# KumarRobotics/top_down_renderer

Measured on AMD Instinct MI355X. Metric: particle-updates/sec (render+score+resample), higher is better.
Workload: dtype f32

## Files before the change

### top_down_renderer_amd/csrc/tdr_common.h

```cpp
#ifndef TDR_COMMON_H_
#define TDR_COMMON_H_
#include <hip/hip_runtime.h>

#include <cmath>
#include <cstdarg>
#include <cstdint>
#include <cstdio>
#include <cstdlib>
#include <cstring>
#include <limits>
#include <type_traits>
#include <utility>
#include <vector>

#include "tdr.h"

#ifndef TDR_SCORE_U
#define TDR_SCORE_U 4
#endif
#ifndef TDR_INIT_SCAN_LDS
#define TDR_INIT_SCAN_LDS 1
#endif
#ifndef TDR_XCD_SWIZZLE
#define TDR_XCD_SWIZZLE 0
#endif
#ifndef TDR_OOB_ALIAS
#define TDR_OOB_ALIAS 1
#endif

int tdr_fail(int code, const char* fmt, ...);
#define fail tdr_fail
#define HIP_TRY(expr)                                                                       \
  do {                                                                                      \
    hipError_t e_ = (expr);                                                                 \
    if (e_ != hipSuccess) return fail(TDR_ERR_HIP, "%s: %s", #expr, hipGetErrorString(e_)); \
  } while (0)
#define LAUNCH_CHECK(name)                                                                   \
  do {                                                                                       \
    hipError_t e_ = hipGetLastError();                                                       \
    if (e_ != hipSuccess) return fail(TDR_ERR_HIP, "launch %s: %s", name, hipGetErrorString(e_)); \
  } while (0)

int tdr_libm_fma();

static inline int64_t cdiv(int64_t a, int64_t b) { return (a + b - 1) / b; }

template <class F>
static inline int with_flags(F&& f) { return f(); }
template <class F, class... Rest>
static inline int with_flags(F&& f, bool b, Rest... rest) {
  auto next = [&](auto B) { return with_flags([&](auto... bs) { return f(B, bs...); }, rest...); };
  return b ? next(std::true_type{}) : next(std::false_type{});
}
template <class F>
static inline int with_nv4(int rf, const char* who, F&& f) {
  switch (rf / 4) {
    case 1: return f(std::integral_constant<int, 1>{});
    case 2: return f(std::integral_constant<int, 2>{});
    case 3: return f(std::integral_constant<int, 3>{});
    case 4: return f(std::integral_constant<int, 4>{});
    default: return fail(TDR_ERR_ARG, "%s: unsupported record size %d", who, rf);
  }
}

int tdr_chain_total(const float* raw, const float* mean_dev, int kind, int64_t n, float* total_out, void* workspace,
                    hipStream_t st);
int tdr_uw_small(const float* raw, const float* last_dist, int64_t n, float* w, float* info, hipStream_t st);
int tdr_mt_raw_stream(const uint32_t* state, int64_t nblocks, uint32_t* raw, hipStream_t s);
int tdr_mt_advance(const uint32_t* raw, int64_t nblocks, const uint32_t* consumed, uint32_t* state, hipStream_t s);
bool tdr_score_polar_float_form(const tdr_map_desc* map, int nb, int nr, int64_t n, int64_t n_total);
__host__ __device__ inline bool tdr_has_kslot(int ncls, int rf) { return ncls + 2 <= rf; }
uint32_t* tdr_profile_stats_ptr();
#endif
```

### top_down_renderer_amd/csrc/tdr_filter.hip

```cpp
#include <random>

#include <rocprim/device/device_radix_sort.hpp>
using TdrSortConfig = rocprim::radix_sort_config<rocprim::default_config, rocprim::merge_sort_config<512, 512, 4>, rocprim::default_config>;

#include "tdr_common.h"
#include "tdr_filter_dev.h"

__device__ __forceinline__ uint32_t mulhi32(uint32_t a, uint32_t b) { return __umulhi(a, b); }
__device__ void philox4x32_10(uint32_t c[4], uint32_t k0, uint32_t k1) {
#pragma unroll
  for (int r = 0; r < 10; r++) {
    uint32_t hi0 = mulhi32(0xD2511F53u, c[0]), lo0 = 0xD2511F53u * c[0];
    uint32_t hi1 = mulhi32(0xCD9E8D57u, c[2]), lo1 = 0xCD9E8D57u * c[2];
    uint32_t n0 = hi1 ^ c[1] ^ k0, n1 = lo1, n2 = hi0 ^ c[3] ^ k1, n3 = lo0;
    c[0] = n0; c[1] = n1; c[2] = n2; c[3] = n3;
    k0 += 0x9E3779B9u; k1 += 0xBB67AE85u;
  }
}

__global__ void propagate_kernel(float* __restrict__ st, int64_t cap, int64_t n, float* __restrict__ last_dist,
                                 float tx, float ty, float omega, int scale_freeze, float pos_cov, float theta_cov,
                                 const float* __restrict__ z4, uint64_t seed, uint64_t step, int64_t index_base,
                                 int libm_fma) {
  const int64_t p = (int64_t)blockIdx.x * blockDim.x + threadIdx.x;
// ... 28 lines not shown
}

extern "C" void* tdr_rng_create(uint32_t seed) { return new std::mt19937(seed); }
extern "C" void tdr_rng_destroy(void* rng) { delete (std::mt19937*)rng; }
extern "C" float tdr_rng_uniform_host(void* rng) {
  std::uniform_real_distribution<float> d(0., 1.);
  return d(*(std::mt19937*)rng);
}
extern "C" int tdr_propagate_normals_host(void* rng, int64_t n, int scale_freeze, float* z4) {
  if (!rng || !z4 || n < 0) return fail(TDR_ERR_ARG, "propagate_normals: bad arguments");
  std::mt19937& gen = *(std::mt19937*)rng;
  for (int64_t p = 0; p < n; p++) {
    std::normal_distribution<float> disp{0, 1}, th{0, 1};
    z4[4 * p + 0] = th(gen);
    z4[4 * p + 1] = disp(gen);
    z4[4 * p + 2] = disp(gen);
    if (!scale_freeze) {
      std::normal_distribution<float> sc{0, 1};
      z4[4 * p + 3] = sc(gen);
    } else {
      z4[4 * p + 3] = 0.f;
    }
  }
  return TDR_OK;
}

static bool on_road_host(const float* maps, int ncls, int rows, int cols, float resolution, int px, int py) {
  const int c0 = (int)((float)px / resolution), c1 = (int)((float)py / resolution);
  if (ncls < 2) return false;
  if (!(c0 < cols && c1 < rows && c0 >= 0 && c1 >= 0)) return false;
  return maps[(size_t)1 * rows * cols + c1 + (size_t)rows * c0] < 1;
}
static tdr_state draw_particle(std::mt19937& gen, const float* maps, int ncls, int rows, int cols, float resolution,
                               const tdr_filter_params* fp) {
  std::uniform_real_distribution<float> uniform_dist(0., 1.);
  std::normal_distribution<float> normal_dist(0., 1.);
  tdr_state st;
  std::memset(&st, 0, sizeof(st));
  const float map_w = (float)cols * resolution, map_h = (float)rows * resolution;
  if (fp->fixed_scale < 0) st.scale = (float)std::pow(10, ((double)uniform_dist(gen) - 0.5) * 2);
  else st.scale = fp->fixed_scale;
  while (true) {
    if (fp->init_pos_px_x > 0) {
      st.init_x_px = std::min(std::max(normal_dist(gen) * fp->init_pos_px_cov + fp->init_pos_px_x, 0.f), map_w);
      st.init_y_px = std::min(std::max(normal_dist(gen) * fp->init_pos_px_cov + fp->init_pos_px_y, 0.f), map_h);
    } else {
      st.init_x_px = uniform_dist(gen) * map_w;
      st.init_y_px = uniform_dist(gen) * map_h;
    }
    if (on_road_host(maps, ncls, rows, cols, resolution, (int)st.init_x_px, (int)st.init_y_px)) break;
  }
  if (fp->init_pos_deg_theta != std::numeric_limits<float>::infinity()) {
    st.theta = normal_dist(gen) * fp->init_pos_deg_cov + fp->init_pos_deg_theta;
    st.theta = (float)((double)st.theta * (M_PI / 180));
    st.have_init = 1;
  } else {
    st.theta = 0;
    st.have_init = 0;
  }
  return st;
}
extern "C" int tdr_init_particle_host(void* rng, const float* class_maps, int ncls, int rows, int cols, float resolution,
                                      const tdr_filter_params* fp, tdr_state* out) {
  if (!rng || !class_maps || !fp || !out) return fail(TDR_ERR_ARG, "init_particle: bad arguments");
  if (ncls < 2) return fail(TDR_ERR_ARG, "init_particle: class 1 (road) is required for the on-road test");
  bool any_road = false;
  for (size_t k = 0; k < (size_t)rows * cols && !any_road; k++) any_road = class_maps[(size_t)rows * cols + k] < 1;
  if (!any_road) return fail(TDR_ERR_ARG, "init_particle: the map has no road cell, rejection sampling cannot end");
  *out = draw_particle(*(std::mt19937*)rng, class_maps, ncls, rows, cols, resolution, fp);
  return TDR_OK;
}
extern "C" int tdr_init_particles_host(void* rng, const float* class_maps, int ncls, int rows, int cols,
                                       float resolution, const tdr_filter_params* fp, int max_num, tdr_state* out,
                                       int64_t* n_out) {
  if (!rng || !class_maps || !fp || !out || !n_out || max_num < 0) return fail(TDR_ERR_ARG, "init_particles: bad arguments");
  if (ncls < 2) return fail(TDR_ERR_ARG, "init_particles: class 1 (road) is required for the on-road test");
  std::mt19937& gen = *(std::mt19937*)rng;
  bool any_road = false;
  for (size_t k = 0; k < (size_t)rows * cols && !any_road; k++) any_road = class_maps[(size_t)rows * cols + k] < 1;
  if (!any_road) return fail(TDR_ERR_ARG, "init_particles: the map has no road cell, rejection sampling cannot end");
  const size_t num_at_scale = (fp->fixed_scale < 0) ? 10 : 1;
  int64_t count = 0;
  for (int i = 0; i < (int)((size_t)max_num / num_at_scale); i++) {
    const tdr_state proto = draw_particle(gen, class_maps, ncls, rows, cols, resolution, fp);
    for (float scale = 0; scale < 1; scale += 1. / num_at_scale) {
      tdr_state part = draw_particle(gen, class_maps, ncls, rows, cols, resolution, fp);
      if (fp->fixed_scale < 0) {
        part = proto;
        part.scale = (float)std::pow(10., (double)scale);
      }
      if (count < max_num + 16) out[count] = part;
      count++;
      (void)draw_particle(gen, class_maps, ncls, rows, cols, resolution, fp);
    }
  }
  *n_out = count;
  return TDR_OK;
}

__device__ long long block_sum_ll(long long v, long long* sh) {
  const int lane = threadIdx.x & 63, wave = threadIdx.x >> 6;
  for (int o = 32; o > 0; o >>= 1) v += __shfl_down(v, o, 64);
  __syncthreads();
  if (lane == 0) sh[wave] = v;
  __syncthreads();
  long long t = 0;
  const int nw = blockDim.x >> 6;
  for (int w = 0; w < nw; w++) t += sh[w];
  return t;
}

#define UW_G 256
struct UwScratch {
  double a[UW_G];
  double b[UW_G];
};
__device__ __forceinline__ void uw_chunk(int64_t n, int64_t& lo, int64_t& hi) {
  const int64_t per = (n + UW_G - 1) / UW_G;
  lo = (int64_t)blockIdx.x * per;
  hi = lo + per < n ? lo + per : n;
  if (lo > n) lo = n;
}
__device__ double uw_total(const double* part) {
  __shared__ double stage[UW_G];
  __shared__ double result;
  __syncthreads();
  for (int g = threadIdx.x; g < UW_G; g += blockDim.x) stage[g] = part[g];
  __syncthreads();
  if (threadIdx.x == 0) {
    double t = 0;
    for (int g = 0; g < UW_G; g++) t += stage[g];
    result = t;
  }
  __syncthreads();
  return result;
}
__global__ __launch_bounds__(256) void uw_pass1(const float* __restrict__ raw, int64_t n, UwScratch* s1) {
  __shared__ double shd[4];
  __shared__ long long shl[4];
  int64_t lo, hi;
  uw_chunk(n, lo, hi);
  double s = 0;
  long long c = 0;
  for (int64_t i = lo + threadIdx.x; i < hi; i += 256) {
    const float v = raw[i];
    if (!isnan(v)) { s += (double)v; c++; }
  }
  const double ts = block_sum_d(s, shd);
  const long long tc = block_sum_ll(c, shl);
  if (threadIdx.x == 0) { s1->a[blockIdx.x] = ts; s1->b[blockIdx.x] = (double)tc; }
}
struct UwExact {
  float sum, mean, bsum, pad;
};
__global__ __launch_bounds__(256) void uw_pass2(const float* __restrict__ raw, int64_t n, const UwScratch* s1,
                                                UwScratch* s2, UwExact* ex) {
  __shared__ long long shl[4];
  const float mean = ex->sum / (float)(long long)uw_total(s1->b);
  int64_t lo, hi;
  uw_chunk(n, lo, hi);
  long long cu = 0;
  for (int64_t i = lo + threadIdx.x; i < hi; i += 256) {
    const float v = raw[i];
    if (!isnan(v) && v < mean) cu++;
  }
  const long long tc = block_sum_ll(cu, shl);
  if (threadIdx.x == 0) {
    s2->b[blockIdx.x] = (double)tc;
    if (blockIdx.x == 0) ex->mean = mean;
  }
}
__global__ __launch_bounds__(256) void uw_pass3(const float* __restrict__ raw, int64_t n, const UwExact* ex,
                                                const UwScratch* s2, UwScratch* s3, float* __restrict__ w) {
  __shared__ double shd[4];
  const float sum = ex->sum, mean = ex->mean;
  const long long num_under = (long long)uw_total(s2->b);
  const float bottom = sqrtf(ex->bsum / (float)num_under);
  const bool fallback = (sum == 0.f || num_under < 1);
  const float fill = mean - bottom;
  int64_t lo, hi;
  uw_chunk(n, lo, hi);
  double acc = 0;
  for (int64_t i = lo + threadIdx.x; i < hi; i += 256) {
    float v = raw[i];
    v = fallback ? 1.f : (isnan(v) ? fill : v);
    w[i] = v;
    acc += (double)v;
  }
  const double t = block_sum_d(acc, shd);
  if (threadIdx.x == 0) s3->a[blockIdx.x] = t;
}
__global__ __launch_bounds__(256) void uw_pass4(const float* __restrict__ last_dist, int64_t n, const UwScratch* s3,
                                                UwScratch* s4, float* __restrict__ w) {
  __shared__ double shd[4];
  const float fs1 = (float)uw_total(s3->a);
  const float fn = (float)n;
  int64_t lo, hi;
  uw_chunk(n, lo, hi);
  double acc = 0;
  for (int64_t i = lo + threadIdx.x; i < hi; i += 256) {
    float v = w[i] / fs1;
    const float d = fminf(last_dist[i] * 5.f, 1.f);
    v = d * v + (1.f - d) / fn;
    w[i] = v;
    acc += (double)v;
  }
  const double t = block_sum_d(acc, shd);
  if (threadIdx.x == 0) s4->a[blockIdx.x] = t;
}
__global__ __launch_bounds__(256) void uw_pass5(int64_t n, const UwScratch* s4, UwScratch* s5, float* __restrict__ w) {
  __shared__ float sb[4];
  __shared__ long long si[4];
  const float fs2 = (float)uw_total(s4->a);
  int64_t lo, hi;
  uw_chunk(n, lo, hi);
  float best = -INFINITY;
  long long besti = 0x7fffffffffffffffll;
  for (int64_t i = lo + threadIdx.x; i < hi; i += 256) {
    const float v = w[i] / fs2;
    w[i] = v;
    if (v > best || (v == best && i < besti)) { best = v; besti = i; }
  }
  for (int o = 32; o > 0; o >>= 1) {
    const float ob = __shfl_down(best, o, 64);
    const long long oi = __shfl_down(besti, o, 64);
    if (ob > best || (ob == best && oi < besti)) { best = ob; besti = oi; }
  }
  if ((threadIdx.x & 63) == 0) { sb[threadIdx.x >> 6] = best; si[threadIdx.x >> 6] = besti; }
  __syncthreads();
  if (threadIdx.x == 0) {
    for (int k = 1; k < 4; k++)
      if (sb[k] > best || (sb[k] == best && si[k] < besti)) { best = sb[k]; besti = si[k]; }
    s5->a[blockIdx.x] = (double)best;
    s5->b[blockIdx.x] = (double)besti;
  }
}
__global__ __launch_bounds__(256) void uw_pass6(int64_t n, const UwScratch* s1, const UwScratch* s2,
                                                const UwScratch* s5, const UwExact* ex, float* info) {
  static_assert(UW_G == 256, "one candidate per thread");
  __shared__ float sb[4];
  __shared__ long long si[4];
  float best = (float)s5->a[threadIdx.x];
  long long besti = (long long)s5->b[threadIdx.x];
  if (best != best) { best = -INFINITY; besti = 0x7fffffffffffffffll; }
  for (int o = 32; o > 0; o >>= 1) {
    const float ob = __shfl_down(best, o, 64);
    const long long oi = __shfl_down(besti, o, 64);
    if (ob > best || (ob == best && oi < besti)) { best = ob; besti = oi; }
  }
  if ((threadIdx.x & 63) == 0) { sb[threadIdx.x >> 6] = best; si[threadIdx.x >> 6] = besti; }
  const float sum = ex->sum, mean = ex->mean;
  const long long nv = (long long)uw_total(s1->b), nu = (long long)uw_total(s2->b);
  const float bottom = sqrtf(ex->bsum / (float)nu);
  if (threadIdx.x != 0) return;
  for (int k = 1; k < 4; k++)
    if (sb[k] > best || (sb[k] == best && si[k] < besti)) { best = sb[k]; besti = si[k]; }
  if (besti == 0x7fffffffffffffffll) besti = 0;
  info[0] = __int_as_float((int)besti);
  info[1] = sum; info[2] = mean; info[3] = bottom; info[4] = (sum == 0.f || nu < 1) ? 1.f : 0.f;
  info[5] = (float)nv; info[6] = (float)nu; info[7] = 0.f;
}

#define TDR_UW_SINGLE_MAX_N 32768
extern "C" int tdr_k_update_weights(const float* raw_w, const float* last_dist, int64_t n, float* w_out,
                                    float* info_out, void* stream) {
  if (!raw_w || !last_dist || !w_out || !info_out) return fail(TDR_ERR_ARG, "update_weights: null pointer");
  if (n < 1) return fail(TDR_ERR_ARG, "update_weights: n must be >= 1");
  hipStream_t s = (hipStream_t)stream;
  if (n <= TDR_UW_SINGLE_MAX_N) {
    const int rc = tdr_uw_small(raw_w, last_dist, n, w_out, info_out, s);
    if (rc) return rc;
    LAUNCH_CHECK("update_weights");
    return TDR_OK;
  }
  constexpr size_t kFixed = 8 * sizeof(float) + 64 + 5 * sizeof(UwScratch) + sizeof(UwExact) + 64;
  static_assert(kFixed + 32 * 1024 <= TDR_UW_INFO_FLOATS * sizeof(float), "info scratch");
  UwScratch* sc = reinterpret_cast<UwScratch*>(
      (reinterpret_cast<uintptr_t>(info_out + 8) + 63) & ~(uintptr_t)63);
  UwExact* ex = reinterpret_cast<UwExact*>(sc + 5);
  void* chain_ws = reinterpret_cast<void*>((reinterpret_cast<uintptr_t>(ex + 1) + 63) & ~(uintptr_t)63);
  const size_t chain_room = TDR_UW_INFO_FLOATS * sizeof(float) - kFixed;
  if ((size_t)tdr_prefix_workspace_bytes(n) > chain_room)
    return fail(TDR_ERR_ARG, "update_weights: n = %lld needs more than TDR_UW_INFO_FLOATS of scratch", (long long)n);
  hipLaunchKernelGGL(uw_pass1, dim3(UW_G), dim3(256), 0, s, raw_w, n, sc + 0);
  int rc = tdr_chain_total(raw_w, nullptr, 0, n, &ex->sum, chain_ws, s);
  if (rc) return rc;
  hipLaunchKernelGGL(uw_pass2, dim3(UW_G), dim3(256), 0, s, raw_w, n, (const UwScratch*)(sc + 0), sc + 1, ex);
  rc = tdr_chain_total(raw_w, &ex->mean, 1, n, &ex->bsum, chain_ws, s);
  if (rc) return rc;
  hipLaunchKernelGGL(uw_pass3, dim3(UW_G), dim3(256), 0, s, raw_w, n, (const UwExact*)ex, (const UwScratch*)(sc + 1),
                     sc + 2, w_out);
  hipLaunchKernelGGL(uw_pass4, dim3(UW_G), dim3(256), 0, s, last_dist, n, (const UwScratch*)(sc + 2), sc + 3, w_out);
  hipLaunchKernelGGL(uw_pass5, dim3(UW_G), dim3(256), 0, s, n, (const UwScratch*)(sc + 3), sc + 4, w_out);
  hipLaunchKernelGGL(uw_pass6, dim3(1), dim3(256), 0, s, n, (const UwScratch*)(sc + 0), (const UwScratch*)(sc + 1),
                     (const UwScratch*)(sc + 4), (const UwExact*)ex, info_out);
  LAUNCH_CHECK("update_weights(multi)");
  return TDR_OK;
}

__global__ void resample_kernel(const float* __restrict__ runmax, int64_t n, int64_t n_new, float shift,
                                int64_t i_begin, int64_t i_end, int32_t* __restrict__ idx) {
  const int64_t i = i_begin + (int64_t)blockIdx.x * blockDim.x + threadIdx.x;
  if (i >= i_end) return;
  idx[i - i_begin] = (int32_t)resample_pick(runmax, n, n_new, i, shift);
}

extern "C" int tdr_k_resample(const float* runmax, int64_t n, int64_t n_new, float shift, int64_t i_begin,
                              int64_t i_end, int32_t* idx_out, void* stream) {
  if (!runmax || !idx_out) return fail(TDR_ERR_ARG, "resample: null pointer");
  if (n < 1 || n_new < 1 || i_begin < 0 || i_end > n_new || i_begin > i_end)
    return fail(TDR_ERR_ARG, "resample: bad range");
  if (i_begin == i_end) return TDR_OK;
  hipLaunchKernelGGL(resample_kernel, dim3((unsigned)cdiv(i_end - i_begin, 256)), dim3(256), 0, (hipStream_t)stream,
                     runmax, n, n_new, shift, i_begin, i_end, idx_out);
  LAUNCH_CHECK("resample");
  return TDR_OK;
}

__global__ void resample_dev_kernel(const float* __restrict__ runmax, int64_t n, int64_t n_new, const float* __restrict__ shift_dev,
                                    int64_t i_begin, int64_t i_end, int32_t* __restrict__ idx) {
  const int64_t i = i_begin + (int64_t)blockIdx.x * blockDim.x + threadIdx.x;
  if (i >= i_end) return;
  idx[i - i_begin] = (int32_t)resample_pick(runmax, n, n_new, i, *shift_dev);
}
extern "C" int tdr_k_resample_dev(const float* runmax, int64_t n, int64_t n_new, const float* shift_dev, int64_t i_begin,
                                  int64_t i_end, int32_t* idx_out, void* stream) {
  if (!runmax || !idx_out || !shift_dev) return fail(TDR_ERR_ARG, "resample: null pointer");
  if (n < 1 || n_new < 1 || i_begin < 0 || i_end > n_new || i_begin > i_end)
    return fail(TDR_ERR_ARG, "resample: bad range");
  if (i_begin == i_end) return TDR_OK;
  hipLaunchKernelGGL(resample_dev_kernel, dim3((unsigned)cdiv(i_end - i_begin, 256)), dim3(256), 0, (hipStream_t)stream,
                     runmax, n, n_new, shift_dev, i_begin, i_end, idx_out);
  LAUNCH_CHECK("resample");
  return TDR_OK;
}

__global__ void gather_states_kernel(const float* __restrict__ src, int64_t src_cap, int64_t src_shard,
                                     const int32_t* __restrict__ idx, int64_t n_new, float* __restrict__ dst,
                                     int64_t dst_cap) {
  const int64_t i = (int64_t)blockIdx.x * blockDim.x + threadIdx.x;
  if (i >= n_new) return;
  const int64_t j = idx[i];
  if (src_shard > 0) {
    const int64_t r = j / src_shard, l = j - r * src_shard;
#pragma unroll
    for (int f = 0; f < TDR_ST_FIELDS; f++) dst[f * dst_cap + i] = src[(r * TDR_ST_FIELDS + f) * src_shard + l];
  } else {
    gather_particle(src, src_cap, j, dst, dst_cap, i);
  }
}

extern "C" int tdr_k_gather_states(const float* src, int64_t src_cap, int64_t src_shard, const int32_t* idx,
                                   int64_t n_new, float* dst, int64_t dst_cap, void* stream) {
  if (!src || !idx || !dst) return fail(TDR_ERR_ARG, "gather_states: null pointer");
  if (n_new < 0 || dst_cap < n_new || src_shard < 0) return fail(TDR_ERR_ARG, "gather_states: n_new exceeds capacity");
  if (n_new == 0) return TDR_OK;
  hipLaunchKernelGGL(gather_states_kernel, dim3((unsigned)cdiv(n_new, 256)), dim3(256), 0, (hipStream_t)stream, src,
                     src_cap, src_shard, idx, n_new, dst, dst_cap);
  LAUNCH_CHECK("gather_states");
  return TDR_OK;
}

__device__ __forceinline__ McScratch* mc_scratch(float* out) { return reinterpret_cast<McScratch*>(out + 24); }
__global__ __launch_bounds__(1024) void mean_cov_kernel(const float* __restrict__ st, int64_t cap, int64_t n,
                                                       const float* __restrict__ about, float* __restrict__ out,
                                                       int libm_fma) {
  mean_cov_body(st, cap, n, about, out, libm_fma);
}
__global__ __launch_bounds__(MC_THREADS) void mc_sums_kernel(const float* __restrict__ st, int64_t cap, int64_t n,
                                                             float* __restrict__ out, int libm_fma) {
  mc_sums_body(st, cap, n, mc_scratch(out), libm_fma);
}
__global__ __launch_bounds__(MC_THREADS) void mc_cov_kernel(const float* __restrict__ st, int64_t cap, int64_t n,
                                                            const float* __restrict__ about, float* __restrict__ out) {
  mc_cov_body(st, cap, n, about, mc_scratch(out));
}
__global__ __launch_bounds__(MC_THREADS) void mc_final_kernel(int64_t n, const float* __restrict__ about,
                                                              float* __restrict__ out) {
  mc_final_body(n, about, mc_scratch(out), out);
}

extern "C" int tdr_k_mean_cov(const float* st, int64_t cap, int64_t n, const float* about, float* out, void* stream) {
  if (!st || !out || n < 1 || cap < n) return fail(TDR_ERR_ARG, "mean_cov: bad arguments");
  hipStream_t s = (hipStream_t)stream;
  if (n <= MC_SINGLE_MAX_N) {
    hipLaunchKernelGGL(mean_cov_kernel, dim3(1), dim3(1024), 0, s, st, cap, n, about, out, tdr_libm_fma());
  } else {
    hipLaunchKernelGGL(mc_sums_kernel, dim3(MC_WGS), dim3(MC_THREADS), 0, s, st, cap, n, out, tdr_libm_fma());
    hipLaunchKernelGGL(mc_cov_kernel, dim3(MC_WGS), dim3(MC_THREADS), 0, s, st, cap, n, about, out);
    hipLaunchKernelGGL(mc_final_kernel, dim3(1), dim3(MC_THREADS), 0, s, n, about, out);
  }
  LAUNCH_CHECK("mean_cov");
  return TDR_OK;
}

__global__ void set_scale_kernel(float* __restrict__ st, int64_t cap, int64_t n, const float* __restrict__ scale) {
  const int64_t p = (int64_t)blockIdx.x * blockDim.x + threadIdx.x;
  if (p < n) st[TDR_ST_SCALE * cap + p] = *scale;
}
extern "C" int tdr_k_set_scale(float* st, int64_t cap, int64_t n, const float* scale_dev, void* stream) {
  if (!st || !scale_dev || n < 0 || cap < n) return fail(TDR_ERR_ARG, "set_scale: bad arguments");
  if (n == 0) return TDR_OK;
  hipLaunchKernelGGL(set_scale_kernel, dim3((unsigned)cdiv(n, 256)), dim3(256), 0, (hipStream_t)stream, st, cap, n,
                     scale_dev);
  LAUNCH_CHECK("set_scale");
  return TDR_OK;
}

__global__ void shift_init_kernel(float* __restrict__ st, int64_t cap, int64_t n, float dx, float dy) {
  const int64_t p = (int64_t)blockIdx.x * blockDim.x + threadIdx.x;
  if (p < n) {
    st[TDR_ST_INIT_X * cap + p] += dx;
    st[TDR_ST_INIT_Y * cap + p] += dy;
  }
}
extern "C" int tdr_k_shift_init(float* st, int64_t cap, int64_t n, float dx, float dy, void* stream) {
  if (!st || n < 0 || cap < n) return fail(TDR_ERR_ARG, "shift_init: bad arguments");
  if (n == 0) return TDR_OK;
  hipLaunchKernelGGL(shift_init_kernel, dim3((unsigned)cdiv(n, 256)), dim3(256), 0, (hipStream_t)stream, st, cap, n,
                     dx, dy);
  LAUNCH_CHECK("shift_init");
  return TDR_OK;
}

__global__ void save_ml_state_kernel(const float* __restrict__ info, const float* __restrict__ st, int64_t cap,
                                     int64_t src_shard, int64_t n, float* __restrict__ out) {
  if (threadIdx.x != 0 || blockIdx.x != 0) return;
  const int64_t best = ml_index(info, n);
  float f[TDR_ST_FIELDS];
  if (src_shard > 0) {
    const int64_t r = best / src_shard, l = best - r * src_shard;
#pragma unroll
    for (int k = 0; k < TDR_ST_FIELDS; k++) f[k] = st[(r * TDR_ST_FIELDS + k) * src_shard + l];
  } else {
#pragma unroll
    for (int k = 0; k < TDR_ST_FIELDS; k++) f[k] = st[(int64_t)k * cap + best];
  }
  ml_record(f, out);
}
extern "C" int tdr_k_save_ml_state(const float* info, const float* st, int64_t cap, int64_t src_shard, int64_t n,
                                   float* out12, void* stream) {
  if (!info || !st || !out12 || n < 1 || src_shard < 0 || (src_shard == 0 && cap < n))
    return fail(TDR_ERR_ARG, "save_ml_state: bad arguments");
  hipLaunchKernelGGL(save_ml_state_kernel, dim3(1), dim3(64), 0, (hipStream_t)stream, info, st, cap, src_shard, n,
                     out12);
  LAUNCH_CHECK("save_ml_state");
  return TDR_OK;
}
// ... 225 lines not shown
```

### top_down_renderer_amd/csrc/tdr_prefix.hip

```cpp
#include "tdr_common.h"
#include "tdr_batch.h"

#define TDR_PFX_BLOCK 4096
__global__ __launch_bounds__(64) void prefix_serial_kernel(const float* __restrict__ w, int64_t n,
                                                           float* __restrict__ runmax) {
  __shared__ float4 buf4[TDR_PFX_BLOCK / 4];
  float* buf = reinterpret_cast<float*>(buf4);
  const int lane = threadIdx.x;
  float run = 0.f;
  float carry_max = -INFINITY;
  for (int64_t base = 0; base < n; base += TDR_PFX_BLOCK) {
    const int cnt = (int)min((int64_t)TDR_PFX_BLOCK, n - base);
    for (int t = lane; t < TDR_PFX_BLOCK; t += 64) buf[t] = (t < cnt) ? w[base + t] : 0.f;
    __builtin_amdgcn_s_waitcnt(0);
    __builtin_amdgcn_wave_barrier();
    if (lane == 0) {
      const int q4 = (cnt + 3) / 4;
#pragma unroll 4
      for (int q = 0; q < q4; q++) {
        float4 v = buf4[q];
        run = run + v.x; v.x = run;
        run = run + v.y; v.y = run;
        run = run + v.z; v.z = run;
        run = run + v.w; v.w = run;
// ... 892 lines not shown
  typename A::value_t xv[K];
  a.load_items(lo, cnt, threadIdx.x * K, xv);
  PfxPair mine = {0u, 0u};
  bool anybad = false;
#pragma unroll
  for (int k = 0; k < K; k++) {
    unsigned f; bool tie, bad;
    A::classify(xv[k], (unsigned)re, f, tie, bad);
    anybad |= bad;
    mine = pfx_compose(mine, pfx_element_pair(f, tie));
  }
  if (anybad) s_bad = 1;
  PfxPair total;
  (void)pfx_pair_scan<NT>(mine, shp, total);
  if (threadIdx.x == 0) {
    const bool ok = s_bad == 0 && total.a0 < (1u << 24) && total.a1 < (1u << 24);
    ch[c].re = ok ? re : -1;
    ch[c].d0 = total.a0;
    ch[c].d1 = total.a1;
  }
}
#define PFXW_BLOCK 512
template <bool FILL, class CH, class SLOW>
__device__ __forceinline__ void chain_walk_chunks(CH* __restrict__ ch, int nch, int c_first, float& r, float& carry, SLOW slow) {
  __shared__ int sm_re[PFXW_BLOCK];
  __shared__ unsigned sm_d0[PFXW_BLOCK], sm_d1[PFXW_BLOCK];
  __shared__ int sm_acc[FILL ? PFXW_BLOCK : 1];
  __shared__ float sm_r0[FILL ? PFXW_BLOCK : 1], sm_c0[FILL ? PFXW_BLOCK : 1];
  for (int cb = 0; cb < nch; cb += PFXW_BLOCK) {
    pfx_sync();
    for (int t = threadIdx.x; t < PFXW_BLOCK && cb + t < nch; t += PFXW_THREADS) {
      const PfxChunk x = ch[cb + t];
      sm_re[t] = x.re; sm_d0[t] = x.d0; sm_d1[t] = x.d1;
      if constexpr (FILL) sm_acc[t] = 0;
    }
    pfx_sync();
    const int ce = min(nch, cb + PFXW_BLOCK);
    for (int c = max(cb, c_first); c < ce; c++) {
      const unsigned rb = __float_as_uint(r);
      const int re = (int)(rb >> 23);
      const unsigned R = (rb & 0x7FFFFFu) | 0x800000u;
      const unsigned D = (R & 1u) ? sm_d1[c - cb] : sm_d0[c - cb];
      if (c > 0 && sm_re[c - cb] == re && R + D < (1u << 24)) {
        if constexpr (FILL) { sm_r0[c - cb] = r; sm_c0[c - cb] = carry; sm_acc[c - cb] = 1; }
        r = chain_mant((unsigned)re, R + D);
        carry = fmaxf(carry, r);
      } else {
        slow(c);
      }
#ifdef TDR_PFX_TIMING
      if constexpr (FILL)
        if (threadIdx.x == 0) *reinterpret_cast<long long*>(&ch[c].sum) = (long long)wall_clock64();
#endif
    }
    if constexpr (FILL) {
      pfx_sync();
      for (int t = threadIdx.x; t < PFXW_BLOCK && cb + t < nch; t += PFXW_THREADS) {
        PfxChunk* o = ch + cb + t;
        o->r0 = sm_r0[t];
        o->carry0 = sm_c0[t];
        o->accepted = sm_acc[t];
      }
    }
  }
}

__global__ __launch_bounds__(PFXM_THREADS) void pfx_chunk_sum_kernel(const float* __restrict__ w, int64_t n,
                                                                     PfxChunk* __restrict__ ch) {
  chain_sum_body<PFXM_THREADS, PFXM_K>(PfxRunSum{{w}, CHAIN_RUNSUM, 0.f}, n, ch);
}
__global__ __launch_bounds__(PFXM_THREADS) void pfx_chunk_summary_kernel(const float* __restrict__ w, int64_t n,
                                                                         PfxChunk* __restrict__ ch, int c_first) {
  chain_summary_body<PFXM_THREADS, PFXM_K>(PfxRunSum{{w}, CHAIN_RUNSUM, 0.f}, n, ch, c_first);
}
#define PFXW_HEAD 64
static int g_pfx_head = PFXW_HEAD;
extern "C" int tdr_config_prefix_head(int n) {
  if (n >= 0) g_pfx_head = n < 1 ? 1 : (n > PFX_HEAD ? PFX_HEAD : n);
  return g_pfx_head;
}
__device__ __forceinline__ void pfx_walk_chunk(const float* __restrict__ w, long long lo, int cnt,
                                               float* __restrict__ runmax, float* __restrict__ prefix_opt,
                                               float& r, float& carry, int head_len) {
  __shared__ PfxPair shp[PFXW_THREADS / 64];
  __shared__ ChainWgStop<float> stp;
  const PfxRunSum a{{w}, CHAIN_RUNSUM, 0.f};
  const int t0 = threadIdx.x * PFXW_K;
  float wv[PFXW_K];
  a.load_items(lo, cnt, t0, wv);
  const ChainWg<PFXW_THREADS, float> sc{shp, &stp};
  PfxGlobalSink sink{w, lo, runmax, prefix_opt, carry, head_len};
  r = chain_walk(a, wv, t0, 0, cnt, r, sc, sink);
}
__global__ __launch_bounds__(PFXW_THREADS) void pfx_walk_kernel(const float* __restrict__ w, int64_t n,
                                                               PfxChunk* __restrict__ ch, int nch,
                                                               float* __restrict__ runmax,
                                                               float* __restrict__ prefix_opt, int head_len,
                                                               int c_first, const float* __restrict__ tail) {
  float r = c_first > 0 ? tail[0] : 0.f, carry = c_first > 0 ? tail[1] : -INFINITY;
  chain_walk_chunks<true>(ch, nch, c_first, r, carry, [&](int c) {
    const long long lo = (long long)c * PFXM_CHUNK;
    const int cnt = (int)min((long long)PFXM_CHUNK, (long long)n - lo);
    pfx_walk_chunk(w, lo, cnt, runmax, prefix_opt, r, carry, head_len);
  });
}
__global__ __launch_bounds__(PFXM_THREADS) void pfx_chunk_fill_kernel(const float* __restrict__ w, int64_t n,
                                                                      const PfxChunk* __restrict__ ch,
                                                                      float* __restrict__ runmax,
                                                                      float* __restrict__ prefix_opt) {
  __shared__ PfxPair shp[PFXM_THREADS / 64];
  const int c = blockIdx.x;
  const PfxChunk hdr = ch[c];
  if (!hdr.accepted) return;
  const long long lo = (long long)c * PFXM_CHUNK;
  const int cnt = (int)min((long long)PFXM_CHUNK, (long long)n - lo);
  const PfxRunSum a{{w}, CHAIN_RUNSUM, 0.f};
  const int t0 = threadIdx.x * PFXM_K;
  float wv[PFXM_K];
  a.load_items(lo, cnt, t0, wv);
  const ChainWg<PFXM_THREADS, float> sc{shp, nullptr};
  unsigned st[PFXM_K];
  (void)chain_step<false, PfxRunSum>(wv, t0, 0, cnt, hdr.r0, sc, st);
  float val[PFXM_K];
#pragma unroll
  for (int k = 0; k < PFXM_K; k++) val[k] = chain_mant(__float_as_uint(hdr.r0) >> 23, st[k]);
  const float carry = hdr.carry0;
  if (t0 + PFXM_K <= cnt && ((lo & 3) == 0)) {
    float4* o = reinterpret_cast<float4*>(runmax + lo + t0);
#pragma unroll
    for (int k = 0; k < PFXM_K / 4; k++)
      o[k] = make_float4(fmaxf(carry, val[4 * k]), fmaxf(carry, val[4 * k + 1]), fmaxf(carry, val[4 * k + 2]),
                         fmaxf(carry, val[4 * k + 3]));
    if (prefix_opt) {
      float4* q = reinterpret_cast<float4*>(prefix_opt + lo + t0);
#pragma unroll
      for (int k = 0; k < PFXM_K / 4; k++) q[k] = make_float4(val[4 * k], val[4 * k + 1], val[4 * k + 2], val[4 * k + 3]);
    }
  } else {
#pragma unroll
    for (int k = 0; k < PFXM_K; k++)
      if (t0 + k < cnt) {
        runmax[lo + t0 + k] = fmaxf(carry, val[k]);
        if (prefix_opt) prefix_opt[lo + t0 + k] = val[k];
      }
  }
}

struct ChainSrc {
  const float* raw;
  const float* mean;
  int kind;
};
__device__ __forceinline__ ChainStat chain_stat(const ChainSrc& s) { return {{s.raw}, s.kind, s.kind ? *s.mean : 0.f}; }
__global__ __launch_bounds__(PFXW_THREADS) void chain_sum_kernel(ChainSrc s, int64_t n, PfxChunk* __restrict__ ch) {
  chain_sum_body<PFXW_THREADS, CHAIN_K>(chain_stat(s), n, ch);
}
__global__ __launch_bounds__(PFXW_THREADS) void chain_summary_kernel(ChainSrc s, int64_t n, PfxChunk* __restrict__ ch,
                                                                    int c_first) {
  chain_summary_body<PFXW_THREADS, CHAIN_K>(chain_stat(s), n, ch, c_first);
}
template <class A>
__device__ __forceinline__ void chain_walk_chunk(const A& a, long long lo, int cnt, float& r, int pos) {
  __shared__ PfxPair shp[PFXW_THREADS / 64];
  __shared__ ChainWgStop<double> stp;
  const int t0 = threadIdx.x * CHAIN_K;
  double xv[CHAIN_K];
  a.load_items(lo, cnt, t0, xv);
  const ChainWg<PFXW_THREADS, double> sc{shp, &stp};
  ChainNoSink sink;
  r = chain_walk(a, xv, t0, pos, cnt, r, sc, sink);
}
__global__ __launch_bounds__(PFXW_THREADS) void chain_walk_kernel(ChainSrc s, int64_t n, const PfxChunk* __restrict__ ch,
                                                                 int nch, float* __restrict__ total_out, int c_first,
                                                                 const float* __restrict__ r_first) {
  const ChainStat a = chain_stat(s);
  const int hn = c_first > 0 ? 0 : (int)min((long long)CHAIN_HEAD, (long long)n);
  float r = chain_head_serial<PFXW_THREADS>(a, hn, c_first > 0 ? *r_first : 0.f), carry = 0.f;
  chain_walk_chunks<false>(ch, nch, c_first, r, carry, [&](int c) {
    const long long lo = (long long)c * PFXM_CHUNK;
    chain_walk_chunk(a, lo, (int)min((long long)PFXM_CHUNK, (long long)n - lo), r, c == 0 ? hn : 0);
  });
  if (threadIdx.x == 0) *total_out = r;
}
static int g_pfx_small = 1;
extern "C" int tdr_config_prefix_small(int on) {
  if (on >= 0) g_pfx_small = on ? 1 : 0;
  return g_pfx_small;
}
#define CHAIN_HEAD_N 32768
static int chain_head_chunks(int64_t n) { return (g_pfx_small && n >= CHAIN_HEAD_N) ? CHAIN_HEAD_N / PFXM_CHUNK : 0; }
static int chain_head_launch(const float* raw, const float* mean_dev, int kind, int n_head, float* r_out, hipStream_t st);
int tdr_chain_total(const float* raw, const float* mean_dev, int kind, int64_t n, float* total_out, void* workspace,
                    hipStream_t st) {
  const int64_t nch64 = cdiv(n, (int64_t)PFXM_CHUNK);
  if (nch64 > (1 << 24)) return fail(TDR_ERR_ARG, "chain_total: n too large");
  const int nch = (int)nch64;
  PfxChunk* ch = reinterpret_cast<PfxChunk*>(workspace);
  ChainSrc s{raw, mean_dev, kind};
  const int c_first = chain_head_chunks(n);
  hipLaunchKernelGGL(chain_sum_kernel, dim3(nch), dim3(PFXW_THREADS), 0, st, s, n, ch);
  if (nch > c_first)
    hipLaunchKernelGGL(chain_summary_kernel, dim3(nch - c_first), dim3(PFXW_THREADS), 0, st, s, n, ch, c_first);
  float* r_first = reinterpret_cast<float*>(&ch[0].r0);
  if (c_first > 0) {
    const int rc = chain_head_launch(raw, mean_dev, kind, c_first * PFXM_CHUNK, r_first, st);
    if (rc) return rc;
  }
  hipLaunchKernelGGL(chain_walk_kernel, dim3(1), dim3(PFXW_THREADS), 0, st, s, n, (const PfxChunk*)ch, nch, total_out,
                     c_first, (const float*)r_first);
  return TDR_OK;
}

__device__ __forceinline__ float uws_chain_total(int kind, int n, float mean) {
  const UwsWgAdd a{{}, kind, mean};
  const int hn = min(CHAIN_HEAD, n);
  float r = chain_head_serial<PFXW_THREADS>(a, hn, 0.f);
  UW_STAMP(kind ? 5 : 2);
  const int nch = (n + PFXM_CHUNK - 1) / PFXM_CHUNK;
  for (int c = 0; c < nch; c++) {
    const int lo = c * PFXM_CHUNK;
    const int cnt = min((int)PFXM_CHUNK, n - lo);
    if (c == 0 && hn >= cnt) continue;
    chain_walk_chunk(a, lo, cnt, r, c == 0 ? hn : 0);
  }
  return r;
}
#define UWS_THREADS 1024
#define UWS_DUAL_SLOTS 8
#define UWS_DUAL_FLAG 0x100
struct UwsShared {
  double csum[64];
  int code[64];
  unsigned d0[64], d1[64];
  uint4 dual[UWS_DUAL_SLOTS][64];
  double shd[UWS_THREADS / 64];
  float total;
};
template <class A>
__device__ __forceinline__ float uws_wave_walk(const A& a, int lo, int cnt, float r, int pos) {
  const auto ad = a.as_double();
  const int t0 = (threadIdx.x & 63) * CHAIN_K;
  double xv[CHAIN_K];
  ad.load_items(lo, cnt, t0, xv);
  ChainNoSink sink;
  return chain_walk(ad, xv, t0, pos, cnt, r, ChainWave<false>{}, sink);
}
template <class A>
__device__ __forceinline__ float uws_wave_dual(const A& a, int lo, int cnt, float r, const uint4* pq, int& pos) {
  const int lane = threadIdx.x & 63, t0 = lane * CHAIN_K;
  const unsigned rb = __float_as_uint(r), re = rb >> 23, R = (rb & 0x7FFFFFu) | 0x800000u;
  const uint4 v = pq[lane];
  const unsigned after = R + ((R & 1u) ? v.y : v.x);
  const unsigned long long cross = __ballot(after >= (1u << 24));
  pos = cnt;
  if (cross == 0ull) return chain_mant(re, (unsigned)__builtin_amdgcn_readlane((int)after, 63));
  const int L = __ffsll((long long)cross) - 1;
  float rl = chain_mant(re, L > 0 ? (unsigned)__builtin_amdgcn_readlane((int)after, L - 1) : R);
  typename A::value_t x[CHAIN_K];
  a.load_items(lo, cnt, t0, x);
#pragma unroll
  for (int k = 0; k < CHAIN_K; k++) rl = chain_add(rl, x[k]);
  const float r2 = __uint_as_float((unsigned)__builtin_amdgcn_readlane((int)__float_as_uint(rl), L));
  const unsigned rb2 = __float_as_uint(r2), R2 = (rb2 & 0x7FFFFFu) | 0x800000u;
  const int next = (L + 1) * CHAIN_K;
  if (next >= cnt) return r2;
  pos = next;
  if ((rb2 >> 23) != re + 1u) return r2;
  const unsigned qL = (unsigned)__builtin_amdgcn_readlane((int)v.z, L);
  if (qL != (unsigned)__builtin_amdgcn_readlane((int)v.w, L)) return r2;
  const unsigned q63 = (unsigned)__builtin_amdgcn_readlane((int)(((R2 + qL) & 1u) ? v.w : v.z), 63);
  if (q63 >= PFXM_SAT || R2 + (q63 - qL) >= (1u << 24)) return r2;
  pos = cnt;
  return chain_mant(re + 1u, R2 + (q63 - qL));
}
template <class A>
__device__ __forceinline__ float uws_chain_total_waves(const A& a, int n, UwsShared& sh, float* rin = nullptr) {
  const int kind = a.kind;
  constexpr int NW = UWS_THREADS / 64;
  const int lane = threadIdx.x & 63, wave = __builtin_amdgcn_readfirstlane(threadIdx.x >> 6), t0 = lane * CHAIN_K;
  const int nwc = (n + UWS_WC - 1) / UWS_WC;
  float r = 0.f;
  if (wave == 0) {
    r = kind == CHAIN_RUNSUM ? chain_head_lanes<true>(a, min(UWS_WC, n)) : chain_head_lanes<false>(a, min(UWS_WC, n));
  } else {
    int my_code;
    {
      const double own = lane < nwc ? sh.csum[lane] : 0.0;
      const double after = uws_wave_scan_d(own), before = after - own;
      const int re_b = (int)(__float_as_uint((float)before) >> 23), re_a = (int)(__float_as_uint((float)after) >> 23);
      const bool inr = lane >= 1 && lane < nwc && re_b >= PFXM_RE_MIN && re_a <= PFXM_RE_MAX;
      const bool dualc = inr && re_a == re_b + 1;
      const unsigned long long dm = __ballot(dualc);
      const int slot = __popcll(dm & ((1ull << lane) - 1ull));
      my_code = (inr && re_a == re_b) ? re_b : (dualc && slot < UWS_DUAL_SLOTS) ? (re_b | UWS_DUAL_FLAG | (slot << 16)) : -1;
    }
    for (int c = wave; c < nwc; c += NW - 1) {
      const int code = __builtin_amdgcn_readlane(my_code, c);
      const int lo = c * UWS_WC, cnt = min(UWS_WC, n - lo);
      PfxPair P = {0u, 0u}, Q = {0u, 0u};
      bool anybad = false;
      if (code >= 0) {
        const unsigned re = (unsigned)(code & 0xFF);
        const bool dual = (code & UWS_DUAL_FLAG) != 0;
        typename A::value_t x[CHAIN_K];
        a.load_items(lo, cnt, t0, x);
        bool anytie = false;
        unsigned f; bool tie, bad;
#pragma unroll
        for (int k = 0; k < CHAIN_K; k++) {
          A::classify(x[k], re, f, tie, bad);
          anybad |= bad; anytie |= tie;
          P.a0 += f;
        }
        if (dual) {
#pragma unroll
          for (int k = 0; k < CHAIN_K; k++) {
            A::classify(x[k], re + 1u, f, tie, bad);
            anybad |= bad; anytie |= tie;
            Q.a0 += f;
          }
        }
        if (__ballot(anytie) == 0ull) {
          P.a0 = P.a1 = uws_wave_scan_u(P.a0);
          if (dual) Q.a0 = Q.a1 = uws_wave_scan_u(Q.a0);
        } else {
          unsigned re_t = re;
          asm volatile("" : "+s"(re_t));
          P = PfxPair{0u, 0u}; Q = PfxPair{0u, 0u};
#pragma unroll
          for (int k = 0; k < CHAIN_K; k++) {
            A::classify(x[k], re_t, f, tie, bad);
            P = pfx_compose(P, pfx_element_pair(f, tie));
          }
          P = pfx_pair_wave_scan(P);
          if (dual) {
#pragma unroll
            for (int k = 0; k < CHAIN_K; k++) {
              A::classify(x[k], re_t + 1u, f, tie, bad);
              Q = pfx_compose(Q, pfx_element_pair(f, tie));
            }
            Q = pfx_pair_wave_scan(Q);
          }
        }
        if (dual) sh.dual[code >> 16][lane] = make_uint4(P.a0, P.a1, Q.a0, Q.a1);
      }
      const bool ok = code >= 0 && __ballot(anybad) == 0ull;
      if (lane == 63) {
        sh.code[c] = (ok && ((code & UWS_DUAL_FLAG) || (P.a0 < (1u << 24) && P.a1 < (1u << 24)))) ? code : -1;
        sh.d0[c] = P.a0; sh.d1[c] = P.a1;
      }
    }
  }
  pfx_sync();
  UW_STAMP(kind ? 5 : 2);
  if (wave == 0) {
    const int v_code = (lane >= 1 && lane < nwc) ? sh.code[lane] : -1;
    const unsigned v_d0 = (lane >= 1 && lane < nwc) ? sh.d0[lane] : 0u, v_d1 = (lane >= 1 && lane < nwc) ? sh.d1[lane] : 0u;
    float v_rin = 0.f;
    int c = 1;
    while (c < nwc) {
      const unsigned rb = __float_as_uint(r);
      const int re = (int)(rb >> 23);
// ... 528 lines not shown
```

### top_down_renderer_amd/csrc/tdr_score.hip

```cpp

#include "tdr_common.h"
#include "tdr_batch.h"
#include "tdr_sincosf.h"

struct ScoreArgs {
  const float* rec;
  int rows, cols;
  float resolution;
  const float* tab;
  const float* utab = nullptr;
  const float* scan_pk;
  int nb, nr;
  float res;
  const float* st;
  int64_t cap, n;
  const int32_t* order;
  const int32_t* count = nullptr;
  const int32_t* slot_base = nullptr;
  int use_theta_override = 0;
  float theta_override = 0.f;
  int only_uninit = 0;
  int group, nchunks;
  int64_t npad;
  float* part;
// ... 54 lines not shown

  if constexpr (COMPACT)
    for (int t = threadIdx.x; t < a.dict_n; t += 256) ldict[t] = a.dict[t];
  const int rs = (a.group * NV4) | 1;
  for (int jj = 0; jj < gn; jj++)
    for (int t = threadIdx.x; t < nb * NV4; t += 256) {
      const float4 v = scan4[(int64_t)(j0 + jj) * nb * NV4 + t];
      const int row = t / NV4, pl = t - row * NV4;
      ring[row * rs + jj * NV4 + pl] = v;
    }
  __syncthreads();

  typedef float tdr_v2f __attribute__((ext_vector_type(2)));
  const tdr_v2f offv = {off0, off1};
  auto cell_offset = [&](float2 t) -> unsigned {
    tdr_v2f pv = {t.x, t.y};
    if constexpr (!USCALE) pv = (pv * scale) * a.res;
    pv = pv + offv;
    tdr_v2f qv = {__builtin_amdgcn_fmed3f(pv.x, -1.f, rmaxf), __builtin_amdgcn_fmed3f(pv.y, -1.f, cmaxf)};
    qv = qv + 0.49999997f;
    int ri, ci;
    asm("v_cvt_flr_i32_f32 %0, %1" : "=v"(ri) : "v"(qv.x));
    asm("v_cvt_flr_i32_f32 %0, %1" : "=v"(ci) : "v"(qv.y));
    if constexpr (COMPACT) {
      return cmap_offset<CW, LC>(ri, ci, ckcol, ckconst);
    } else {
#if TDR_OOB_ALIAS
      const bool inb = (unsigned)ri < (unsigned)a.rows && (unsigned)ci < (unsigned)a.cols;
      return inb ? (unsigned)(__mul24(ri, rowstride) + (ci * (RF * 4) + kbase)) : 0u;
#else
      return (unsigned)(__mul24(ri, rowstride) + (ci * (RF * 4) + kbase));
#endif
    }
  };
  struct Raw { uint32_t w[COMPACT ? CW : 1]; float4 q[COMPACT ? 1 : NV4]; };
  auto load_raw = [&](unsigned off, Raw& r) {
    if constexpr (COMPACT) cmap_load<CW>(crecb, off, r.w);
    else {
#pragma unroll
      for (int v = 0; v < NV4; v++) r.q[v] = *reinterpret_cast<const float4*>(recb + off + 16 * v);
    }
  };
  auto operands = [&](const Raw& r, float (&m)[RF]) {
    if constexpr (WIDE) cmap_decode_wide<RF, KSLOT>(r.w, ldict, m);
    else if constexpr (COMPACT) cmap_decode<RF, KSLOT>(r.w, ldict, m);
    else {
#pragma unroll
      for (int v = 0; v < NV4; v++) { m[4 * v] = r.q[v].x; m[4 * v + 1] = r.q[v].y; m[4 * v + 2] = r.q[v].z; m[4 * v + 3] = r.q[v].w; }
    }
  };

  float acc[RF];
#pragma unroll
  for (int k = 0; k < RF; k++) acc[k] = 0.f;
  float known = 0.f;
  auto step = [&](auto full_step, const unsigned (&boff)[U], const float4* const (&sp)[U], int cnt) {
    constexpr bool FULL = decltype(full_step)::value;
    Raw raw[U];
    float4 s[U][NV4];
#pragma unroll
    for (int u = 0; u < U; u++)
      if (FULL || u < cnt) load_raw(boff[u], raw[u]);
#pragma unroll
    for (int u = 0; u < U; u++)
      if (FULL || u < cnt) {
#pragma unroll
        for (int v = 0; v < NV4; v++) s[u][v] = sp[u][v];
      }
#pragma unroll
    for (int u = 0; u < U; u++)
      if (FULL || u < cnt) {
        float m[RF];
        operands(raw[u], m);
#pragma unroll
        for (int v = 0; v < NV4; v++) {
          acc[4 * v + 0] = __builtin_fmaf(s[u][v].x, m[4 * v + 0], acc[4 * v + 0]);
          acc[4 * v + 1] = __builtin_fmaf(s[u][v].y, m[4 * v + 1], acc[4 * v + 1]);
          acc[4 * v + 2] = __builtin_fmaf(s[u][v].z, m[4 * v + 2], acc[4 * v + 2]);
          acc[4 * v + 3] = __builtin_fmaf(s[u][v].w, m[4 * v + 3], acc[4 * v + 3]);
        }
        if (!KSLOT) known += m[RF - 1];
      }
  };
  if (gn >= U) {
    const int gfull = gn - gn % U;
    for (int i = 0; i < nb; i++) {
      int row = i + shift;
      row -= row >= nb ? nb : 0;
      const float4* const rl = ring + __mul24(row, rs);
      for (int jj = 0; jj < gfull; jj += U) {
        unsigned boff[U];
        const float4* sp[U];
        const float4* const rj = rl + jj * NV4;
#pragma unroll
        for (int u = 0; u < U; u++) {
          boff[u] = cell_offset(tab_at((int64_t)(j0 + jj + u) * nb + i));
          sp[u] = rj + u * NV4;
        }
        step(std::true_type{}, boff, sp, U);
      }
    }
    if (gfull < gn) {
      for (int i = 0; i < nb; i++) {
        int row = i + shift;
        row -= row >= nb ? nb : 0;
        const float4* const rl = ring + __mul24(row, rs);
        unsigned boff[U];
        const float4* sp[U];
#pragma unroll
        for (int u = 0; u < U; u++) {
          const int jc = min(gfull + u, gn - 1);
          boff[u] = cell_offset(tab_at((int64_t)(j0 + jc) * nb + i));
          sp[u] = rl + jc * NV4;
        }
        step(std::false_type{}, boff, sp, gn - gfull);
      }
    }
  } else {
    for (int jj = 0; jj < gn; jj++) {
      const float4* const rj = ring + jj * NV4;
      for (int i = 0; i < nb; i += U) {
        unsigned boff[U];
        const float4* sp[U];
#pragma unroll
        for (int u = 0; u < U; u++) {
          const int ic = min(i + u, nb - 1);
          int row = ic + shift;
          row -= row >= nb ? nb : 0;
          boff[u] = cell_offset(tab_at((int64_t)(j0 + jj) * nb + ic));
          sp[u] = rj + __mul24(row, rs);
        }
        step(std::false_type{}, boff, sp, min(U, nb - i));
      }
    }
  }
  if (sbase + slot < a.npad) {
    float* o = a.part + (int64_t)by * (RF + 1) * a.npad + sbase + slot;
#pragma unroll
    for (int k = 0; k < RF; k++) o[(int64_t)k * a.npad] = acc[k];
    o[(int64_t)RF * a.npad] = KSLOT ? acc[RF - 2] : known;
  }
  TDR_TL_END(g_timeline)
}
template <int NV4, int U, bool KSLOT, bool USCALE, bool COMPACT, bool WIDE = false>
__global__ __launch_bounds__(256, COMPACT ? (WIDE ? 3 : 5) : 1) void score_polar_kernel(ScoreArgs a) {
#if TDR_XCD_SWIZZLE
  const unsigned nbx = gridDim.x, per = (nbx + 7) / 8;
  unsigned bx = (blockIdx.x % 8) * per + blockIdx.x / 8;
  if (nbx % 8 != 0) bx = blockIdx.x;
#else
  const unsigned bx = blockIdx.x;
#endif
  score_polar_body<NV4, U, KSLOT, USCALE, COMPACT, WIDE>(a, bx, blockIdx.y);
}
template <int NV4, int U, bool KSLOT, bool USCALE, bool COMPACT, bool WIDE = false>
__global__ __launch_bounds__(256, COMPACT ? (WIDE ? 3 : 5) : 1) void score_polar_batch_kernel(const ScoreArgs* __restrict__ args,
                                                                                              const int32_t* __restrict__ blk, int k) {
  const int e = batch_find(k, (int)blockIdx.x, [&](int i) { return blk[i]; });
  const ScoreArgs a = args[e];
  if ((int)blockIdx.y >= a.nchunks || (a.utab != nullptr) != USCALE) return;
  score_polar_body<NV4, U, KSLOT, USCALE, COMPACT, WIDE>(a, blockIdx.x - (unsigned)blk[e], blockIdx.y);
}

__device__ __forceinline__ float linspaced_dev(int i, int size1, float low, float high, float step) {
  return (i == size1) ? high : (low + (float)i * step);
}

template <int NV4, int U, bool KSLOT, bool COMPACT, bool WIDE = false>
__global__ __launch_bounds__(256) void score_cart_kernel(CartArgs a) {
  constexpr int RF = 4 * NV4;
  static_assert(!WIDE || (COMPACT && NV4 == 2), "wide compact records: 8-float dense records only");
  constexpr int CW = WIDE ? 4 : CmapShape<RF, KSLOT>::CW, LC = WIDE ? 1 : CmapShape<RF, KSLOT>::LC;
  __shared__ float ldict[COMPACT ? (WIDE ? TDR_CMAP_WIDE_MAX_DICT : TDR_CMAP_MAX_DICT) : 1];
  if constexpr (COMPACT) {
    for (int t = threadIdx.x; t < a.dict_n; t += 256) ldict[t] = a.dict[t];
    __syncthreads();
  }
  const int lane = threadIdx.x & 63, wave = threadIdx.x >> 6;
  const int64_t slot = ((int64_t)blockIdx.x * 4 + wave) * 64 + lane;
  if ((int64_t)blockIdx.x * 256 >= a.n) return;
  const bool valid = slot < a.n;
  const int64_t p = a.order ? (int64_t)a.order[valid ? slot : 0] : (valid ? slot : 0);
  const float scale = a.st[TDR_ST_SCALE * a.cap + p];
  const float cx = a.st[TDR_ST_DX * a.cap + p] * scale + a.st[TDR_ST_INIT_X * a.cap + p];
  const float cy = a.st[TDR_ST_DY * a.cap + p] * scale + a.st[TDR_ST_INIT_Y * a.cap + p];
  const float theta = a.st[TDR_ST_THETA * a.cap + p];
  const float off0 = cy / a.resolution;
  const float off1 = cx / a.resolution;
  const float resq = (a.res * scale) / a.resolution;
  const float c = tdr_libm::cosf_v(theta, a.libm_fma), s = tdr_libm::sinf_v(theta, a.libm_fma);
  const float ns = -s;
  typedef float tdr_v2f __attribute__((ext_vector_type(2)));
  const tdr_v2f cs = {c, s}, offv = {off0, off1};
  const float lo_r = (float)((double)(-resq * (float)(a.rows - 1)) / 2.), hi_r = (float)((double)(resq * (float)(a.rows - 1)) / 2.);
  const float lo_c = (float)((double)(-resq * (float)(a.cols - 1)) / 2.), hi_c = (float)((double)(resq * (float)(a.cols - 1)) / 2.);
  const float step_r = a.rows == 1 ? 0.f : (hi_r - lo_r) / (float)(a.rows - 1);
  const float step_c = a.cols == 1 ? 0.f : (hi_c - lo_c) / (float)(a.cols - 1);
  const int r1 = a.rows == 1 ? 1 : a.rows - 1, c1 = a.cols == 1 ? 1 : a.cols - 1;

  const int j0 = blockIdx.y * a.cpc, j1 = min(a.cols, j0 + a.cpc);
  const int rowstride = (a.map_cols + 2) * (RF * 4);
  const int kbase = (a.map_cols + 3) * (RF * 4);
  const float rmaxf = (float)a.map_rows, cmaxf = (float)a.map_cols;
  const char* __restrict__ recb = reinterpret_cast<const char*>(a.rec);
  const char* __restrict__ crecb = reinterpret_cast<const char*>(a.crec);
  const int ckcol = a.ctiles_r * 128 - 16 * CW, ckconst = a.ctiles_r * 128 + 128;
  typedef const float __attribute__((address_space(4))) * tdr_const_f;
  const tdr_const_f scanc = (tdr_const_f)a.scan_pk;

  float acc[RF];
#pragma unroll
  for (int k = 0; k < RF; k++) acc[k] = 0.f;
  float known = 0.f;
  auto fetch = [&](unsigned off, float (&m)[RF]) {
    if constexpr (COMPACT) {
      uint32_t w[CW];
      cmap_load<CW>(crecb, off, w);
      if constexpr (WIDE) cmap_decode_wide<RF, KSLOT>(w, ldict, m);
      else cmap_decode<RF, KSLOT>(w, ldict, m);
    } else {
#pragma unroll
      for (int v = 0; v < NV4; v++) {
        const float4 q = *reinterpret_cast<const float4*>(recb + off + 16 * v);
        m[4 * v + 0] = q.x; m[4 * v + 1] = q.y; m[4 * v + 2] = q.z; m[4 * v + 3] = q.w;
      }
    }
  };
  auto cell_offset = [&](tdr_v2f cyi, tdr_v2f AB) -> unsigned {
    tdr_v2f pv = cyi + AB;
    pv = pv + offv;
    tdr_v2f qv = {__builtin_amdgcn_fmed3f(pv.x, -1.f, rmaxf), __builtin_amdgcn_fmed3f(pv.y, -1.f, cmaxf)};
    qv = qv + 0.49999997f;
    int ri, ci;
    asm("v_cvt_flr_i32_f32 %0, %1" : "=v"(ri) : "v"(qv.x));
    asm("v_cvt_flr_i32_f32 %0, %1" : "=v"(ci) : "v"(qv.y));
    const bool inb = (unsigned)ri < (unsigned)a.map_rows && (unsigned)ci < (unsigned)a.map_cols;
    if constexpr (COMPACT) return cmap_offset<CW, LC>(ri, ci, ckcol, ckconst);
    else return inb ? (unsigned)(__mul24(ri, rowstride) + (ci * (RF * 4) + kbase)) : 0u;
  };
  auto column_terms = [&](int j) -> tdr_v2f {
    const float xj = linspaced_dev(j, c1, lo_c, hi_c, step_c);
    return (tdr_v2f){ns * xj, c * xj};
  };
  int i = 0;
  for (; i + U <= a.rows - 1; i += U) {
    tdr_v2f cyi[U];
#pragma unroll
    for (int u = 0; u < U; u++) cyi[u] = cs * (lo_r + (float)(i + u) * step_r);
    for (int j = j0; j < j1; j++) {
      const tdr_v2f AB = column_terms(j);
      unsigned boff[U];
#pragma unroll
      for (int u = 0; u < U; u++) boff[u] = cell_offset(cyi[u], AB);
      float m[U][RF];
#pragma unroll
      for (int u = 0; u < U; u++) fetch(boff[u], m[u]);
      const int64_t sbase = ((int64_t)j * a.rows + i) * RF;
#pragma unroll
      for (int u = 0; u < U; u++) {
#pragma unroll
        for (int k = 0; k < RF; k++) acc[k] = __builtin_fmaf(scanc[sbase + u * RF + k], m[u][k], acc[k]);
        if (!KSLOT) known += m[u][RF - 1];
      }
    }
  }
  for (; i < a.rows; i++) {
    const tdr_v2f cyi = cs * linspaced_dev(i, r1, lo_r, hi_r, step_r);
    for (int j = j0; j < j1; j++) {
      float m[RF];
      fetch(cell_offset(cyi, column_terms(j)), m);
      const int64_t sbase = ((int64_t)j * a.rows + i) * RF;
#pragma unroll
      for (int k = 0; k < RF; k++) acc[k] = __builtin_fmaf(scanc[sbase + k], m[k], acc[k]);
      if (!KSLOT) known += m[RF - 1];
    }
  }
  if (slot < a.npad) {
    float* o = a.part + (int64_t)blockIdx.y * (RF + 1) * a.npad + slot;
#pragma unroll
    for (int k = 0; k < RF; k++) o[(int64_t)k * a.npad] = acc[k];
    o[(int64_t)RF * a.npad] = KSLOT ? acc[RF - 2] : known;
  }
}

struct LocalMapArgs {
  const float* rec;
  int map_rows, map_cols, ncls, rf;
  float resolution;
  const float* tab;
  int rows, cols;
  float cx, cy, scale_or_rot, res;
  float* dists;
  uint8_t* mask;
  int libm_fma;
};
template <bool POLAR>
__global__ void local_map_kernel(LocalMapArgs a) {
  const int64_t P = (int64_t)a.rows * a.cols;
  const int64_t k = (int64_t)blockIdx.x * blockDim.x + threadIdx.x;
  if (k >= P) return;
  const float off0 = a.cy / a.resolution, off1 = a.cx / a.resolution;
  float p0, p1;
  if constexpr (POLAR) {
    p0 = (a.tab[2 * k] * a.scale_or_rot) * a.res + off0;
    p1 = (a.tab[2 * k + 1] * a.scale_or_rot) * a.res + off1;
  } else {
    const int i = (int)(k % a.rows), j = (int)(k / a.rows);
    const float resq = a.res / a.resolution;
    const float c = tdr_libm::cosf_v(a.scale_or_rot, a.libm_fma), s = tdr_libm::sinf_v(a.scale_or_rot, a.libm_fma);
    const float lo_r = (float)((double)(-resq * (float)(a.rows - 1)) / 2.), hi_r = (float)((double)(resq * (float)(a.rows - 1)) / 2.);
    const float lo_c = (float)((double)(-resq * (float)(a.cols - 1)) / 2.), hi_c = (float)((double)(resq * (float)(a.cols - 1)) / 2.);
    const float step_r = a.rows == 1 ? 0.f : (hi_r - lo_r) / (float)(a.rows - 1);
    const float step_c = a.cols == 1 ? 0.f : (hi_c - lo_c) / (float)(a.cols - 1);
    const float yi = linspaced_dev(i, a.rows == 1 ? 1 : a.rows - 1, lo_r, hi_r, step_r);
    const float xj = linspaced_dev(j, a.cols == 1 ? 1 : a.cols - 1, lo_c, hi_c, step_c);
    p0 = (c * yi + (-s) * xj) + off0;
    p1 = (s * yi + c * xj) + off1;
  }
  p0 = __builtin_amdgcn_fmed3f(p0, -1.f, (float)a.map_rows);
  p1 = __builtin_amdgcn_fmed3f(p1, -1.f, (float)a.map_cols);
  const int ri = round_half_away_clamped(p0), ci = round_half_away_clamped(p1);
  const bool inb = (unsigned)ri < (unsigned)a.map_rows && (unsigned)ci < (unsigned)a.map_cols;
  const float* r = a.rec + ((int64_t)(ri + 1) * (a.map_cols + 2) + (ci + 1)) * a.rf;
  for (int c = 0; c < a.ncls; c++) a.dists[(int64_t)c * P + k] = inb ? r[c] : 0.f;
  a.mask[k] = inb ? (uint8_t)(r[a.rf - 1] == 0.f ? 1 : 0) : (uint8_t)1;
}
static int launch_local_map(bool polar, const tdr_map_desc* map, const float* tab, int rows, int cols, float cx, float cy,
                            float scale_or_rot, float res, float* dists_out, uint8_t* mask_out, void* stream) {
  if (!map || !map->rec || !dists_out || !mask_out || (polar && !tab))
    return fail(TDR_ERR_ARG, "local_map: null pointer");
  if (rows < 1 || cols < 1) return fail(TDR_ERR_ARG, "local_map: bad window shape");
  if (!(map->resolution > 0.f)) return fail(TDR_ERR_ARG, "local_map: map resolution must be > 0");
  LocalMapArgs a;
  a.rec = map->rec; a.map_rows = map->rows; a.map_cols = map->cols; a.ncls = map->ncls; a.rf = map->rec_floats;
  a.resolution = map->resolution; a.tab = tab; a.rows = rows; a.cols = cols; a.cx = cx; a.cy = cy;
  a.scale_or_rot = scale_or_rot; a.res = res; a.dists = dists_out; a.mask = mask_out;
  a.libm_fma = tdr_libm_fma();
  const dim3 grid((unsigned)cdiv((int64_t)rows * cols, 256)), block(256);
  if (polar) hipLaunchKernelGGL((local_map_kernel<true>), grid, block, 0, (hipStream_t)stream, a);
  else hipLaunchKernelGGL((local_map_kernel<false>), grid, block, 0, (hipStream_t)stream, a);
  LAUNCH_CHECK("local_map");
  return TDR_OK;
}
extern "C" int tdr_k_local_map_polar(const tdr_map_desc* map, const float* tab, int nb, int nr, float cx, float cy,
                                     float scale, float res, float* dists_out, uint8_t* mask_out, void* stream) {
  return launch_local_map(true, map, tab, nb, nr, cx, cy, scale, res, dists_out, mask_out, stream);
}
extern "C" int tdr_k_local_map_cart(const tdr_map_desc* map, int rows, int cols, float cx, float cy, float rot,
                                    float res, float* dists_out, uint8_t* mask_out, void* stream) {
  return launch_local_map(false, map, nullptr, rows, cols, cx, cy, rot, res, dists_out, mask_out, stream);
}

struct FinalizeArgs {
  const float* part;
  int rf, nchunks;
  int64_t npad, n, cap;
  const int32_t* order;
  const int32_t* count = nullptr;
  float* st;
  tdr_filter_params fp;
  GateArgs gate;
  int64_t P;
  int ncls;
  int mode = 0;
  int first = 0;
  float theta_override = 0.f;
  float* raw_w;
  float* best_cost = nullptr;
  float* best_theta = nullptr;
  const float* gpart = nullptr;
  int gnchunks = 0;
  float gsum0 = 0.f, gsum1 = 0.f;
  int only_uninit = 0;
  int tlog = 0;
  const int32_t* run_if = nullptr;
  const uint32_t* ipart = nullptr;
  const uint32_t* dict_tail = nullptr;
  const int32_t* counts = nullptr;
  const int32_t* inexact = nullptr;
  int ray_split = 1;
};

__device__ __forceinline__ void score_finalize_body(const FinalizeArgs& a, const int64_t gid) {
  const int T = 1 << a.tlog, t = (int)(gid & (T - 1));
  const int64_t slot = gid >> a.tlog;
  if (a.run_if && !int_form_off(a.run_if)) return;
  const int64_t nact = a.count ? (int64_t)*a.count : a.n;
  if (slot >= nact) return;
  const int64_t p = a.order ? (int64_t)a.order[slot] : slot;
  if (p < 0) return;
  const float scale = a.st[TDR_ST_SCALE * a.cap + p];
  const float cx = a.st[TDR_ST_DX * a.cap + p] * scale + a.st[TDR_ST_INIT_X * a.cap + p];
  const float cy = a.st[TDR_ST_DY * a.cap + p] * scale + a.st[TDR_ST_INIT_Y * a.cap + p];
  if (a.mode == 0 && particle_gated(a.gate, cx, cy, scale)) {
    a.raw_w[p] = 0.f;
    return;
  }
  if (a.mode == 1 && a.only_uninit && a.st[TDR_ST_HAVE_INIT * a.cap + p] != 0.f) return;
  constexpr int FIN_B = 4, FIN_S = TDR_MAX_CLASSES + 2;
  double tot[FIN_S];
#pragma unroll
  for (int k = 0; k < FIN_S; k++) tot[k] = 0;
  const int64_t cstride = (int64_t)(a.rf + 1) * a.npad;
  auto slot_row = [&](int k) { return k < a.ncls ? k : (k == a.ncls ? a.rf - 1 : a.rf); };
  const int share = (a.nchunks + T - 1) >> a.tlog, cend = min(a.nchunks, (t + 1) * share);
  int c0 = t * share;
  for (; c0 + FIN_B <= cend; c0 += FIN_B) {
    float v[FIN_B][FIN_S];
#pragma unroll
    for (int b = 0; b < FIN_B; b++)
#pragma unroll
      for (int k = 0; k < FIN_S; k++)
        if (k < a.ncls + 2) v[b][k] = a.part[(int64_t)(c0 + b) * cstride + (int64_t)slot_row(k) * a.npad + slot];
#pragma unroll
    for (int b = 0; b < FIN_B; b++)
#pragma unroll
      for (int k = 0; k < FIN_S; k++)
        if (k < a.ncls + 2) tot[k] += (double)v[b][k];
  }
  for (; c0 < cend; c0++) {
#pragma unroll
    for (int k = 0; k < FIN_S; k++)
      if (k < a.ncls + 2) tot[k] += (double)a.part[(int64_t)c0 * cstride + (int64_t)slot_row(k) * a.npad + slot];
  }
  if (T > 1) {
    for (int sft = T >> 1; sft >= 1; sft >>= 1)
#pragma unroll
      for (int k = 0; k < FIN_S; k++)
        if (k < a.ncls + 2) tot[k] += __shfl_xor(tot[k], sft, 64);
    if (t != 0) return;
  }
  double known = 0, norm = 0;
#pragma unroll
  for (int k = 0; k < FIN_S; k++) {
    if (k == a.ncls) norm = tot[k];
    if (k == a.ncls + 1) known = tot[k];
  }
  float cost;
  if ((float)known / (float)a.P < 0.5) {
    cost = __builtin_nanf("");
  } else {
    cost = 0.f;
#pragma unroll
    for (int k = 0; k < TDR_MAX_CLASSES; k++)
      if (k < a.ncls) cost = (float)((double)cost + (double)(float)tot[k] * 0.01 * (double)a.fp.class_weights[k]);
    float normf = (float)norm;
    if (a.gpart) {
      double g[2] = {0, 0};
      const int64_t gstride = (int64_t)5 * a.npad;
      for (int c0g = 0; c0g < a.gnchunks; c0g++) {
        g[0] += (double)a.gpart[(int64_t)c0g * gstride + slot];
        g[1] += (double)a.gpart[(int64_t)c0g * gstride + a.npad + slot];
      }
      cost = (float)((double)cost + (double)(float)g[0] * 0.01);
      normf = normf + a.gsum0;
      cost = (float)((double)cost + (double)(float)g[1] * 0.01);
      normf = normf + a.gsum1;
    }
    cost = cost / normf;
  }
  if (a.mode == 0) {
    a.raw_w[p] = (float)(1. / (double)(cost + a.fp.regularization));
  } else {
    float best = a.first ? 3.402823466e+38f : a.best_cost[slot];
    float bt = a.first ? 0.f : a.best_theta[slot];
    if (cost < best) { best = cost; bt = a.theta_override; }
    a.best_cost[slot] = best;
    a.best_theta[slot] = bt;
  }
}
__global__ __launch_bounds__(256) void score_finalize_kernel(FinalizeArgs a) {
  score_finalize_body(a, (int64_t)blockIdx.x * blockDim.x + threadIdx.x);
}
__global__ __launch_bounds__(256) void score_finalize_batch_kernel(const FinalizeArgs* __restrict__ args,
                                                                   const int32_t* __restrict__ blk, int k) {
  const int e = batch_find(k, (int)blockIdx.x, [&](int i) { return blk[i]; });
  const FinalizeArgs a = args[e];
  score_finalize_body(a, (int64_t)(blockIdx.x - (unsigned)blk[e]) * blockDim.x + threadIdx.x);
}

__global__ __launch_bounds__(256) void score_finalize_exact_kernel(FinalizeArgs a) {
  __shared__ unsigned long long red[3][TDR_MAX_CLASSES + 2][64];
  if (int_form_off(a.inexact)) return;
  const int lane = threadIdx.x & 63, t = threadIdx.x >> 6;
  const int64_t nslots = (int64_t)a.counts[2];
  if ((int64_t)blockIdx.x * 64 >= nslots) return;
  const int64_t slot = min((int64_t)blockIdx.x * 64 + lane, nslots - 1);
  const int rows = 2 * a.ncls + 2;
  const int nch = slot < (int64_t)a.counts[0] ? a.nchunks : a.ray_split;
  unsigned long long tot[TDR_MAX_CLASSES], norm = 0, known = 0;
#pragma unroll
  for (int k = 0; k < TDR_MAX_CLASSES; k++) tot[k] = 0;
  for (int c = t; c < nch; c += 4) {
    const uint32_t* o = a.ipart + (int64_t)c * rows * a.npad + slot;
#pragma unroll
    for (int k = 0; k < TDR_MAX_CLASSES; k++)
      if (k < a.ncls)
        tot[k] += (unsigned long long)o[(int64_t)(2 * k) * a.npad] | ((unsigned long long)o[(int64_t)(2 * k + 1) * a.npad] << 32);
    norm += o[(int64_t)(2 * a.ncls) * a.npad];
    known += o[(int64_t)(2 * a.ncls + 1) * a.npad];
  }
  if (t > 0) {
#pragma unroll
    for (int k = 0; k < TDR_MAX_CLASSES; k++)
      if (k < a.ncls) red[t - 1][k][lane] = tot[k];
    red[t - 1][TDR_MAX_CLASSES][lane] = norm;
    red[t - 1][TDR_MAX_CLASSES + 1][lane] = known;
  }
  __syncthreads();
  if (t > 0 || (int64_t)blockIdx.x * 64 + lane >= nslots) return;
  for (int u = 0; u < 3; u++) {
#pragma unroll
    for (int k = 0; k < TDR_MAX_CLASSES; k++)
      if (k < a.ncls) tot[k] += red[u][k][lane];
    norm += red[u][TDR_MAX_CLASSES][lane];
    known += red[u][TDR_MAX_CLASSES + 1][lane];
  }
  const int64_t p = a.order[slot];
  if (p < 0) return;
  const float scale = a.st[TDR_ST_SCALE * a.cap + p];
  const float cx = a.st[TDR_ST_DX * a.cap + p] * scale + a.st[TDR_ST_INIT_X * a.cap + p];
  const float cy = a.st[TDR_ST_DY * a.cap + p] * scale + a.st[TDR_ST_INIT_Y * a.cap + p];
  if (particle_gated(a.gate, cx, cy, scale)) {
    a.raw_w[p] = 0.f;
    return;
  }
  float cost;
  if ((float)known / (float)a.P < 0.5) {
    cost = __builtin_nanf("");
  } else {
    const int q = (int)a.dict_tail[0];
    cost = 0.f;
#pragma unroll
    for (int k = 0; k < TDR_MAX_CLASSES; k++)
      if (k < a.ncls) {
        const float dot = (float)ldexp((double)tot[k], -q);
        cost = (float)((double)cost + (double)dot * 0.01 * (double)a.fp.class_weights[k]);
      }
    cost = cost / (float)norm;
  }
  a.raw_w[p] = (float)(1. / (double)(cost + a.fp.regularization));
}

static int finalize_tlog(int nchunks, int64_t nslots) {
  int tl = 0;
  while (tl < 4 && (nchunks >> (tl + 1)) >= 4 && (nslots << (tl + 1)) <= 131072) tl++;
  return tl;
}
static void launch_finalize(FinalizeArgs& f, int64_t nslots, hipStream_t s) {
  f.tlog = finalize_tlog(f.nchunks, nslots);
  hipLaunchKernelGGL(score_finalize_kernel, dim3((unsigned)cdiv(nslots << f.tlog, 256)), dim3(256), 0, s, f);
}

#define TDR_CART_WAVE_MUL 2
static int64_t g_score_waves = 131072;
static int g_score_group = 0;
static int g_su_group = 0;
static int64_t score_wave_target() { return g_score_waves; }
extern "C" int tdr_config_init_ahead(int);
extern "C" int tdr_config_batch_init_search(int);
extern "C" int tdr_config_prefix_head(int);
extern "C" int tdr_config_ray_block_major(int);
extern "C" int tdr_config_ray_patch(int);
extern "C" int tdr_config_ray_borrow(int);
extern "C" int tdr_config_cart_seg_rows(int);
extern "C" int tdr_config_mt_stretches(int);
extern "C" int tdr_config_su_wave_span(int);
extern "C" int tdr_config_su_lds_pad(int);
extern "C" int tdr_config_su_tail_groups(int);
extern "C" int tdr_config_su_tail_parts(int);
extern "C" int tdr_config_su_order_bucket(int);
extern "C" int tdr_config_init_device(int);
extern "C" int64_t tdr_config_init_window_words(int64_t);
extern "C" int64_t tdr_config_cart_init_chunk(int64_t);
extern "C" int64_t tdr_config_tuning(const char* name, int64_t value) {
  if (!name) return -1;
  const std::string n(name);
  if (n == "score_waves") { if (value > 0) g_score_waves = value; return g_score_waves; }
  if (n == "score_group") { if (value >= 0) g_score_group = (int)value; return g_score_group; }
  if (n == "su_group") { if (value >= 0) g_su_group = (int)value; return g_su_group; }
  if (n == "batch_init_search") return tdr_config_batch_init_search((int)std::max<int64_t>(value, -1));
  if (n == "init_ahead") return tdr_config_init_ahead((int)std::min<int64_t>(std::max<int64_t>(value, -1), 3));
  if (n == "prefix_head") return tdr_config_prefix_head((int)std::max<int64_t>(value, -1));
  if (n == "ray_borrow") return tdr_config_ray_borrow((int)std::max<int64_t>(value, -1));
  if (n == "ray_patch") return tdr_config_ray_patch((int)std::max<int64_t>(value, -1));
  if (n == "ray_block_major") return tdr_config_ray_block_major((int)std::max<int64_t>(value, -1));
  if (n == "cart_seg_rows") return tdr_config_cart_seg_rows((int)std::max<int64_t>(value, -1));
  if (n == "mt_stretches") return tdr_config_mt_stretches((int)std::max<int64_t>(value, -1));
  if (n == "su_lds_pad") return tdr_config_su_lds_pad((int)std::max<int64_t>(value, -1));
  if (n == "su_tail_groups") return tdr_config_su_tail_groups((int)std::min<int64_t>(std::max<int64_t>(value, -1), 1 << 20));
  if (n == "su_tail_parts") return tdr_config_su_tail_parts((int)std::min<int64_t>(std::max<int64_t>(value, -1), 8));
  if (n == "su_order_bucket") return tdr_config_su_order_bucket((int)std::max<int64_t>(value, -1));
  if (n == "su_wave_span") return tdr_config_su_wave_span((int)std::max<int64_t>(value, -1));
  if (n == "init_device") return tdr_config_init_device((int)std::max<int64_t>(value, -1));
  if (n == "init_window_words") return tdr_config_init_window_words(value > 0 ? value : -1);
  if (n == "cart_init_chunk") return tdr_config_cart_init_chunk(value > 0 ? value : -1);
  return -1;
}
static void choose_chunks(int64_t n, int nr, int& rpc, int& nchunks, int target_mul = 1) {
  int64_t nbatches = cdiv(std::max<int64_t>(n, 1), 64);
  int64_t want = std::max<int64_t>(1, cdiv(score_wave_target() * target_mul, nbatches));
  nchunks = (int)std::min<int64_t>(nr, want);
  rpc = (int)cdiv(nr, nchunks);
  nchunks = (int)cdiv(nr, rpc);
}

__global__ void utab_kernel(const float* __restrict__ tab, int64_t n2, float scale, float res,
                            float* __restrict__ utab) {
  const int64_t k = (int64_t)blockIdx.x * blockDim.x + threadIdx.x;
  if (k < n2) utab[k] = (tab[k] * scale) * res;
}

static int score_group_rings(int nb, int nr, int rf, int64_t n_total) {
  const int forced = g_score_group;
  const int64_t ring_bytes = std::max<int64_t>((int64_t)nb * rf * 4, 1);
  int g = (int)std::min<int64_t>(8, (32 * 1024) / ring_bytes);
  const int64_t chunks_wanted = cdiv(2048, cdiv(std::max<int64_t>(n_total, 1), 256));
  g = (int)std::min<int64_t>(g, std::max<int64_t>(1, nr / std::max<int64_t>(chunks_wanted, 1)));
  if (forced > 0) g = forced;
  g = std::max(1, std::min<int>(g, (int)((60 * 1024) / ring_bytes)));
  if (g >= TDR_SCORE_U) g -= g % TDR_SCORE_U;
  return std::max(g, 1);
}
extern "C" int tdr_cmap_words(int ncls);
struct ScoreWs {
  int group, nchunks;
  int su_group, su_nchunks;
  int su_tail_k, su_tail_q, su_rows;
  int64_t npad, npad_part, off_aux, off_utab, off_su, total;
  bool su;
  SuWs suw;
};
static ScoreWs score_ws(int ncls, int nb, int nr, int64_t n, int64_t n_total) {
  ScoreWs w;
  const int rf = tdr_rec_floats(ncls);
  if (n_total <= 0) n_total = n;
  w.group = score_group_rings(nb, nr, rf, n_total);
  if (w.group % 4 != 0 && tdr_cmap_words(ncls) != 0 && tdr_su_shape_ok(nb, nr, 4, n_total))
    w.group = std::max(4, w.group - w.group % 4);
  w.nchunks = (int)cdiv(nr, w.group);
  w.npad = cdiv(std::max<int64_t>(n, 1), 64) * 64;
  w.su = tdr_su_shape_ok(nb, nr, w.group, n_total) && tdr_cmap_words(ncls) != 0;
  w.su_group = w.group;
  {
    const int forced = g_su_group;
    if (w.su && w.group == 4 && nr % 8 == 0 && cdiv(n_total, 256) * (nr / 8) >= 4096) w.su_group = 8;
    int k16 = 0, q16 = 1;
    if (w.su && w.su_group == 8 && nr % 16 == 0 && cdiv(std::max<int64_t>(n, 1), 256) * (nr / 16) >= 4096)
      tdr_su_tail(nr / 16, std::max<int64_t>(n, 1), &k16, &q16);
    if (k16 > 0) w.su_group = 16;
    if (w.su && forced >= 4 && forced % 4 == 0) w.su_group = forced;
  }
  w.su_nchunks = (int)cdiv(nr, w.su_group);
  tdr_su_tail(w.su_nchunks, std::max<int64_t>(n, 1), &w.su_tail_k, &w.su_tail_q);
  {
    int g, s0, s1;
    w.su_rows = su_tail_plan(w.su_nchunks, w.su_tail_k, w.su_tail_q, -1, &g, &s0, &s1);
  }
  w.npad_part = w.su ? su_npad(std::max<int64_t>(n, 1), nb) : w.npad;
  w.off_aux = w.su ? (int64_t)std::max(std::max(w.nchunks, w.su_rows), TDR_RAY_MAX_SPLIT) * std::max(rf + 1, 2 * ncls + 2) * w.npad_part
                   : (int64_t)w.nchunks * (rf + 1) * w.npad_part;
  w.off_utab = w.off_aux + 3 * w.npad + 64;
  w.off_su = (w.off_utab + 2 * (int64_t)nb * nr + 63) / 64 * 64;
  w.total = w.off_su;
  if (w.su) {
    w.suw = tdr_su_ws(nb, nr, w.su_group, std::max<int64_t>(n, 1));
    w.total += w.suw.total;
  }
  return w;
}
extern "C" size_t tdr_score_workspace_floats(int ncls, int nb, int nr, int64_t n, int64_t n_total) {
  if (ncls < 1 || ncls > TDR_MAX_CLASSES || nb < 1 || nr < 1 || n < 0) return 0;
  return (size_t)score_ws(ncls, nb, nr, n, n_total).total;
}
static int fill_utab(ScoreArgs& a, float* workspace, const ScoreWs& W, float uniform_scale, hipStream_t s) {
  a.utab = nullptr;
  if (!(uniform_scale > 0.f)) return TDR_OK;
  float* ut = workspace + W.off_utab;
  const int64_t n2 = 2 * (int64_t)a.nb * a.nr;
  hipLaunchKernelGGL(utab_kernel, dim3((unsigned)cdiv(n2, 256)), dim3(256), 0, s, a.tab, n2, uniform_scale, a.res, ut);
  LAUNCH_CHECK("utab");
  a.utab = ut;
  return TDR_OK;
}

static bool g_prof_on = false;
static std::vector<std::pair<hipEvent_t, hipEvent_t>> g_prof_events;
static size_t g_prof_used = 0;
struct ScoreProfScope {
  hipStream_t s;
  hipEvent_t stop = nullptr;
  explicit ScoreProfScope(hipStream_t s_, bool on = true) : s(s_) {
    if (!g_prof_on || !on) return;
    if (g_prof_used == g_prof_events.size()) {
      hipEvent_t a, b;
      if (hipEventCreate(&a) != hipSuccess || hipEventCreate(&b) != hipSuccess) return;
      g_prof_events.emplace_back(a, b);
    }
    auto& ev = g_prof_events[g_prof_used++];
    (void)hipEventRecord(ev.first, s);
    stop = ev.second;
  }
  ~ScoreProfScope() {
    if (stop) (void)hipEventRecord(stop, s);
  }
};
static hipEvent_t g_share_ev[2][2] = {{nullptr, nullptr}, {nullptr, nullptr}};
static bool g_share_valid = false;
static const int32_t* g_share_counts = nullptr;
struct ShareProfScope {
  hipStream_t s;
  hipEvent_t stop = nullptr;
  ShareProfScope(int which, hipStream_t s_, bool on) : s(s_) {
    if (!g_prof_on || !on) return;
    for (int k = 0; k < 2; k++)
      if (!g_share_ev[which][k] && hipEventCreate(&g_share_ev[which][k]) != hipSuccess) return;
    (void)hipEventRecord(g_share_ev[which][0], s);
    stop = g_share_ev[which][1];
  }
  ~ShareProfScope() {
    if (stop) (void)hipEventRecord(stop, s);
  }
};
static uint32_t* g_variant_stats = nullptr;
static bool g_prof_variants = false;
uint32_t* tdr_profile_stats_ptr() {
  if (!g_prof_on || !g_prof_variants) return nullptr;
  if (!g_variant_stats) {
    if (hipMalloc((void**)&g_variant_stats, 16 * sizeof(uint32_t)) != hipSuccess) { g_variant_stats = nullptr; return nullptr; }
    (void)hipMemset(g_variant_stats, 0, 16 * sizeof(uint32_t));
  }
  return g_variant_stats;
}
extern "C" int tdr_profile_variants(int64_t out[16]) {
  if (!out) return fail(TDR_ERR_ARG, "profile_variants: null pointer");
  for (int k = 0; k < 16; k++) out[k] = 0;
  if (!g_variant_stats) return TDR_OK;
  uint32_t h[16];
  HIP_TRY(hipDeviceSynchronize());
  HIP_TRY(hipMemcpy(h, g_variant_stats, sizeof(h), hipMemcpyDeviceToHost));
  HIP_TRY(hipMemset(g_variant_stats, 0, sizeof(h)));
  for (int k = 0; k < 16; k++) out[k] = h[k];
  return TDR_OK;
}
extern "C" int tdr_profile_enable(int on) {
  g_prof_on = on != 0;
  g_prof_variants = on == 2;
  g_prof_used = 0;
  g_share_valid = false;
  return TDR_OK;
}
extern "C" int tdr_profile_shares(double* dense_ms, double* scattered_ms, int64_t* scattered_particles) {
  if (!dense_ms || !scattered_ms || !scattered_particles) return fail(TDR_ERR_ARG, "profile_shares: null pointer");
  if (!g_share_valid || !g_share_counts) return fail(TDR_ERR_ARG, "profile_shares: no integer-form launch was profiled");
  float ms[2] = {0.f, 0.f};
  for (int k = 0; k < 2; k++) {
    HIP_TRY(hipEventSynchronize(g_share_ev[k][1]));
    HIP_TRY(hipEventElapsedTime(&ms[k], g_share_ev[k][0], g_share_ev[k][1]));
  }
  int32_t counts[3] = {0, 0, 0};
  HIP_TRY(hipMemcpy(counts, g_share_counts, sizeof(counts), hipMemcpyDeviceToHost));
  *scattered_ms = ms[0];
  *dense_ms = ms[1];
  *scattered_particles = counts[1];
  return TDR_OK;
}
extern "C" int tdr_profile_score_ms(double* total_ms, int64_t* launches) {
  if (!total_ms || !launches) return fail(TDR_ERR_ARG, "profile_score_ms: null pointer");
  double tot = 0;
  for (size_t i = 0; i < g_prof_used; i++) {
    HIP_TRY(hipEventSynchronize(g_prof_events[i].second));
    float ms = 0;
    HIP_TRY(hipEventElapsedTime(&ms, g_prof_events[i].first, g_prof_events[i].second));
    tot += ms;
  }
  *total_ms = tot;
  *launches = (int64_t)g_prof_used;
  g_prof_used = 0;
  return TDR_OK;
}

static int check_map_addressing(const tdr_map_desc* map, int rf, const char* who) {
  const uint64_t row_bytes = (uint64_t)(map->cols + 2) * rf * 4;
  const uint64_t total = row_bytes * (uint64_t)(map->rows + 2);
  if (row_bytes >= (1u << 24) || total > 0xFFFFFFFFull)
    return fail(TDR_ERR_ARG, "%s: map of %d x %d cells (%d-float records) exceeds the 4 GiB the kernels address", who,
                map->rows, map->cols, rf);
  return TDR_OK;
}

static int g_use_compact = 1;
extern "C" int tdr_config_compact(int on) {
  if (on >= 0) g_use_compact = on ? 1 : 0;
  return g_use_compact;
}
extern "C" int tdr_cmap_words(int ncls);
extern "C" size_t tdr_cmap_tile_words(int ncls, int rows, int cols);

static bool map_is_wide(const tdr_map_desc* map, int rf) {
  return rf == 8 && map->cwords == 4 && map->dict_n > TDR_CMAP_MAX_DICT;
}
static int compact_lc(const tdr_map_desc* map) {
  return map->cwords == 1 ? 3 : (map->cwords == 2 ? 2 : 1);
}
static bool map_has_compact(const tdr_map_desc* map, int rf) {
  if (!(g_use_compact && map->cwords > 0 && map->crec && map->dict && map->dict_n > 0 && rf <= 12 &&
        (map->cwords == tdr_cmap_words(map->ncls) || map_is_wide(map, rf))))
    return false;
  if (map->dict_n > (map_is_wide(map, rf) ? TDR_CMAP_WIDE_MAX_DICT : TDR_CMAP_MAX_DICT)) return false;
  return (int64_t)((map->rows >> compact_lc(map)) + 2) * 128 < (1 << 23) && map->cols < (1 << 24);
}
template <class Args>
static bool set_compact(Args& a, const tdr_map_desc* map, int rf) {
  const bool cm = map_has_compact(map, rf);
  a.crec = cm ? map->crec : nullptr;
  a.dict = cm ? map->dict : nullptr;
  a.dict_n = cm ? map->dict_n : 0;
  a.ctiles_r = cm ? (map->rows >> compact_lc(map)) + 2 : 0;
  return cm;
}
static size_t polar_lds_bytes(int nb, int group, int rf) { return (size_t)nb * ((group * (rf / 4)) | 1) * 16; }

template <bool BATCH, class F>
static int with_polar_kernel(const tdr_map_desc* map, int rf, bool us, const char* who, F&& f) {
  const bool cm = map_has_compact(map, rf);
  return with_nv4(rf, who, [&](auto N) {
    return with_flags([&](auto KS, auto US, auto CM, auto WD) {
      constexpr int NV4 = decltype(N)::value;
      constexpr bool ks = decltype(KS)::value, usc = decltype(US)::value, c = decltype(CM)::value, w = decltype(WD)::value;
      if constexpr ((c && NV4 == 4) || (w && !(c && NV4 == 2))) return fail(TDR_ERR_ARG, "%s: no kernel for this record form", who);
      else if constexpr (BATCH) return f(score_polar_batch_kernel<NV4, TDR_SCORE_U, ks, usc, c, w>);
      else return f(score_polar_kernel<NV4, TDR_SCORE_U, ks, usc, c, w>);
    }, tdr_has_kslot(map->ncls, rf), us, cm, cm && map_is_wide(map, rf));
  });
}
template <class K>
static void allow_lds(K kfn, size_t lds) {
  if (lds > 65536) (void)hipFuncSetAttribute(reinterpret_cast<const void*>(kfn), hipFuncAttributeMaxDynamicSharedMemorySize, (int)lds);
}
static int launch_score(ScoreArgs a, const tdr_map_desc* map, int rf, hipStream_t s, bool profile = true) {
  ScoreProfScope prof(profile ? s : nullptr, profile);
  set_compact(a, map, rf);
  const dim3 grid((unsigned)cdiv(a.n, 256), (unsigned)a.nchunks), block(256);
  const size_t lds = polar_lds_bytes(a.nb, a.group, rf);
  if (int rc = with_polar_kernel<false>(map, rf, a.utab != nullptr, "score", [&](auto kfn) {
        allow_lds(kfn, lds);
        hipLaunchKernelGGL(kfn, grid, block, lds, s, a);
        return TDR_OK;
      }))
    return rc;
  LAUNCH_CHECK("score_polar");
  return TDR_OK;
}

struct tdr_score_ctx {
  int device = 0;
  SpanTuner tuner;
  const float* fac = nullptr;
  int fac_nb = 0, fac_nr = 0;
};
extern "C" int tdr_score_ctx_set_polar_factors(tdr_score_ctx* c, const float* fac_dev, int nb, int nr) {
  if (!c || (fac_dev && (nb < 1 || nr < 1))) return fail(TDR_ERR_ARG, "score_ctx_set_polar_factors: bad arguments");
  c->fac = fac_dev;
  c->fac_nb = fac_dev ? nb : 0;
  c->fac_nr = fac_dev ? nr : 0;
  return TDR_OK;
}
extern "C" int tdr_score_ctx_create(tdr_score_ctx** out) {
  if (!out) return fail(TDR_ERR_ARG, "score_ctx_create: null pointer");
  *out = nullptr;
  tdr_score_ctx* c = new (std::nothrow) tdr_score_ctx;
  if (!c) return fail(TDR_ERR_NOMEM, "score_ctx_create: out of memory");
  const hipError_t e = hipGetDevice(&c->device);
  if (e != hipSuccess) {
    delete c;
    return fail(TDR_ERR_HIP, "score_ctx_create: %s", hipGetErrorString(e));
  }
  *out = c;
  return TDR_OK;
}
extern "C" void tdr_score_ctx_destroy(tdr_score_ctx* c) {
  if (!c) return;
  if (c->tuner.e0) (void)hipEventDestroy(c->tuner.e0);
  if (c->tuner.e1) (void)hipEventDestroy(c->tuner.e1);
  delete c;
}
extern "C" float tdr_score_ctx_span(const tdr_score_ctx* c) {
  return c ? c->tuner.best : tdr_config_shift_uniform_span(-1.f);
}
extern "C" int64_t tdr_score_ctx_trial_calls(const tdr_score_ctx* c) {
  return c ? c->tuner.trial_calls : 0;
}
struct TunerScope {
  tdr_score_ctx* c;
  hipStream_t s;
  TunerScope(tdr_score_ctx* c_, hipStream_t s_) : c(c_), s(s_) {}
  ~TunerScope() {
    if (c) tdr_su_span_end(&c->tuner, s);
  }
};

static bool int_form_applies(const ScoreWs& W, const tdr_map_desc* map, int rf) {
  return W.su && map_has_compact(map, rf) && !map_is_wide(map, rf) && tdr_ray_map_ok(map);
}
bool tdr_score_polar_float_form(const tdr_map_desc* map, int nb, int nr, int64_t n, int64_t n_total) {
  const int rf = tdr_rec_floats(map->ncls);
  return !int_form_applies(score_ws(map->ncls, nb, nr, n, n_total), map, rf);
}
static ScoreArgs make_score_args(const tdr_map_desc* map, const float* tab, const float* scan_pk, int nb, int nr, float res,
                                 const float* st, int64_t cap, int64_t n, const int32_t* order, const ScoreWs& W) {
  ScoreArgs a;
  a.rec = map->rec; a.rows = map->rows; a.cols = map->cols; a.resolution = map->resolution;
  a.tab = tab; a.scan_pk = scan_pk; a.nb = nb; a.nr = nr; a.res = res;
  a.st = st; a.cap = cap; a.n = n; a.order = order;
  a.group = W.group; a.nchunks = W.nchunks; a.npad = W.npad;
  a.part = nullptr;
  return a;
}
static FinalizeArgs make_finalize_args(const tdr_map_desc* map, const tdr_filter_params* fp, const float* part, int nchunks,
                                       int64_t npad, int64_t P, float* st, int64_t cap, int64_t n, const int32_t* order,
                                       float* raw_w) {
  FinalizeArgs f;
  f.part = part; f.rf = map->rec_floats; f.nchunks = nchunks; f.npad = npad; f.n = n; f.cap = cap;
  f.order = order; f.st = st; f.fp = *fp;
  f.gate = make_gate(fp, map);
  f.P = P; f.ncls = map->ncls; f.raw_w = raw_w;
  return f;
}
static void launch_finalize_exact(FinalizeArgs& f, const tdr_map_desc* map, int64_t npad, const int32_t* slots,
                                  const int32_t* counts, const int32_t* inexact, int nchunks_dense, int ray_split,
                                  hipStream_t s) {
  FinalizeArgs fx = f;
  fx.npad = npad; fx.order = slots; fx.counts = counts; fx.inexact = inexact;
  fx.ipart = reinterpret_cast<const uint32_t*>(f.part);
  fx.dict_tail = reinterpret_cast<const uint32_t*>(map->dict) + 2 * TDR_CMAP_MAX_DICT;
  fx.nchunks = nchunks_dense; fx.ray_split = ray_split;
  hipLaunchKernelGGL(score_finalize_exact_kernel, dim3((unsigned)cdiv(npad, 64)), dim3(256), 0, s, fx);
  f.run_if = inexact;
}

namespace {
struct BatchScoreHdr {
  int32_t blocks, max_chunks, fin_blocks, n_uscale;
  int32_t k_init;
  size_t lds;
};
struct UtabEntry {
  float scale, res;
  float* out;
};
struct BatchScoreLayout {
  size_t args, fargs, blk, fblk, utab, total;
};
BatchScoreLayout batch_layout(int k) {
  auto up = [](size_t x) { return (x + 63) / 64 * 64; };
  BatchScoreLayout L;
  L.args = up(sizeof(BatchScoreHdr));
  L.fargs = L.args + up(sizeof(ScoreArgs) * k);
  L.blk = L.fargs + up(sizeof(FinalizeArgs) * k);
  L.fblk = L.blk + up(sizeof(int32_t) * k);
  L.utab = L.fblk + up(sizeof(int32_t) * k);
  L.total = L.utab + up(sizeof(UtabEntry) * k);
  return L;
}
}
__global__ void utab_batch_kernel(const float* __restrict__ tab, int64_t n2, const UtabEntry* __restrict__ ut) {
  const UtabEntry e = ut[blockIdx.y];
  const int64_t k = (int64_t)blockIdx.x * blockDim.x + threadIdx.x;
  if (e.out && k < n2) e.out[k] = (tab[k] * e.scale) * e.res;
}
size_t tdr_batch_score_stage_bytes(int k, int k_init) {
  return k < 1 ? 0 : batch_layout(k).total + tdr_batch_init_stage_bytes(k_init);
}
int tdr_batch_score_build(const tdr_map_desc* map, const float* tab, int nb, int nr, int k, const TdrBatchScoreIn* in,
                          void* host_stage) {
  if (!map || !tab || !in || !host_stage || k < 1 || nb < 1 || nr < 1) return fail(TDR_ERR_ARG, "batch_score: bad arguments");
  const int rf = tdr_rec_floats(map->ncls);
  if (map->rec_floats != rf) return fail(TDR_ERR_ARG, "batch_score: map record size %d != %d", map->rec_floats, rf);
  if ((size_t)2 * nb * rf * 4 > 64 * 1024) return fail(TDR_ERR_ARG, "batch_score: nb too large for the LDS scan ring");
  if (int rc0 = check_map_addressing(map, rf, "batch_score")) return rc0;
  const BatchScoreLayout Lo = batch_layout(k);
  char* base = static_cast<char*>(host_stage);
  BatchScoreHdr& h = *reinterpret_cast<BatchScoreHdr*>(base);
  ScoreArgs* args = reinterpret_cast<ScoreArgs*>(base + Lo.args);
  FinalizeArgs* fargs = reinterpret_cast<FinalizeArgs*>(base + Lo.fargs);
  int32_t* blk = reinterpret_cast<int32_t*>(base + Lo.blk);
  int32_t* fblk = reinterpret_cast<int32_t*>(base + Lo.fblk);
  UtabEntry* ut = reinterpret_cast<UtabEntry*>(base + Lo.utab);
  h = BatchScoreHdr{};
  std::vector<TdrBatchInitIn> iin;
  for (int i = 0; i < k; i++) {
    const TdrBatchScoreIn& x = in[i];
    if (x.n < 1 || x.cap < x.n || !x.fp || x.fp->num_classes != map->ncls) return fail(TDR_ERR_ARG, "batch_score: filter %d", i);
    const ScoreWs W = score_ws(map->ncls, nb, nr, x.n, x.n);
    if (int_form_applies(W, map, rf)) return fail(TDR_ERR_ARG, "batch_score: filter %d takes the integer form", i);
    ScoreArgs a = make_score_args(map, tab, x.scan_pk, nb, nr, x.res, x.st, x.cap, x.n, nullptr, W);
    a.part = x.ws;
    a.utab = x.uniform_scale > 0.f ? x.ws + W.off_utab : nullptr;
    ut[i] = UtabEntry{x.uniform_scale, x.res, const_cast<float*>(a.utab)};
    set_compact(a, map, rf);
    args[i] = a;
    h.lds = std::max(h.lds, polar_lds_bytes(nb, a.group, rf));
    blk[i] = h.blocks;
    h.blocks += (int32_t)cdiv(x.n, 256);
    h.max_chunks = std::max(h.max_chunks, a.nchunks);
    h.n_uscale += a.utab ? 1 : 0;
    FinalizeArgs f = make_finalize_args(map, x.fp, a.part, a.nchunks, a.npad, (int64_t)nb * nr, x.st, x.cap, x.n, nullptr, x.raw_w);
    f.tlog = finalize_tlog(f.nchunks, x.n);
    fargs[i] = f;
    fblk[i] = h.fin_blocks;
    h.fin_blocks += (int32_t)cdiv(x.n << f.tlog, 256);
    if (x.init_search) iin.push_back(TdrBatchInitIn{x.scan_pk, x.res, x.fp, x.st, x.cap, x.n, a.utab, x.ws + W.off_aux, a.npad, x.raw_w});
  }
  h.k_init = (int32_t)iin.size();
  if (h.k_init > 0) return tdr_batch_init_build(map, tab, nb, nr, h.k_init, iin.data(), base + Lo.total);
  return TDR_OK;
}
int tdr_batch_score_launch(const tdr_map_desc* map, const float* tab, int nb, int nr, int k, const void* host_stage,
                           const void* dev_stage, hipStream_t s) {
  if (!map || !tab || !host_stage || !dev_stage || k < 1) return fail(TDR_ERR_ARG, "batch_score: bad arguments");
  const BatchScoreLayout Lo = batch_layout(k);
  const BatchScoreHdr& h = *static_cast<const BatchScoreHdr*>(host_stage);
  const char* d = static_cast<const char*>(dev_stage);
  const ScoreArgs* args = reinterpret_cast<const ScoreArgs*>(d + Lo.args);
  const FinalizeArgs* fargs = reinterpret_cast<const FinalizeArgs*>(d + Lo.fargs);
  const int32_t* blk = reinterpret_cast<const int32_t*>(d + Lo.blk);
  const int32_t* fblk = reinterpret_cast<const int32_t*>(d + Lo.fblk);
  const UtabEntry* ut = reinterpret_cast<const UtabEntry*>(d + Lo.utab);
  const int rf = tdr_rec_floats(map->ncls);
  if (h.n_uscale > 0) {
    const int64_t n2 = 2 * (int64_t)nb * nr;
    hipLaunchKernelGGL(utab_batch_kernel, dim3((unsigned)cdiv(n2, 256), (unsigned)k), dim3(256), 0, s, tab, n2, ut);
    LAUNCH_CHECK("batch_utab");
  }
  if (h.k_init > 0)
    if (int rc = tdr_batch_init_launch(map, nb, nr, static_cast<const char*>(host_stage) + Lo.total, d + Lo.total, s)) return rc;
  const dim3 grid((unsigned)h.blocks, (unsigned)h.max_chunks);
  for (int us = 1; us >= 0; us--) {
    if (us ? h.n_uscale == 0 : h.n_uscale == k) continue;
    if (int rc = with_polar_kernel<true>(map, rf, us != 0, "batch_score", [&](auto kfn) {
          allow_lds(kfn, h.lds);
          hipLaunchKernelGGL(kfn, grid, dim3(256), h.lds, s, args, blk, k);
          return TDR_OK;
        }))
      return rc;
  }
  LAUNCH_CHECK("batch_score_polar");
  hipLaunchKernelGGL(score_finalize_batch_kernel, dim3((unsigned)h.fin_blocks), dim3(256), 0, s, fargs, fblk, k);
  LAUNCH_CHECK("batch_score_finalize");
  if (h.k_init > 0) return tdr_batch_init_fixup(static_cast<const char*>(host_stage) + Lo.total, d + Lo.total, s);
  return TDR_OK;
}
extern "C" int tdr_k_score_polar(const tdr_map_desc* map, const float* tab, const float* scan_pk, int nb, int nr,
                                 float res, const tdr_filter_params* fp, float* st, int64_t cap, int64_t n,
                                 int64_t n_total, const int32_t* perm, float uniform_scale, int init_search,
                                 float* raw_w, float* workspace, void* stream) {
  return tdr_k_score_polar_ctx(map, tab, scan_pk, nb, nr, res, fp, st, cap, n, n_total, perm, uniform_scale, init_search,
                               raw_w, workspace, nullptr, stream);
}
extern "C" int tdr_k_score_polar_ctx(const tdr_map_desc* map, const float* tab, const float* scan_pk, int nb, int nr,
                                     float res, const tdr_filter_params* fp, float* st, int64_t cap, int64_t n,
                                     int64_t n_total, const int32_t* perm, float uniform_scale, int init_search,
                                     float* raw_w, float* workspace, tdr_score_ctx* ctx, void* stream) {
  if (!map || !map->rec || !tab || !scan_pk || !fp || !st || !raw_w || !workspace)
    return fail(TDR_ERR_ARG, "score: null pointer");
  if (n_total <= 0) n_total = n;
  if (n < 0 || cap < n) return fail(TDR_ERR_ARG, "score: n=%lld exceeds capacity %lld", (long long)n, (long long)cap);
  if (n == 0) return TDR_OK;
  if (nb < 1 || nr < 1) return fail(TDR_ERR_ARG, "score: bad image shape");
  if (map->ncls < 1 || map->ncls > TDR_MAX_CLASSES || fp->num_classes != map->ncls)
    return fail(TDR_ERR_ARG, "score: class count mismatch (map %d, params %d)", map->ncls, fp->num_classes);
  const int rf = tdr_rec_floats(map->ncls);
  if (map->rec_floats != rf) return fail(TDR_ERR_ARG, "score: map record size %d != %d", map->rec_floats, rf);
  if ((size_t)2 * nb * rf * 4 > 64 * 1024) return fail(TDR_ERR_ARG, "score: nb too large for the LDS scan ring");
  if (!(map->resolution > 0.f)) return fail(TDR_ERR_ARG, "score: map resolution must be > 0");
  if (int rc0 = check_map_addressing(map, rf, "score")) return rc0;
  hipStream_t s = (hipStream_t)stream;

  const ScoreWs W = score_ws(map->ncls, nb, nr, n, n_total);
  ScoreArgs a = make_score_args(map, tab, scan_pk, nb, nr, res, st, cap, n, perm, W);
  a.part = workspace;
  int rc = fill_utab(a, workspace, W, uniform_scale, s);
  if (rc) return rc;
  float* res_flag = workspace + W.off_aux;
  if (init_search)
    if ((rc = tdr_score_init_search(map, a.tab, a.utab, scan_pk, nb, nr, res, fp, st, cap, n, n_total, perm, res_flag, a.npad, s)))
      return rc;
  FinalizeArgs f = make_finalize_args(map, fp, a.part, a.nchunks, a.npad, (int64_t)nb * nr, st, cap, n, perm, raw_w);
  if (int_form_applies(W, map, rf)) {
    const int32_t* slots = nullptr;
    const int32_t* counts = nullptr;
    SuLaunch L;
    L.map = map; L.tab = a.utab ? a.utab : a.tab; L.uniform_scale = a.utab != nullptr; L.scan_pk = scan_pk;
    L.nb = nb; L.nr = nr; L.rf = rf; L.res = res; L.st = st; L.cap = cap; L.n = n; L.perm = perm;
    L.group = W.su_group; L.nchunks = W.su_nchunks; L.npad = W.npad_part; L.part = a.part;
    L.tail_k = W.su_tail_k; L.tail_q = W.su_tail_q; L.rows = W.su_rows;
    L.fac = ctx && ctx->fac && ctx->fac_nb == nb && ctx->fac_nr == nr ? ctx->fac : nullptr;
    L.uscale = uniform_scale;
    L.wave_span = tdr_su_wave_span();
    L.ray_split = tdr_ray_splits(nb, nr, n, tdr_ray_block_major(L));
    L.ws = reinterpret_cast<int32_t*>(workspace + W.off_su);
    TunerScope tuner_scope(ctx, s);
    L.span = tdr_su_span_begin(ctx ? &ctx->tuner : nullptr,
                               ((int64_t)n << 24) ^ ((int64_t)nb << 12) ^ nr ^ ((int64_t)map->rows << 40), s);
    if ((rc = tdr_su_prepare(L, W.suw, s, &slots, &counts))) return rc;
    if ((rc = tdr_ray_prepare(L, W.suw, s))) return rc;
    const int32_t* inexact = counts + 4;
    {
      ScoreProfScope prof(s);
      {
        ShareProfScope sp(0, s, true);
        if ((rc = tdr_ray_score(L, W.suw, s))) return rc;
      }
      {
        ShareProfScope sp(1, s, true);
        if ((rc = tdr_su_score(L, W.suw, s))) return rc;
      }
      if (g_prof_on) { g_share_valid = true; g_share_counts = counts; }
      ScoreArgs r = a;
      r.run_if = inexact;
      if ((rc = launch_score(r, map, rf, s, false))) return rc;
    }
    launch_finalize_exact(f, map, W.npad_part, slots, counts, inexact, W.su_rows, L.ray_split, s);
    LAUNCH_CHECK("score_finalize_exact");
    launch_finalize(f, n, s);
  } else {
    if ((rc = launch_score(a, map, rf, s))) return rc;
    launch_finalize(f, n, s);
  }
  LAUNCH_CHECK("score_finalize");
  if (init_search) return tdr_score_init_fixup(res_flag, n, fp->regularization, raw_w, s);
  return TDR_OK;
}

__global__ void init_from_best_kernel(const float* __restrict__ best_cost, const float* __restrict__ best_theta,
                                      const int32_t* __restrict__ order, int64_t n, float* __restrict__ st, int64_t cap,
                                      GateArgs gate, float* __restrict__ res_flag) {
  const int64_t slot = (int64_t)blockIdx.x * blockDim.x + threadIdx.x;
  if (slot >= n) return;
  const int64_t p = order ? (int64_t)order[slot] : slot;
  res_flag[p] = 0.f;
  if (st[TDR_ST_HAVE_INIT * cap + p] != 0.f) return;
  const float scale = st[TDR_ST_SCALE * cap + p];
  const float cx = st[TDR_ST_DX * cap + p] * scale + st[TDR_ST_INIT_X * cap + p];
  const float cy = st[TDR_ST_DY * cap + p] * scale + st[TDR_ST_INIT_Y * cap + p];
  if (particle_gated(gate, cx, cy, scale)) return;
  const bool none = !(best_cost[slot] < 3.402823466e+38f);
  st[TDR_ST_THETA * cap + p] = none ? 0.f : best_theta[slot];
  st[TDR_ST_HAVE_INIT * cap + p] = 1.f;
  res_flag[p] = none ? 2.f : 1.f;
}
extern "C" size_t tdr_score_geo_workspace_floats(int ncls, int nb, int nr, int64_t n, int64_t n_total) {
  const int64_t npad = cdiv(std::max<int64_t>(n, 1), 64) * 64;
  const int ggroup = score_group_rings(nb, nr, 4, n_total > 0 ? n_total : n);
  return tdr_score_workspace_floats(ncls, nb, nr, n, n_total) + (size_t)(cdiv(nr, ggroup) * 5 * npad);
}
extern "C" int tdr_k_score_polar_geo(const tdr_map_desc* map, const tdr_map_desc* geo_map, const float* tab,
                                     const float* scan_pk, const float* geo_pk, float geo_sum0, float geo_sum1, int nb,
                                     int nr, float res, const tdr_filter_params* fp, float* st, int64_t cap, int64_t n,
                                     int64_t n_total, const int32_t* perm, float uniform_scale, int init_search,
                                     float* raw_w, float* workspace, void* stream) {
  if (!map || !map->rec || !geo_map || !geo_map->rec || !tab || !scan_pk || !geo_pk || !fp || !st || !raw_w || !workspace)
    return fail(TDR_ERR_ARG, "score_geo: null pointer");
  if (n < 0 || cap < n) return fail(TDR_ERR_ARG, "score_geo: n exceeds capacity");
  if (n == 0) return TDR_OK;
  if (n_total <= 0) n_total = n;
  if (nb < 1 || nr < 1) return fail(TDR_ERR_ARG, "score_geo: bad image shape");
  if (map->ncls < 1 || map->ncls > TDR_MAX_CLASSES || fp->num_classes != map->ncls)
    return fail(TDR_ERR_ARG, "score_geo: class count mismatch");
  if (geo_map->ncls != 2 || geo_map->rec_floats != 4 || geo_map->rows != map->rows || geo_map->cols != map->cols)
    return fail(TDR_ERR_ARG, "score_geo: the geometric map must be the 2-layer map of the same grid");
  const int rf = tdr_rec_floats(map->ncls);
  if (map->rec_floats != rf) return fail(TDR_ERR_ARG, "score_geo: map record size mismatch");
  if ((size_t)nb * rf * 4 > 60 * 1024) return fail(TDR_ERR_ARG, "score_geo: nb too large for the LDS scan ring");
  if (int rc0 = check_map_addressing(map, rf, "score_geo")) return rc0;
  hipStream_t s = (hipStream_t)stream;
  const ScoreWs W = score_ws(map->ncls, nb, nr, n, n_total);
  ScoreArgs a = make_score_args(map, tab, scan_pk, nb, nr, res, st, cap, n, perm, W);
  a.part = workspace;
  int rc = fill_utab(a, workspace, W, uniform_scale, s);
  if (rc) return rc;
  float* best_cost = workspace + W.off_aux;
  float* best_theta = best_cost + a.npad;
  float* res_flag = best_theta + a.npad;
  ScoreArgs g = a;
  g.rec = geo_map->rec; g.scan_pk = geo_pk;
  g.group = score_group_rings(nb, nr, 4, n_total);
  g.nchunks = (int)cdiv(nr, g.group);
  g.part = workspace + tdr_score_workspace_floats(map->ncls, nb, nr, n, n_total);
  FinalizeArgs f = make_finalize_args(map, fp, a.part, a.nchunks, a.npad, (int64_t)nb * nr, st, cap, n, perm, raw_w);
  f.best_cost = best_cost; f.best_theta = best_theta;
  f.gpart = g.part; f.gnchunks = g.nchunks; f.gsum0 = geo_sum0; f.gsum1 = geo_sum1;
  const dim3 fgrid((unsigned)cdiv(n, 256)), fblock(256);
  if (init_search) {
    a.only_uninit = g.only_uninit = 1;
    a.use_theta_override = g.use_theta_override = 1;
    f.mode = 1; f.only_uninit = 1;
    int k = 0;
    for (float t = 0; t < 2 * M_PI; t += 2 * M_PI / 40) {
      a.theta_override = g.theta_override = t;
      if ((rc = launch_score(a, map, rf, s))) return rc;
      if ((rc = launch_score(g, geo_map, 4, s))) return rc;
      f.first = k == 0; f.theta_override = t;
      launch_finalize(f, n, s);
      LAUNCH_CHECK("score_finalize(geo init)");
      k++;
    }
    hipLaunchKernelGGL(init_from_best_kernel, fgrid, fblock, 0, s, (const float*)best_cost, (const float*)best_theta, perm,
                       n, st, cap, f.gate, res_flag);
    LAUNCH_CHECK("init_from_best");
    a.only_uninit = g.only_uninit = 0;
    a.use_theta_override = g.use_theta_override = 0;
  }
  if ((rc = launch_score(a, map, rf, s))) return rc;
  if ((rc = launch_score(g, geo_map, 4, s))) return rc;
  f.mode = 0; f.first = 0; f.theta_override = 0.f; f.only_uninit = 0;
  launch_finalize(f, n, s);
  LAUNCH_CHECK("score_finalize(geo)");
  if (init_search) return tdr_score_init_fixup(res_flag, n, fp->regularization, raw_w, s);
  return TDR_OK;
}

static int64_t cart_part_floats(int ncls, int cols, int64_t n, int64_t n_total) {
  int cpc, nchunks;
  choose_chunks(n_total > 0 ? n_total : n, cols, cpc, nchunks, TDR_CART_WAVE_MUL);
  const int64_t npad = su_npad(std::max<int64_t>(n, 1), 1);
  const int rowsmax = std::max(tdr_rec_floats(ncls) + 1, 2 * ncls + 2);
  return cdiv((int64_t)std::max(nchunks, TDR_RAY_MAX_SPLIT) * rowsmax * npad + 64, 64) * 64;
}
extern "C" size_t tdr_score_cart_workspace_floats(int ncls, int rows, int cols, int64_t n, int64_t n_total) {
  return (size_t)(cart_part_floats(ncls, cols, n, n_total) + tdr_cart_desc_words(rows, cols) +
                  tdr_cart_int_words(rows, cols, std::max<int64_t>(n, 1)));
}

extern "C" int tdr_k_score_cart(const tdr_map_desc* map, const float* scan_pk, int rows, int cols, float res,
                                const tdr_filter_params* fp, float* st, int64_t cap, int64_t n, int64_t n_total,
                                const int32_t* perm, float* raw_w, float* workspace, void* stream) {
  if (!map || !map->rec || !scan_pk || !fp || !st || !raw_w || !workspace)
    return fail(TDR_ERR_ARG, "score_cart: null pointer");
  if (n_total <= 0) n_total = n;
  if (n < 0 || cap < n) return fail(TDR_ERR_ARG, "score_cart: n exceeds capacity");
  if (n == 0) return TDR_OK;
  if (rows < 1 || cols < 1) return fail(TDR_ERR_ARG, "score_cart: bad window shape");
  if (fp->num_classes != map->ncls) return fail(TDR_ERR_ARG, "score_cart: class count mismatch");
  const int rf = tdr_rec_floats(map->ncls);
  if (map->rec_floats != rf) return fail(TDR_ERR_ARG, "score_cart: map record size mismatch");
  if (int rc0 = check_map_addressing(map, rf, "score_cart")) return rc0;
  hipStream_t s = (hipStream_t)stream;
  CartArgs a;
  a.rec = map->rec; a.map_rows = map->rows; a.map_cols = map->cols; a.resolution = map->resolution;
  a.scan_pk = scan_pk; a.rows = rows; a.cols = cols; a.res = res;
  a.st = st; a.cap = cap; a.n = n; a.order = perm;
  choose_chunks(n_total, cols, a.cpc, a.nchunks, TDR_CART_WAVE_MUL);
  a.npad = cdiv(n, 64) * 64;
  a.part = workspace;
  a.libm_fma = tdr_libm_fma();
  dim3 grid((unsigned)cdiv(n, 256), (unsigned)a.nchunks), block(256);
  const bool ks = tdr_has_kslot(map->ncls, rf);
  const bool cm = set_compact(a, map, rf), wide = cm && map_is_wide(map, rf);
  CartIntOut io{};
  bool int_form = false;
  if (cm && !wide && tdr_cart_skip_ok(map, rf)) {
    ScoreProfScope prof(s);
    uint32_t* desc_ws = reinterpret_cast<uint32_t*>(workspace + cart_part_floats(map->ncls, cols, n, n_total));
    if (tdr_cart_int_ok(map, rf, rows, cols, n_total)) {
      int32_t* iws = reinterpret_cast<int32_t*>(desc_ws + tdr_cart_desc_words(rows, cols));
      if (int rc = tdr_cart_int_launch(a, map, rf, desc_ws, iws, 4.f * tdr_config_shift_uniform_span(-1.f), s, &io)) return rc;
      int_form = true;
    } else if (int rc = tdr_cart_skip_launch(a, map, rf, desc_ws, s)) return rc;
  } else {
    ScoreProfScope prof(s);
    if (int rc = with_nv4(rf, "score_cart", [&](auto N) {
          return with_flags([&](auto KS, auto CM, auto WD) {
            constexpr int NV4 = decltype(N)::value;
            constexpr bool c = decltype(CM)::value, w = decltype(WD)::value;
            if constexpr ((c && NV4 == 4) || (w && !(c && NV4 == 2))) return fail(TDR_ERR_ARG, "score_cart: no kernel for this record form");
            else hipLaunchKernelGGL((score_cart_kernel<NV4, TDR_SCORE_U, decltype(KS)::value, c, w>), grid, block, 0, s, a);
            return TDR_OK;
          }, ks, cm, wide);
        }))
      return rc;
  }
  LAUNCH_CHECK("score_cart");
  FinalizeArgs f = make_finalize_args(map, fp, a.part, a.nchunks, a.npad, (int64_t)rows * cols, st, cap, n, perm, raw_w);
  f.gate.force_on_map = 0;
  f.gate.scale_unknown = 0;
  if (int_form) launch_finalize_exact(f, map, io.npad, io.slots, io.counts, io.flags, io.nchunks_dense, io.ray_split, s);
  launch_finalize(f, n, s);
  LAUNCH_CHECK("score_finalize(cart)");
  return TDR_OK;
}

__global__ void selftest_round_kernel(const float* __restrict__ x, int64_t n, float limit, int32_t* __restrict__ out) {
  const int64_t i = (int64_t)blockIdx.x * blockDim.x + threadIdx.x;
  if (i < n) out[i] = round_half_away_clamped(__builtin_amdgcn_fmed3f(x[i], -1.f, limit));
}
extern "C" int tdr_k_selftest_round(const float* x, int64_t n, float limit, int32_t* out, void* stream) {
  if (!x || !out || n < 1) return fail(TDR_ERR_ARG, "selftest_round: bad arguments");
  hipLaunchKernelGGL(selftest_round_kernel, dim3((unsigned)cdiv(n, 256)), dim3(256), 0, (hipStream_t)stream, x, n, limit,
                     out);
  LAUNCH_CHECK("selftest_round");
  return TDR_OK;
}
```

### top_down_renderer_amd/csrc/tdr_score_su.hip

```cpp
#include <rocprim/device/device_radix_sort.hpp>

#include <atomic>

#include "tdr_score_dev.h"
#include "tdr_score_su.h"
#include "tdr_score_su_asm.h"

#define SU_CODE_FULL 0xFFu
#define SU_CODE_FULL_ALL 0xFEu
#define SU_CODE_PAD 0xFDu
#define SU_NSECT TDR_SU_NSECT
#define SU_BOX_WORDS 4096

struct SuArgs {
  const uint32_t* crec;
  const uint32_t* kmask;
  int kcolw;
  unsigned kmask_off;
  const uint32_t* dict_int;
  int dict_n, ctiles_r;
  int pkcol;
  const int32_t* inexact;
  int rows, cols;
  float resolution;
  const float* tab_su;
  const uint32_t* desc;
  const float* bbox;
  const float* scan_pk;
  int nb, nr;
  float res;
  const float* st;
  int64_t cap;
  const int32_t* slots;
  const int32_t* nslots;
  int group, nchunks, ncls;
  int tail_k, tail_q;
  int64_t npad;
  uint32_t* part;
  uint32_t* stats;
};

__global__ __launch_bounds__(256) void su_prep_kernel(const float* __restrict__ tab, const float* __restrict__ scan_pk,
                                                      int nb, int nr, int rf, int ncls, int ckconst, unsigned pbase,
                                                      unsigned plane_bytes, int group, int nchunks,
                                                      const float* __restrict__ dict, int dict_n, float* __restrict__ tab_su,
                                                      uint32_t* __restrict__ desc) {
  const int64_t t = (int64_t)blockIdx.x * blockDim.x + threadIdx.x;
  bool bad = false;
  for (int k = threadIdx.x; k < dict_n; k += blockDim.x) bad |= !(fabsf(dict[k]) <= 3.402823466e+38f);
  const bool dict_bad = __syncthreads_or(bad);
  const int64_t total = (int64_t)nchunks * nb * group;
  const bool live = t < total;
  const int64_t tt = live ? t : 0;
  const int jj = (int)(tt % group);
  const int64_t q = tt / group;
  const int i = (int)(q % nb), chunk = (int)(q / nb);
  const int j = chunk * group + jj;
  float tx = 0.f, ty = 0.f, val = 0.f;
  uint32_t code = SU_CODE_PAD, ckc = (uint32_t)ckconst, sh = 0;
  if (live && j >= nr) {
    const int64_t k = (int64_t)(nr - 1) * nb + i;
    tx = tab[2 * k];
    ty = tab[2 * k + 1];
  }
  if (live && j < nr) {
    code = 0;
    const int64_t k = (int64_t)j * nb + i;
    tx = tab[2 * k];
    ty = tab[2 * k + 1];
    const float* r = scan_pk + k * rf;
    int nz = 0, first = 0;
    bool finite = true;
    for (int c = 0; c < ncls; c++) {
      finite &= fabsf(r[c]) <= 3.402823466e+38f;
      if (r[c] != 0.f) {
        if (!nz) first = c;
        nz++;
      }
    }
    if (dict_bad || !finite) { code = SU_CODE_FULL_ALL; val = r[rf - 1]; }
    else if (nz == 1) { code = (uint32_t)first + 1u; val = r[first]; ckc = pbase + (uint32_t)first * plane_bytes; }
    else if (nz > 1) { code = SU_CODE_FULL; val = r[rf - 1]; }
  }
  uint32_t anyfull = code >= SU_CODE_FULL_ALL ? 1u : 0u;
  anyfull |= __shfl_xor(anyfull, 1);
  anyfull |= __shfl_xor(anyfull, 2);
  if (!live) return;
  tab_su[2 * t] = tx;
  tab_su[2 * t + 1] = ty;
  desc[4 * t] = code;
  desc[4 * t + 1] = (uint32_t)val;
  desc[4 * t + 2] = ckc;
  desc[4 * t + 3] = sh | (((jj & 3) == 0 && anyfull) ? 0x80000000u : 0u);
}

__global__ __launch_bounds__(256) void su_bbox_kernel(const float* __restrict__ tab_su, int nb, int nr, int group,
                                                      float* __restrict__ bbox) {
  const int chunk = blockIdx.x, sect = blockIdx.y;
  const int i0 = (int)((int64_t)sect * nb / SU_NSECT), i1 = (int)((int64_t)(sect + 1) * nb / SU_NSECT);
  const int gn = min(nr - chunk * group, group);
  float lo0 = 3.402823466e+38f, hi0 = -3.402823466e+38f, lo1 = lo0, hi1 = hi0;
  const int cnt = (i1 - i0) * gn;
  for (int t = threadIdx.x; t < cnt; t += 256) {
    const int i = i0 + t / gn, jj = t % gn;
    const float* e = tab_su + (((int64_t)chunk * nb + i) * group + jj) * 2;
    lo0 = fminf(lo0, e[0]); hi0 = fmaxf(hi0, e[0]);
    lo1 = fminf(lo1, e[1]); hi1 = fmaxf(hi1, e[1]);
  }
  __shared__ float red[4][256];
  red[0][threadIdx.x] = lo0; red[1][threadIdx.x] = hi0; red[2][threadIdx.x] = lo1; red[3][threadIdx.x] = hi1;
  __syncthreads();
  for (int d = 128; d > 0; d >>= 1) {
    if ((int)threadIdx.x < d) {
      red[0][threadIdx.x] = fminf(red[0][threadIdx.x], red[0][threadIdx.x + d]);
      red[1][threadIdx.x] = fmaxf(red[1][threadIdx.x], red[1][threadIdx.x + d]);
      red[2][threadIdx.x] = fminf(red[2][threadIdx.x], red[2][threadIdx.x + d]);
      red[3][threadIdx.x] = fmaxf(red[3][threadIdx.x], red[3][threadIdx.x + d]);
    }
    __syncthreads();
  }
  if (threadIdx.x < 4) bbox[((int64_t)chunk * SU_NSECT + sect) * 4 + threadIdx.x] = red[threadIdx.x][0];
}

__global__ __launch_bounds__(256) void su_key_kernel(const float* __restrict__ st, int64_t cap, int64_t n,
                                                     const int32_t* __restrict__ perm, int nb, float span, int per_block,
                                                     uint32_t* __restrict__ keys, int32_t* __restrict__ vals,
                                                     int* __restrict__ cnt, int* __restrict__ seg_hist) {
  extern __shared__ int hist[];
  for (int k = threadIdx.x; k <= nb; k += 256) hist[k] = 0;
  __syncthreads();
  for (int it = 0; it < per_block; it += 256) {
    const int64_t t = (int64_t)blockIdx.x * per_block + it + threadIdx.x;
    if (t >= n) break;
    const int32_t p = perm ? perm[t] : (int32_t)t;
    uint32_t key = (uint32_t)rot_shift_dev(st[TDR_ST_THETA * cap + p], nb);
    if (span > 0.f) {
      auto centre = [&](int64_t q, float& x, float& y) {
        const float sc = st[TDR_ST_SCALE * cap + q];
        x = st[TDR_ST_DX * cap + q] * sc + st[TDR_ST_INIT_X * cap + q];
        y = st[TDR_ST_DY * cap + q] * sc + st[TDR_ST_INIT_Y * cap + q];
      };
      const int64_t ta = t >= 32 ? t - 32 : 0, tb = t + 32 < n ? t + 32 : n - 1;
      float x0, y0, x1, y1;
      centre(perm ? perm[ta] : ta, x0, y0);
      centre(perm ? perm[tb] : tb, x1, y1);
      if (!(fabsf(x1 - x0) <= span && fabsf(y1 - y0) <= span)) key = (uint32_t)nb;
    }
    keys[t] = key;
    vals[t] = p;
    atomicAdd(&hist[key], 1);
  }
  __syncthreads();
  if (seg_hist) {
    int* row = seg_hist + (int64_t)blockIdx.x * (nb + 1);
    for (int k = threadIdx.x; k <= nb; k += 256) row[k] = hist[k];
  } else {
    for (int k = threadIdx.x; k <= nb; k += 256)
      if (hist[k]) atomicAdd(&cnt[k], hist[k]);
  }
}

#define SU_SEG 512
#define SU_COLSCAN_WAVES 16
__global__ __launch_bounds__(64 * SU_COLSCAN_WAVES) void su_colscan_kernel(int* __restrict__ seg_hist, int segs, int nkeys,
                                                                           int* __restrict__ cnt) {
  __shared__ int wsum[SU_COLSCAN_WAVES][64];
  const int lane = threadIdx.x & 63, w = threadIdx.x >> 6;
  const int k = blockIdx.x * 64 + lane;
  const bool live = k < nkeys;
  const int per = (segs + SU_COLSCAN_WAVES - 1) / SU_COLSCAN_WAVES;
  const int s0 = min(w * per, segs), s1 = min(s0 + per, segs);
  int* col = seg_hist + (live ? k : 0);
  int sum = 0;
  if (live)
    for (int sgm = s0; sgm < s1; sgm += 8) {
      int v[8];
#pragma unroll
      for (int u = 0; u < 8; u++) v[u] = sgm + u < s1 ? col[(int64_t)(sgm + u) * nkeys] : 0;
#pragma unroll
      for (int u = 0; u < 8; u++) sum += v[u];
    }
  wsum[w][lane] = sum;
  __syncthreads();
  int run = 0, tot = 0;
#pragma unroll
  for (int j = 0; j < SU_COLSCAN_WAVES; j++) {
    const int v = wsum[j][lane];
    run += j < w ? v : 0;
    tot += v;
  }
  if (!live) return;
  if (w == 0) cnt[k] = tot;
  for (int sgm = s0; sgm < s1; sgm += 8) {
    int v[8];
#pragma unroll
    for (int u = 0; u < 8; u++) v[u] = sgm + u < s1 ? col[(int64_t)(sgm + u) * nkeys] : 0;
#pragma unroll
    for (int u = 0; u < 8; u++) {
      if (sgm + u < s1) col[(int64_t)(sgm + u) * nkeys] = run;
      run += v[u];
    }
  }
}

__global__ __launch_bounds__(256) void su_offsets_kernel(const int* __restrict__ cnt, int nkeys, int* __restrict__ start,
                                                         int* __restrict__ slot_start, int* __restrict__ counts,
                                                         int32_t* __restrict__ pad_slots) {
  __shared__ int sa[256], sb[256];
  int carry_a = 0, carry_b = 0;
  for (int base = 0; base < nkeys; base += 256) {
    const int k = base + threadIdx.x;
    const int c = k < nkeys ? cnt[k] : 0;
    const int cp = k < nkeys - 1 ? (c + 63) & ~63 : c;
    sa[threadIdx.x] = c;
    sb[threadIdx.x] = cp;
    __syncthreads();
    for (int d = 1; d < 256; d <<= 1) {
      const int va = threadIdx.x >= d ? sa[threadIdx.x - d] : 0;
      const int vb = threadIdx.x >= d ? sb[threadIdx.x - d] : 0;
      __syncthreads();
      sa[threadIdx.x] += va;
      sb[threadIdx.x] += vb;
      __syncthreads();
    }
    if (k < nkeys) {
      start[k] = carry_a + sa[threadIdx.x] - c;
      slot_start[k] = carry_b + sb[threadIdx.x] - cp;
      if (pad_slots)
        for (int j = c; j < cp; j++) pad_slots[carry_b + sb[threadIdx.x] - cp + j] = -1;
    }
    carry_a += sa[255];
    carry_b += sb[255];
    __syncthreads();
  }
  if (threadIdx.x == 0) {
    const int sparse = cnt[nkeys - 1];
    counts[0] = carry_b - sparse;
    counts[1] = sparse;
    counts[2] = carry_b;
  }
  if (pad_slots && threadIdx.x >= 3 && threadIdx.x < TDR_SU_TAIL_INTS) counts[threadIdx.x] = 0;
}

__global__ __launch_bounds__(256) void su_scatter_kernel(const uint32_t* __restrict__ keys, const int32_t* __restrict__ vals,
                                                         int64_t n, const int* __restrict__ start,
                                                         const int* __restrict__ slot_start, int32_t* __restrict__ slots) {
  const int64_t t = (int64_t)blockIdx.x * blockDim.x + threadIdx.x;
  if (t >= n) return;
  const uint32_t k = keys[t];
  slots[slot_start[k] + ((int)t - start[k])] = vals[t];
}

__global__ __launch_bounds__(64) void su_rank_scatter_kernel(const uint32_t* __restrict__ keys, const int32_t* __restrict__ vals,
                                                             int64_t n, const int* __restrict__ seg_pre,
                                                             const int* __restrict__ slot_start, int nkeys, int bits,
                                                             int32_t* __restrict__ slots) {
  extern __shared__ int ctr[];
  const int lane = threadIdx.x;
  const int64_t t0 = (int64_t)blockIdx.x * SU_SEG;
  uint32_t key[SU_SEG / 64];
  int32_t val[SU_SEG / 64];
#pragma unroll
  for (int it = 0; it < SU_SEG / 64; it++) {
    const int64_t t = t0 + it * 64 + lane;
    key[it] = t < n ? keys[t] : 0u;
    val[it] = t < n ? vals[t] : 0;
  }
  const int* row = seg_pre + (int64_t)blockIdx.x * nkeys;
  for (int k0 = lane; k0 < nkeys; k0 += 256) {
    int a[4], b[4];
#pragma unroll
    for (int u = 0; u < 4; u++) {
      const int k = k0 + 64 * u;
      a[u] = k < nkeys ? slot_start[k] : 0;
      b[u] = k < nkeys ? row[k] : 0;
    }
#pragma unroll
    for (int u = 0; u < 4; u++)
      if (k0 + 64 * u < nkeys) ctr[k0 + 64 * u] = a[u] + b[u];
  }
  __syncthreads();
#pragma unroll
  for (int it = 0; it < SU_SEG / 64; it++) {
    const bool live = t0 + it * 64 + lane < n;
    uint64_t same = __ballot(live);
    for (int b = 0; b < bits; b++) {
      const bool one = (key[it] >> b) & 1u;
      const uint64_t ones = __ballot(one);
      same &= one ? ones : ~ones;
    }
    const int below = __popcll(same & (((uint64_t)1 << lane) - 1)), all = __popcll(same);
    int at = 0;
    if (live) {
      at = ctr[key[it]];
      slots[at + below] = val[it];
    }
    __syncthreads();
    if (live && below == all - 1) ctr[key[it]] = at + all;
    __syncthreads();
  }
}

__global__ __launch_bounds__(256) void su_wave_far_kernel(const float* __restrict__ st, int64_t cap, const int32_t* __restrict__ slots,
                                                          const int32_t* __restrict__ counts, float wave_span,
                                                          int32_t* __restrict__ keep, int32_t* __restrict__ moved) {
  const int lane = threadIdx.x & 63;
  const int64_t w = (int64_t)blockIdx.x * 4 + (threadIdx.x >> 6), base = w * 64;
  if (base >= (int64_t)counts[0]) return;
  const int32_t p = slots[base + lane];
  float x0 = 3.0e38f, x1 = -3.0e38f, y0 = 3.0e38f, y1 = -3.0e38f;
  if (p >= 0) {
    const float sc = st[TDR_ST_SCALE * cap + p];
    const float x = st[TDR_ST_DX * cap + p] * sc + st[TDR_ST_INIT_X * cap + p];
    const float y = st[TDR_ST_DY * cap + p] * sc + st[TDR_ST_INIT_Y * cap + p];
    x0 = x1 = x;
    y0 = y1 = y;
  }
#pragma unroll
  for (int d = 32; d > 0; d >>= 1) {
    x0 = fminf(x0, __shfl_xor(x0, d)); x1 = fmaxf(x1, __shfl_xor(x1, d));
    y0 = fminf(y0, __shfl_xor(y0, d)); y1 = fmaxf(y1, __shfl_xor(y1, d));
  }
  const int nvalid = __popcll(__ballot(p >= 0));
  const bool far = (x1 - x0 > wave_span) || (y1 - y0 > wave_span);
  if (lane == 0) {
    keep[w] = far ? 0 : 1;
    moved[w] = far ? nvalid : 0;
  }
}
__global__ __launch_bounds__(256) void su_compact_offsets_kernel(int32_t* __restrict__ keep, int32_t* __restrict__ moved,
                                                                 int32_t* __restrict__ counts, int32_t* __restrict__ old_counts) {
  __shared__ int sa[256], sb[256];
  const int c0 = counts[0], c1 = counts[1], c2 = counts[2];
  const int nw = c0 >> 6;
  int carry_a = 0, carry_b = 0;
  for (int base = 0; base < nw; base += 256) {
    const int w = base + threadIdx.x;
    const int a = w < nw ? keep[w] : 0, b = w < nw ? moved[w] : 0;
    sa[threadIdx.x] = a;
    sb[threadIdx.x] = b;
    __syncthreads();
    for (int d = 1; d < 256; d <<= 1) {
      const int va = threadIdx.x >= d ? sa[threadIdx.x - d] : 0;
      const int vb = threadIdx.x >= d ? sb[threadIdx.x - d] : 0;
      __syncthreads();
      sa[threadIdx.x] += va;
      sb[threadIdx.x] += vb;
      __syncthreads();
    }
    if (w < nw) {
      keep[w] = a ? (carry_a + sa[threadIdx.x] - a) * 64 : -1;
      moved[w] = carry_b + sb[threadIdx.x] - b;
    }
    carry_a += sa[255];
    carry_b += sb[255];
    __syncthreads();
  }
  if (threadIdx.x == 0) {
    old_counts[0] = c0; old_counts[1] = c1; old_counts[2] = c2;
    counts[0] = carry_a * 64;
    counts[1] = c1 + carry_b;
    counts[2] = carry_a * 64 + c1 + carry_b;
  }
}
__global__ __launch_bounds__(256) void su_compact_scatter_kernel(const int32_t* __restrict__ slots, const int32_t* __restrict__ keep,
                                                                 const int32_t* __restrict__ moved,
                                                                 const int32_t* __restrict__ counts,
                                                                 const int32_t* __restrict__ old_counts, int32_t* __restrict__ out) {
  const int64_t t = (int64_t)blockIdx.x * blockDim.x + threadIdx.x;
  const int oc0 = old_counts[0], oc1 = old_counts[1];
  if (t >= (int64_t)oc0 + oc1) return;
  const int32_t p = slots[t];
  if (t >= oc0) {
    out[(int64_t)counts[0] + (t - oc0)] = p;
    return;
  }
  const int64_t w = t >> 6;
  const int32_t k = keep[w];
  const uint64_t valid = __ballot(p >= 0);
  if (k >= 0) {
    out[(int64_t)k + (t & 63)] = p;
  } else if (p >= 0) {
    const int rank = __popcll(valid & (((uint64_t)1 << (t & 63)) - 1));
    out[(int64_t)counts[0] + oc1 + moved[w] + rank] = p;
  }
}
__global__ void su_copy_slots_kernel(const int32_t* __restrict__ src, const int32_t* __restrict__ counts, int32_t* __restrict__ dst) {
  const int64_t t = (int64_t)blockIdx.x * blockDim.x + threadIdx.x;
  if (t < (int64_t)counts[2]) dst[t] = src[t];
}

struct SuLds {
  uint32_t dict[TDR_CMAP_MAX_DICT];
  uint32_t bits[SU_BOX_WORDS];
// ... 494 lines not shown
}
namespace {
constexpr float kSpanCand[] = {2.f, 8.f, 16.f, 24.f, 40.f};
constexpr int kSpanCands = (int)(sizeof(kSpanCand) / sizeof(kSpanCand[0]));
constexpr int kSpanTrials = 2;
constexpr int kSpanSkip = 30;
constexpr int kSpanRetune = 4000;
}
float tdr_su_span_begin(SpanTuner* t, int64_t shape, hipStream_t s) {
  if (g_su_span_fixed || !t) return g_su_span;
  if (!t->e0 && (hipEventCreate(&t->e0) != hipSuccess || hipEventCreate(&t->e1) != hipSuccess)) return g_su_span;
  if (shape != t->shape) { t->shape = shape; t->phase = -kSpanSkip; t->trial = 0; t->best_ms = 3.0e38f; t->pending = false; t->best = t->round_best = g_su_span; }
  if (t->pending) {
    if (hipEventQuery(t->e1) != hipSuccess) return t->best;
    float ms = 0.f;
    if (hipEventElapsedTime(&ms, t->e0, t->e1) == hipSuccess && ms > 0.f && ms < t->best_ms) {
      t->best_ms = ms;
      t->round_best = kSpanCand[t->phase];
    }
    t->pending = false;
    if (++t->trial >= kSpanTrials) { t->trial = 0; t->phase++; }
    if (t->phase >= kSpanCands) { t->settled_launches = 0; t->best = t->round_best; }
  }
  if (t->phase < 0) { t->phase++; return t->best; }
  if (t->phase >= kSpanCands) {
    if (++t->settled_launches < kSpanRetune) return t->best;
    t->phase = 0;
    t->best_ms = 3.0e38f;
    t->round_best = t->best;
  }
  t->open = hipEventRecord(t->e0, s) == hipSuccess;
  t->trial_calls++;
  return kSpanCand[t->phase];
}
void tdr_su_span_end(SpanTuner* t, hipStream_t s) {
  if (g_su_span_fixed || !t || !t->open) return;
  t->open = false;
  t->pending = hipEventRecord(t->e1, s) == hipSuccess;
}
static float g_su_wave_span = 0.f;
extern "C" int tdr_config_su_wave_span(int cells) {
  if (cells >= 0) g_su_wave_span = (float)cells;
  return (int)g_su_wave_span;
}
float tdr_su_wave_span() { return g_su_wave_span; }
static int g_su_lds_pad = 0;
extern "C" int tdr_config_su_lds_pad(int bytes) {
  if (bytes >= 0) g_su_lds_pad = bytes;
  return g_su_lds_pad;
}
static std::atomic<int64_t> g_su_launches{0};
extern "C" int64_t tdr_shift_uniform_launches(void) { return g_su_launches.load(); }
bool tdr_su_shape_ok(int nb, int nr, int group, int64_t n_total) {
  if (g_su_mode == 0) return false;
  if (group % 4 != 0 || nb > 4095) return false;
  if (g_su_mode == 2) return true;
  if ((int64_t)nb * nr < 8192) return false;
  return n_total >= (int64_t)64 * nb;
}
static int g_su_tail_groups = 4, g_su_tail_parts = 4;
extern "C" int tdr_config_su_tail_groups(int k) {
  if (k >= 0) g_su_tail_groups = k;
  return g_su_tail_groups;
}
extern "C" int tdr_config_su_tail_parts(int q) {
  if (q >= 0) g_su_tail_parts = q >= 8 ? 8 : (q >= 4 ? 4 : (q >= 2 ? 2 : 1));
  return g_su_tail_parts;
}
void tdr_su_tail(int nchunks, int64_t n, int* k, int* q) {
  *k = std::min(g_su_tail_groups, nchunks);
  *q = g_su_tail_parts;
  if (g_su_mode != 2 && cdiv(std::max<int64_t>(n, 1), 256) * nchunks < 2 * 256 * 6) *k = 0;
  if (*k == 0 || *q == 1) { *k = 0; *q = 1; }
}
extern "C" int tdr_su_tail_plan(int nchunks, int k, int q, int row, int* group, int* s0, int* s1) {
  int g = 0, a = 0, b = 0;
  const int rows = su_tail_plan(nchunks, k, q, row, &g, &a, &b);
  if (row >= 0 && row < rows) {
    if (group) *group = g;
    if (s0) *s0 = a;
    if (s1) *s1 = b;
  }
  return rows;
}
static int g_su_order_bucket = 1;
extern "C" int tdr_config_su_order_bucket(int v) {
  if (v >= 0) g_su_order_bucket = v ? 1 : 0;
  return g_su_order_bucket;
}
static int64_t su_seg_table_words(int nb, int64_t n) {
  const int64_t words = cdiv(std::max<int64_t>(n, 1), SU_SEG) * ((int64_t)nb + 1);
  return words <= 4 * std::max<int64_t>(n, 1) + 65536 ? words : 0;
}
static int64_t su_seg_table_reserve(int nb, int64_t n) {
  const int64_t m = std::max<int64_t>(n, 1);
  return std::min<int64_t>(cdiv(m, SU_SEG) * ((int64_t)nb + 1), 4 * m + 65536);
}
static bool su_order_is_bucket(int nb, int64_t n) { return g_su_order_bucket && su_seg_table_words(nb, n) > 0; }
static size_t su_sort_tmp_bytes(int64_t n) {
  size_t bytes = 0;
  uint32_t* k = nullptr;
  int32_t* v = nullptr;
  hipError_t e = rocprim::radix_sort_pairs(nullptr, bytes, k, k, v, v, (size_t)std::max<int64_t>(n, 1), 0u, 12u,
                                           (hipStream_t)0, false);
  if (e != hipSuccess || bytes == 0) bytes = (size_t)(n + 4096) * 16;
  return bytes;
}
SuWs tdr_su_ws(int nb, int nr, int group, int64_t n) {
  SuWs w;
  const int64_t nchunks = cdiv(nr, group), nbins = nchunks * nb * group;
  int64_t o = 0;
  auto take = [&](int64_t words) { const int64_t at = o; o += (words + 63) / 64 * 64; return at; };
  w.tab_su = take(2 * nbins);
  w.desc = take(4 * nbins);
  w.bbox = take(nchunks * SU_NSECT * 4);
  w.keys_in = take(n);
  w.keys_out = take(n);
  w.vals_in = take(n);
  w.vals_out = take(n);
  w.ints = take(3 * ((int64_t)nb + 1) + TDR_SU_TAIL_INTS);
  w.slots = take(su_npad(n, nb));
  w.slots2 = take(su_npad(n, nb));
  w.wave_tmp = take(2 * (su_npad(n, nb) / 64 + 1));
  w.sort_tmp = take((int64_t)((su_sort_tmp_bytes(n) + 3) / 4));
  const int64_t T = tdr_ray_padded_samples(nb, nr);
  w.ray_tab = take(2 * T);
  w.ray_desc = take((T + 1) / 2);
  w.ray_multi = take((int64_t)nb * nr);
  w.ray_rad = take(T / nb);
  w.seg_hist = take(su_seg_table_reserve(nb, n));
  w.total = o;
  return w;
}

int tdr_su_order(const SuLaunch& L, const SuWs& W, hipStream_t s, const int32_t** slots_out, const int32_t** counts_out) {
  int32_t* base = L.ws;
  uint32_t* keys_in = reinterpret_cast<uint32_t*>(base + W.keys_in);
  uint32_t* keys_out = reinterpret_cast<uint32_t*>(base + W.keys_out);
  int32_t* vals_in = base + W.vals_in;
  int32_t* vals_out = base + W.vals_out;
  int* cnt = base + W.ints;
  const int nkeys = L.nb + 1;
  int* start = cnt + nkeys;
  int* slot_start = start + nkeys;
  int* counts = slot_start + nkeys;
  int32_t* slots = base + W.slots;
  const int64_t n = L.n;
  if (su_order_is_bucket(L.nb, n)) {
    int* seg_hist = base + W.seg_hist;
    const int64_t segs = cdiv(n, SU_SEG);
    hipLaunchKernelGGL(su_key_kernel, dim3((unsigned)segs), dim3(256), sizeof(int) * (size_t)nkeys, s, L.st, L.cap, n, L.perm,
                       L.nb, L.span, SU_SEG, keys_in, vals_in, (int*)nullptr, seg_hist);
    LAUNCH_CHECK("su_key");
    hipLaunchKernelGGL(su_colscan_kernel, dim3((unsigned)cdiv(nkeys, 64)), dim3(64 * SU_COLSCAN_WAVES), 0, s, seg_hist,
                       (int)segs, nkeys, cnt);
    LAUNCH_CHECK("su_colscan");
    hipLaunchKernelGGL(su_offsets_kernel, dim3(1), dim3(256), 0, s, (const int*)cnt, nkeys, start, slot_start, counts, slots);
    LAUNCH_CHECK("su_offsets");
    unsigned bits = 1;
    while ((1u << bits) < (unsigned)nkeys) bits++;
    hipLaunchKernelGGL(su_rank_scatter_kernel, dim3((unsigned)segs), dim3(64), sizeof(int) * (size_t)nkeys, s,
                       (const uint32_t*)keys_in, (const int32_t*)vals_in, n, (const int*)seg_hist, (const int*)slot_start, nkeys,
                       (int)bits, slots);
    LAUNCH_CHECK("su_rank_scatter");
  } else {
    HIP_TRY(hipMemsetAsync(cnt, 0, sizeof(int) * (size_t)(3 * nkeys + TDR_SU_TAIL_INTS), s));
    HIP_TRY(hipMemsetAsync(slots, 0xFF, sizeof(int32_t) * (size_t)L.npad, s));
    hipLaunchKernelGGL(su_key_kernel, dim3((unsigned)cdiv(n, 256)), dim3(256), sizeof(int) * (size_t)nkeys, s, L.st, L.cap, n,
                       L.perm, L.nb, L.span, 256, keys_in, vals_in, cnt, (int*)nullptr);
    LAUNCH_CHECK("su_key");
    hipLaunchKernelGGL(su_offsets_kernel, dim3(1), dim3(256), 0, s, (const int*)cnt, nkeys, start, slot_start, counts,
                       (int32_t*)nullptr);
    LAUNCH_CHECK("su_offsets");
    unsigned bits = 1;
    while ((1u << bits) < (unsigned)nkeys) bits++;
    size_t tmp_bytes = su_sort_tmp_bytes(n);
    HIP_TRY(rocprim::radix_sort_pairs(base + W.sort_tmp, tmp_bytes, keys_in, keys_out, vals_in, vals_out, (size_t)n, 0u, bits,
                                      s, false));
    hipLaunchKernelGGL(su_scatter_kernel, dim3((unsigned)cdiv(n, 256)), dim3(256), 0, s, (const uint32_t*)keys_out,
                       (const int32_t*)vals_out, n, (const int*)start, (const int*)slot_start, slots);
    LAUNCH_CHECK("su_scatter");
  }
  if (L.wave_span > 0.f && L.nb > 1) {
    int32_t* slots2 = base + W.slots2;
    int32_t* keep = base + W.wave_tmp;
    int32_t* moved = keep + (L.npad / 64 + 1);
    int32_t* old_counts = counts + 7;
    const int64_t nwaves = L.npad / 64;
    hipLaunchKernelGGL(su_wave_far_kernel, dim3((unsigned)cdiv(nwaves, 4)), dim3(256), 0, s, L.st, L.cap, (const int32_t*)slots,
                       (const int32_t*)counts, L.wave_span, keep, moved);
    hipLaunchKernelGGL(su_compact_offsets_kernel, dim3(1), dim3(256), 0, s, keep, moved, counts, old_counts);
    hipLaunchKernelGGL(su_compact_scatter_kernel, dim3((unsigned)cdiv(L.npad, 256)), dim3(256), 0, s, (const int32_t*)slots,
                       (const int32_t*)keep, (const int32_t*)moved, (const int32_t*)counts, (const int32_t*)old_counts, slots2);
    hipLaunchKernelGGL(su_copy_slots_kernel, dim3((unsigned)cdiv(L.npad, 256)), dim3(256), 0, s, (const int32_t*)slots2,
                       (const int32_t*)counts, slots);
    LAUNCH_CHECK("su_reroute");
  }
  *slots_out = slots;
  *counts_out = counts;
  return TDR_OK;
}
extern "C" size_t tdr_k_su_order_workspace_ints(int64_t n, int nb) {
  if (n < 1 || nb < 1 || nb > 4095) return 0;
  return (size_t)tdr_su_ws(nb, 4, 4, n).total;
}
extern "C" int64_t tdr_k_su_order_slots(int64_t n, int nb) { return n < 1 || nb < 1 ? 0 : su_npad(n, nb); }
extern "C" int tdr_k_su_order(const float* st, int64_t cap, int64_t n, const int32_t* perm, int nb, float span,
                              int32_t* workspace, int32_t* slots_out, int32_t* keys_out, int32_t* counts_out, int* bucket_out,
                              void* stream) {
  if (!st || !workspace || !slots_out || !keys_out || !counts_out) return fail(TDR_ERR_ARG, "su_order: null pointer");
  if (n < 1 || cap < n || nb < 1 || nb > 4095) return fail(TDR_ERR_ARG, "su_order: bad shape");
  hipStream_t s = (hipStream_t)stream;
  const SuWs W = tdr_su_ws(nb, 4, 4, n);
  SuLaunch L{};
  L.st = st; L.cap = cap; L.n = n; L.perm = perm; L.nb = nb; L.span = span; L.ws = workspace;
  L.npad = su_npad(n, nb);
  const int32_t* slots = nullptr;
  const int32_t* counts = nullptr;
  if (bucket_out) *bucket_out = su_order_is_bucket(nb, n) ? 1 : 0;
  if (int rc = tdr_su_order(L, W, s, &slots, &counts)) return rc;
  HIP_TRY(hipMemcpyAsync(slots_out, slots, sizeof(int32_t) * (size_t)L.npad, hipMemcpyDeviceToDevice, s));
  HIP_TRY(hipMemcpyAsync(keys_out, workspace + W.keys_in, sizeof(int32_t) * (size_t)n, hipMemcpyDeviceToDevice, s));
  HIP_TRY(hipMemcpyAsync(counts_out, counts, sizeof(int32_t) * 3, hipMemcpyDeviceToDevice, s));
  return TDR_OK;
}
int tdr_su_prepare(const SuLaunch& L, const SuWs& W, hipStream_t s, const int32_t** slots_out, const int32_t** counts_out) {
  if (int rc = tdr_su_order(L, W, s, slots_out, counts_out)) return rc;
  int32_t* base = L.ws;
  float* tab_su = reinterpret_cast<float*>(base + W.tab_su);
  uint32_t* desc = reinterpret_cast<uint32_t*>(base + W.desc);
  const int64_t ndesc = (int64_t)L.nchunks * L.nb * L.group;
  const int lc = L.map->cwords == 1 ? 3 : (L.map->cwords == 2 ? 2 : 1);
  const int ckconst = ((L.map->rows >> lc) + 2) * 128 + 128;
  const unsigned plane_bytes = (unsigned)(tdr_cmap_plane_words(L.map->ncls, L.map->rows, L.map->cols) * 4);
  const unsigned pbase = (unsigned)(tdr_cmap_plane_offset_words(L.map->ncls, L.map->rows, L.map->cols) * 4) +
                         (unsigned)(plane_trows(L.map->rows) * 128) + 128u;
  hipLaunchKernelGGL(su_prep_kernel, dim3((unsigned)cdiv(ndesc, 256)), dim3(256), 0, s, L.tab, L.scan_pk, L.nb, L.nr, L.rf,
                     L.map->ncls, ckconst, pbase, plane_bytes, L.group, L.nchunks, L.map->dict, L.map->dict_n, tab_su, desc);
  LAUNCH_CHECK("su_prep");
  hipLaunchKernelGGL(su_bbox_kernel, dim3((unsigned)L.nchunks, SU_NSECT), dim3(256), 0, s, (const float*)tab_su, L.nb, L.nr,
                     L.group, reinterpret_cast<float*>(base + W.bbox));
  LAUNCH_CHECK("su_bbox");
  return TDR_OK;
}

int tdr_su_score(const SuLaunch& L, const SuWs& W, hipStream_t s) {
  const tdr_map_desc* map = L.map;
  int32_t* base = L.ws;
  int* nslots = base + W.ints + 3 * (L.nb + 1);
  SuArgs u;
  const int lc = map->cwords == 1 ? 3 : (map->cwords == 2 ? 2 : 1);
  u.crec = map->crec; u.dict_int = reinterpret_cast<const uint32_t*>(map->dict) + TDR_CMAP_MAX_DICT;
  u.dict_n = map->dict_n; u.ctiles_r = (map->rows >> lc) + 2;
  u.pkcol = plane_trows(map->rows) * 128 - 16;
  u.inexact = nslots + 4;
  u.rows = map->rows; u.cols = map->cols; u.resolution = map->resolution;
  u.tab_su = reinterpret_cast<const float*>(base + W.tab_su);
  u.desc = reinterpret_cast<const uint32_t*>(base + W.desc);
  u.bbox = reinterpret_cast<const float*>(base + W.bbox);
  u.kmask = map->crec + tdr_cmap_tile_words(map->ncls, map->rows, map->cols);
  u.kcolw = kmask_trows(map->rows) * 32;
  u.kmask_off = (unsigned)(tdr_cmap_tile_words(map->ncls, map->rows, map->cols) * 4);
  u.scan_pk = L.scan_pk;
  u.nb = L.nb; u.nr = L.nr; u.res = L.res; u.st = L.st; u.cap = L.cap;
  u.slots = base + W.slots; u.nslots = nslots;
  u.group = L.group; u.nchunks = L.nchunks; u.tail_k = L.tail_k; u.tail_q = L.tail_q; u.ncls = map->ncls; u.npad = L.npad; u.part = reinterpret_cast<uint32_t*>(L.part);
  u.stats = tdr_profile_stats_ptr();
  int rg, r0, r1;
  const int rows = su_tail_plan(L.nchunks, L.tail_k, L.tail_q, -1, &rg, &r0, &r1);
  if (L.rows != rows) return fail(TDR_ERR_ARG, "score: %d rows of partial sums for a plan of %d", L.rows, rows);
  const dim3 grid((unsigned)cdiv(L.npad, 256), (unsigned)rows), block(256);
  const bool ks = tdr_has_kslot(map->ncls, L.rf), us = L.uniform_scale;
#define TDR_LAUNCH_SU(NV4)                                                                         \
  if (ks && us) hipLaunchKernelGGL((score_polar_su_kernel<NV4, true, true>), grid, block, g_su_lds_pad, s, u);  \
  else if (ks) hipLaunchKernelGGL((score_polar_su_kernel<NV4, true, false>), grid, block, g_su_lds_pad, s, u);  \
  else if (us) hipLaunchKernelGGL((score_polar_su_kernel<NV4, false, true>), grid, block, g_su_lds_pad, s, u);  \
  else hipLaunchKernelGGL((score_polar_su_kernel<NV4, false, false>), grid, block, g_su_lds_pad, s, u);
  switch (L.rf / 4) {
    case 1: TDR_LAUNCH_SU(1) break;
    case 2: TDR_LAUNCH_SU(2) break;
    case 3: TDR_LAUNCH_SU(3) break;
    default: return fail(TDR_ERR_ARG, "score: no shift-uniform kernel for record size %d", L.rf);
  }
#undef TDR_LAUNCH_SU
  LAUNCH_CHECK("score_polar_su");
  g_su_launches.fetch_add(1);
  return TDR_OK;
}
```

Before: 23.48 million.

## Fold weight-update count passes into chain sums and fuse several small scoring kernels

```diff
diff --git a/top_down_renderer_amd/csrc/tdr_common.h b/top_down_renderer_amd/csrc/tdr_common.h
--- a/top_down_renderer_amd/csrc/tdr_common.h
+++ b/top_down_renderer_amd/csrc/tdr_common.h
@@ -64,7 +64,7 @@
 }
 
 int tdr_chain_total(const float* raw, const float* mean_dev, int kind, int64_t n, float* total_out, void* workspace,
-                    hipStream_t st);
+                    hipStream_t st, long long* count_out = nullptr, float* mean_out = nullptr);
 int tdr_uw_small(const float* raw, const float* last_dist, int64_t n, float* w, float* info, hipStream_t st);
 int tdr_mt_raw_stream(const uint32_t* state, int64_t nblocks, uint32_t* raw, hipStream_t s);
 int tdr_mt_advance(const uint32_t* raw, int64_t nblocks, const uint32_t* consumed, uint32_t* state, hipStream_t s);
diff --git a/top_down_renderer_amd/csrc/tdr_filter.hip b/top_down_renderer_amd/csrc/tdr_filter.hip
--- a/top_down_renderer_amd/csrc/tdr_filter.hip
+++ b/top_down_renderer_amd/csrc/tdr_filter.hip
@@ -204,6 +204,7 @@
 }
 struct UwExact {
   float sum, mean, bsum, pad;
+  long long nvalid, nunder;
 };
 __global__ __launch_bounds__(256) void uw_pass2(const float* __restrict__ raw, int64_t n, const UwScratch* s1,
                                                 UwScratch* s2, UwExact* ex) {
@@ -226,7 +227,7 @@
                                                 const UwScratch* s2, UwScratch* s3, float* __restrict__ w) {
   __shared__ double shd[4];
   const float sum = ex->sum, mean = ex->mean;
-  const long long num_under = (long long)uw_total(s2->b);
+  const long long num_under = s2 ? (long long)uw_total(s2->b) : ex->nunder;
   const float bottom = sqrtf(ex->bsum / (float)num_under);
   const bool fallback = (sum == 0.f || num_under < 1);
   const float fill = mean - bottom;
@@ -302,7 +303,13 @@
   }
   if ((threadIdx.x & 63) == 0) { sb[threadIdx.x >> 6] = best; si[threadIdx.x >> 6] = besti; }
   const float sum = ex->sum, mean = ex->mean;
-  const long long nv = (long long)uw_total(s1->b), nu = (long long)uw_total(s2->b);
+  long long nv, nu;
+  if (s1) {
+    nv = (long long)uw_total(s1->b); nu = (long long)uw_total(s2->b);
+  } else {
+    nv = ex->nvalid; nu = ex->nunder;
+    __syncthreads();
+  }
   const float bottom = sqrtf(ex->bsum / (float)nu);
   if (threadIdx.x != 0) return;
   for (int k = 1; k < 4; k++)
@@ -313,6 +320,11 @@
   info[5] = (float)nv; info[6] = (float)nu; info[7] = 0.f;
 }
 
+static int g_uw_fold_counts = 1;
+extern "C" int tdr_config_uw_fold_counts(int on) {
+  if (on >= 0) g_uw_fold_counts = on ? 1 : 0;
+  return g_uw_fold_counts;
+}
 #define TDR_UW_SINGLE_MAX_N 32768
 extern "C" int tdr_k_update_weights(const float* raw_w, const float* last_dist, int64_t n, float* w_out,
                                     float* info_out, void* stream) {
@@ -334,18 +346,20 @@
   const size_t chain_room = TDR_UW_INFO_FLOATS * sizeof(float) - kFixed;
   if ((size_t)tdr_prefix_workspace_bytes(n) > chain_room)
     return fail(TDR_ERR_ARG, "update_weights: n = %lld needs more than TDR_UW_INFO_FLOATS of scratch", (long long)n);
-  hipLaunchKernelGGL(uw_pass1, dim3(UW_G), dim3(256), 0, s, raw_w, n, sc + 0);
-  int rc = tdr_chain_total(raw_w, nullptr, 0, n, &ex->sum, chain_ws, s);
+  const bool fold = g_uw_fold_counts != 0;
+  const UwScratch* const c1 = fold ? nullptr : sc + 0;
+  const UwScratch* const c2 = fold ? nullptr : sc + 1;
+  if (!fold) hipLaunchKernelGGL(uw_pass1, dim3(UW_G), dim3(256), 0, s, raw_w, n, sc + 0);
+  int rc = tdr_chain_total(raw_w, nullptr, 0, n, &ex->sum, chain_ws, s, fold ? &ex->nvalid : nullptr,
+                           fold ? &ex->mean : nullptr);
   if (rc) return rc;
-  hipLaunchKernelGGL(uw_pass2, dim3(UW_G), dim3(256), 0, s, raw_w, n, (const UwScratch*)(sc + 0), sc + 1, ex);
-  rc = tdr_chain_total(raw_w, &ex->mean, 1, n, &ex->bsum, chain_ws, s);
+  if (!fold) hipLaunchKernelGGL(uw_pass2, dim3(UW_G), dim3(256), 0, s, raw_w, n, c1, sc + 1, ex);
+  rc = tdr_chain_total(raw_w, &ex->mean, 1, n, &ex->bsum, chain_ws, s, fold ? &ex->nunder : nullptr);
   if (rc) return rc;
-  hipLaunchKernelGGL(uw_pass3, dim3(UW_G), dim3(256), 0, s, raw_w, n, (const UwExact*)ex, (const UwScratch*)(sc + 1),
-                     sc + 2, w_out);
+  hipLaunchKernelGGL(uw_pass3, dim3(UW_G), dim3(256), 0, s, raw_w, n, (const UwExact*)ex, c2, sc + 2, w_out);
   hipLaunchKernelGGL(uw_pass4, dim3(UW_G), dim3(256), 0, s, last_dist, n, (const UwScratch*)(sc + 2), sc + 3, w_out);
   hipLaunchKernelGGL(uw_pass5, dim3(UW_G), dim3(256), 0, s, n, (const UwScratch*)(sc + 3), sc + 4, w_out);
-  hipLaunchKernelGGL(uw_pass6, dim3(1), dim3(256), 0, s, n, (const UwScratch*)(sc + 0), (const UwScratch*)(sc + 1),
-                     (const UwScratch*)(sc + 4), (const UwExact*)ex, info_out);
+  hipLaunchKernelGGL(uw_pass6, dim3(1), dim3(256), 0, s, n, c1, c2, (const UwScratch*)(sc + 4), (const UwExact*)ex, info_out);
   LAUNCH_CHECK("update_weights(multi)");
   return TDR_OK;
 }
diff --git a/top_down_renderer_amd/csrc/tdr_prefix.hip b/top_down_renderer_amd/csrc/tdr_prefix.hip
--- a/top_down_renderer_amd/csrc/tdr_prefix.hip
+++ b/top_down_renderer_amd/csrc/tdr_prefix.hip
@@ -1068,8 +1068,28 @@
   int kind;
 };
 __device__ __forceinline__ ChainStat chain_stat(const ChainSrc& s) { return {{s.raw}, s.kind, s.kind ? *s.mean : 0.f}; }
+template <bool COUNT>
 __global__ __launch_bounds__(PFXW_THREADS) void chain_sum_kernel(ChainSrc s, int64_t n, PfxChunk* __restrict__ ch) {
-  chain_sum_body<PFXW_THREADS, CHAIN_K>(chain_stat(s), n, ch);
+  const ChainStat a = chain_stat(s);
+  chain_sum_body<PFXW_THREADS, CHAIN_K>(a, n, ch);
+  if constexpr (COUNT) {
+    __shared__ int s_cnt;
+    const long long lo = (long long)blockIdx.x * PFXM_CHUNK;
+    const int cnt = (int)min((long long)PFXM_CHUNK, (long long)n - lo), t0 = threadIdx.x * CHAIN_K;
+    if (threadIdx.x == 0) s_cnt = 0;
+    int c = 0;
+#pragma unroll
+    for (int k = 0; k < CHAIN_K; k++) {
+      const float v = a.src.read(lo + t0 + k, t0 + k < cnt);
+      c += (t0 + k < cnt && v == v && (a.kind == CHAIN_SUM || v < a.mean)) ? 1 : 0;
+    }
+#pragma unroll
+    for (int o = 32; o >= 1; o >>= 1) c += __shfl_xor(c, o, 64);
+    pfx_sync();
+    if ((threadIdx.x & 63) == 0) atomicAdd(&s_cnt, c);
+    pfx_sync();
+    if (threadIdx.x == 0) ch[blockIdx.x].accepted = s_cnt;
+  }
 }
 __global__ __launch_bounds__(PFXW_THREADS) void chain_summary_kernel(ChainSrc s, int64_t n, PfxChunk* __restrict__ ch,
                                                                     int c_first) {
@@ -1088,15 +1108,34 @@
 }
 __global__ __launch_bounds__(PFXW_THREADS) void chain_walk_kernel(ChainSrc s, int64_t n, const PfxChunk* __restrict__ ch,
                                                                  int nch, float* __restrict__ total_out, int c_first,
-                                                                 const float* __restrict__ r_first) {
+                                                                 const float* __restrict__ r_first,
+                                                                 long long* __restrict__ count_out,
+                                                                 float* __restrict__ mean_out) {
   const ChainStat a = chain_stat(s);
+  __shared__ long long s_count[PFXW_THREADS / 64];
+  if (count_out) {
+    long long c = 0;
+    for (int j = threadIdx.x; j < nch; j += PFXW_THREADS) c += ch[j].accepted;
+#pragma unroll
+    for (int o = 32; o >= 1; o >>= 1) c += __shfl_xor(c, o, 64);
+    if ((threadIdx.x & 63) == 0) s_count[threadIdx.x >> 6] = c;
+  }
   const int hn = c_first > 0 ? 0 : (int)min((long long)CHAIN_HEAD, (long long)n);
   float r = chain_head_serial<PFXW_THREADS>(a, hn, c_first > 0 ? *r_first : 0.f), carry = 0.f;
   chain_walk_chunks<false>(ch, nch, c_first, r, carry, [&](int c) {
     const long long lo = (long long)c * PFXM_CHUNK;
     chain_walk_chunk(a, lo, (int)min((long long)PFXM_CHUNK, (long long)n - lo), r, c == 0 ? hn : 0);
   });
-  if (threadIdx.x == 0) *total_out = r;
+  pfx_sync();
+  if (threadIdx.x == 0) {
+    *total_out = r;
+    if (count_out) {
+      long long c = 0;
+      for (int w = 0; w < PFXW_THREADS / 64; w++) c += s_count[w];
+      *count_out = c;
+      if (mean_out) *mean_out = r / (float)c;
+    }
+  }
 }
 static int g_pfx_small = 1;
 extern "C" int tdr_config_prefix_small(int on) {
@@ -1107,14 +1146,15 @@
 static int chain_head_chunks(int64_t n) { return (g_pfx_small && n >= CHAIN_HEAD_N) ? CHAIN_HEAD_N / PFXM_CHUNK : 0; }
 static int chain_head_launch(const float* raw, const float* mean_dev, int kind, int n_head, float* r_out, hipStream_t st);
 int tdr_chain_total(const float* raw, const float* mean_dev, int kind, int64_t n, float* total_out, void* workspace,
-                    hipStream_t st) {
+                    hipStream_t st, long long* count_out, float* mean_out) {
   const int64_t nch64 = cdiv(n, (int64_t)PFXM_CHUNK);
   if (nch64 > (1 << 24)) return fail(TDR_ERR_ARG, "chain_total: n too large");
   const int nch = (int)nch64;
   PfxChunk* ch = reinterpret_cast<PfxChunk*>(workspace);
   ChainSrc s{raw, mean_dev, kind};
   const int c_first = chain_head_chunks(n);
-  hipLaunchKernelGGL(chain_sum_kernel, dim3(nch), dim3(PFXW_THREADS), 0, st, s, n, ch);
+  if (count_out) hipLaunchKernelGGL(chain_sum_kernel<true>, dim3(nch), dim3(PFXW_THREADS), 0, st, s, n, ch);
+  else hipLaunchKernelGGL(chain_sum_kernel<false>, dim3(nch), dim3(PFXW_THREADS), 0, st, s, n, ch);
   if (nch > c_first)
     hipLaunchKernelGGL(chain_summary_kernel, dim3(nch - c_first), dim3(PFXW_THREADS), 0, st, s, n, ch, c_first);
   float* r_first = reinterpret_cast<float*>(&ch[0].r0);
@@ -1123,7 +1163,7 @@
     if (rc) return rc;
   }
   hipLaunchKernelGGL(chain_walk_kernel, dim3(1), dim3(PFXW_THREADS), 0, st, s, n, (const PfxChunk*)ch, nch, total_out,
-                     c_first, (const float*)r_first);
+                     c_first, (const float*)r_first, count_out, count_out ? mean_out : nullptr);
   return TDR_OK;
 }
 
diff --git a/top_down_renderer_amd/csrc/tdr_score.hip b/top_down_renderer_amd/csrc/tdr_score.hip
--- a/top_down_renderer_amd/csrc/tdr_score.hip
+++ b/top_down_renderer_amd/csrc/tdr_score.hip
@@ -230,6 +230,22 @@
   const unsigned bx = blockIdx.x;
 #endif
   score_polar_body<NV4, U, KSLOT, USCALE, COMPACT, WIDE>(a, bx, blockIdx.y);
+}
+#define TDR_SCORE_UNITS_GRID 2048
+template <int NV4, int U, bool KSLOT, bool USCALE>
+__global__ __launch_bounds__(256, 5) void score_polar_units_kernel(ScoreArgs a, unsigned nbx, unsigned nby) {
+  if (!int_form_off(a.run_if)) return;
+  const uint64_t units = (uint64_t)nbx * nby;
+  for (uint64_t u = blockIdx.x; u < units; u += gridDim.x) {
+    const unsigned x = (unsigned)(u % nbx), by = (unsigned)(u / nbx);
+#if TDR_XCD_SWIZZLE
+    const unsigned bx = nbx % 8 != 0 ? x : (x % 8) * ((nbx + 7) / 8) + x / 8;
+#else
+    const unsigned bx = x;
+#endif
+    score_polar_body<NV4, U, KSLOT, USCALE, true, false>(a, bx, by);
+    __syncthreads();
+  }
 }
 template <int NV4, int U, bool KSLOT, bool USCALE, bool COMPACT, bool WIDE = false>
 __global__ __launch_bounds__(256, COMPACT ? (WIDE ? 3 : 5) : 1) void score_polar_batch_kernel(const ScoreArgs* __restrict__ args,
@@ -459,6 +475,7 @@
   int ray_split = 1;
 };
 
+template <int NCMAX = TDR_MAX_CLASSES, int FIN_B = 4>
 __device__ __forceinline__ void score_finalize_body(const FinalizeArgs& a, const int64_t gid) {
   const int T = 1 << a.tlog, t = (int)(gid & (T - 1));
   const int64_t slot = gid >> a.tlog;
@@ -475,7 +492,7 @@
     return;
   }
   if (a.mode == 1 && a.only_uninit && a.st[TDR_ST_HAVE_INIT * a.cap + p] != 0.f) return;
-  constexpr int FIN_B = 4, FIN_S = TDR_MAX_CLASSES + 2;
+  constexpr int FIN_S = NCMAX + 2;
   double tot[FIN_S];
 #pragma unroll
   for (int k = 0; k < FIN_S; k++) tot[k] = 0;
@@ -520,7 +537,7 @@
   } else {
     cost = 0.f;
 #pragma unroll
-    for (int k = 0; k < TDR_MAX_CLASSES; k++)
+    for (int k = 0; k < NCMAX; k++)
       if (k < a.ncls) cost = (float)((double)cost + (double)(float)tot[k] * 0.01 * (double)a.fp.class_weights[k]);
     float normf = (float)norm;
     if (a.gpart) {
@@ -557,22 +574,22 @@
   score_finalize_body(a, (int64_t)(blockIdx.x - (unsigned)blk[e]) * blockDim.x + threadIdx.x);
 }
 
-__global__ __launch_bounds__(256) void score_finalize_exact_kernel(FinalizeArgs a) {
-  __shared__ unsigned long long red[3][TDR_MAX_CLASSES + 2][64];
-  if (int_form_off(a.inexact)) return;
+template <int NCMAX>
+__device__ __forceinline__ void score_finalize_exact_body(const FinalizeArgs& a, const unsigned bx) {
+  __shared__ unsigned long long red[3][NCMAX + 2][64];
   const int lane = threadIdx.x & 63, t = threadIdx.x >> 6;
   const int64_t nslots = (int64_t)a.counts[2];
-  if ((int64_t)blockIdx.x * 64 >= nslots) return;
-  const int64_t slot = min((int64_t)blockIdx.x * 64 + lane, nslots - 1);
+  if ((int64_t)bx * 64 >= nslots) return;
+  const int64_t slot = min((int64_t)bx * 64 + lane, nslots - 1);
   const int rows = 2 * a.ncls + 2;
   const int nch = slot < (int64_t)a.counts[0] ? a.nchunks : a.ray_split;
-  unsigned long long tot[TDR_MAX_CLASSES], norm = 0, known = 0;
-#pragma unroll
-  for (int k = 0; k < TDR_MAX_CLASSES; k++) tot[k] = 0;
+  unsigned long long tot[NCMAX], norm = 0, known = 0;
+#pragma unroll
+  for (int k = 0; k < NCMAX; k++) tot[k] = 0;
   for (int c = t; c < nch; c += 4) {
     const uint32_t* o = a.ipart + (int64_t)c * rows * a.npad + slot;
 #pragma unroll
-    for (int k = 0; k < TDR_MAX_CLASSES; k++)
+    for (int k = 0; k < NCMAX; k++)
       if (k < a.ncls)
         tot[k] += (unsigned long long)o[(int64_t)(2 * k) * a.npad] | ((unsigned long long)o[(int64_t)(2 * k + 1) * a.npad] << 32);
     norm += o[(int64_t)(2 * a.ncls) * a.npad];
@@ -580,19 +597,19 @@
   }
   if (t > 0) {
 #pragma unroll
-    for (int k = 0; k < TDR_MAX_CLASSES; k++)
+    for (int k = 0; k < NCMAX; k++)
       if (k < a.ncls) red[t - 1][k][lane] = tot[k];
-    red[t - 1][TDR_MAX_CLASSES][lane] = norm;
-    red[t - 1][TDR_MAX_CLASSES + 1][lane] = known;
+    red[t - 1][NCMAX][lane] = norm;
+    red[t - 1][NCMAX + 1][lane] = known;
   }
   __syncthreads();
-  if (t > 0 || (int64_t)blockIdx.x * 64 + lane >= nslots) return;
+  if (t > 0 || (int64_t)bx * 64 + lane >= nslots) return;
   for (int u = 0; u < 3; u++) {
 #pragma unroll
-    for (int k = 0; k < TDR_MAX_CLASSES; k++)
+    for (int k = 0; k < NCMAX; k++)
       if (k < a.ncls) tot[k] += red[u][k][lane];
-    norm += red[u][TDR_MAX_CLASSES][lane];
-    known += red[u][TDR_MAX_CLASSES + 1][lane];
+    norm += red[u][NCMAX][lane];
+    known += red[u][NCMAX + 1][lane];
   }
   const int64_t p = a.order[slot];
   if (p < 0) return;
@@ -610,7 +627,7 @@
     const int q = (int)a.dict_tail[0];
     cost = 0.f;
 #pragma unroll
-    for (int k = 0; k < TDR_MAX_CLASSES; k++)
+    for (int k = 0; k < NCMAX; k++)
       if (k < a.ncls) {
         const float dot = (float)ldexp((double)tot[k], -q);
         cost = (float)((double)cost + (double)dot * 0.01 * (double)a.fp.class_weights[k]);
@@ -618,6 +635,11 @@
     cost = cost / (float)norm;
   }
   a.raw_w[p] = (float)(1. / (double)(cost + a.fp.regularization));
+}
+template <int NV4>
+__global__ __launch_bounds__(256) void score_finalize_both_kernel(FinalizeArgs fx, FinalizeArgs f) {
+  if (int_form_off(fx.inexact)) score_finalize_body<4 * NV4 - 1, 2>(f, (int64_t)blockIdx.x * blockDim.x + threadIdx.x);
+  else score_finalize_exact_body<4 * NV4 - 1>(fx, blockIdx.x);
 }
 
 static int finalize_tlog(int nchunks, int64_t nslots) {
@@ -648,6 +670,7 @@
 extern "C" int tdr_config_su_tail_groups(int);
 extern "C" int tdr_config_su_tail_parts(int);
 extern "C" int tdr_config_su_order_bucket(int);
+extern "C" int tdr_config_uw_fold_counts(int);
 extern "C" int tdr_config_init_device(int);
 extern "C" int64_t tdr_config_init_window_words(int64_t);
 extern "C" int64_t tdr_config_cart_init_chunk(int64_t);
@@ -670,6 +693,7 @@
   if (n == "su_tail_parts") return tdr_config_su_tail_parts((int)std::min<int64_t>(std::max<int64_t>(value, -1), 8));
   if (n == "su_order_bucket") return tdr_config_su_order_bucket((int)std::max<int64_t>(value, -1));
   if (n == "su_wave_span") return tdr_config_su_wave_span((int)std::max<int64_t>(value, -1));
+  if (n == "uw_fold_counts") return tdr_config_uw_fold_counts((int)std::max<int64_t>(value, -1));
   if (n == "init_device") return tdr_config_init_device((int)std::max<int64_t>(value, -1));
   if (n == "init_window_words") return tdr_config_init_window_words(value > 0 ? value : -1);
   if (n == "cart_init_chunk") return tdr_config_cart_init_chunk(value > 0 ? value : -1);
@@ -930,6 +954,27 @@
   LAUNCH_CHECK("score_polar");
   return TDR_OK;
 }
+static int launch_score_fallback(ScoreArgs a, const tdr_map_desc* map, int rf, hipStream_t s) {
+  set_compact(a, map, rf);
+  const unsigned nbx = (unsigned)cdiv(a.n, 256), nby = (unsigned)a.nchunks;
+  const dim3 grid((unsigned)std::min<uint64_t>((uint64_t)nbx * nby, TDR_SCORE_UNITS_GRID)), block(256);
+  const size_t lds = polar_lds_bytes(a.nb, a.group, rf);
+  if (int rc = with_nv4(rf, "score", [&](auto N) {
+        return with_flags([&](auto KS, auto US) {
+          constexpr int NV4 = decltype(N)::value;
+          if constexpr (NV4 == 4) return fail(TDR_ERR_ARG, "score: no kernel for this record form");
+          else {
+            auto kfn = score_polar_units_kernel<NV4, TDR_SCORE_U, decltype(KS)::value, decltype(US)::value>;
+            allow_lds(kfn, lds);
+            hipLaunchKernelGGL(kfn, grid, block, lds, s, a, nbx, nby);
+            return TDR_OK;
+          }
+        }, tdr_has_kslot(map->ncls, rf), a.utab != nullptr);
+      }))
+    return rc;
+  LAUNCH_CHECK("score_polar_units");
+  return TDR_OK;
+}
 
 struct tdr_score_ctx {
   int device = 0;
@@ -1007,14 +1052,20 @@
 }
 static void launch_finalize_exact(FinalizeArgs& f, const tdr_map_desc* map, int64_t npad, const int32_t* slots,
                                   const int32_t* counts, const int32_t* inexact, int nchunks_dense, int ray_split,
-                                  hipStream_t s) {
+                                  int64_t n_float, hipStream_t s) {
   FinalizeArgs fx = f;
   fx.npad = npad; fx.order = slots; fx.counts = counts; fx.inexact = inexact;
   fx.ipart = reinterpret_cast<const uint32_t*>(f.part);
   fx.dict_tail = reinterpret_cast<const uint32_t*>(map->dict) + 2 * TDR_CMAP_MAX_DICT;
   fx.nchunks = nchunks_dense; fx.ray_split = ray_split;
-  hipLaunchKernelGGL(score_finalize_exact_kernel, dim3((unsigned)cdiv(npad, 64)), dim3(256), 0, s, fx);
   f.run_if = inexact;
+  f.tlog = finalize_tlog(f.nchunks, n_float);
+  const dim3 grid((unsigned)std::max<int64_t>(cdiv(npad, 64), cdiv(n_float << f.tlog, 256))), block(256);
+  switch (tdr_rec_floats(map->ncls) / 4) {
+    case 1: hipLaunchKernelGGL(score_finalize_both_kernel<1>, grid, block, 0, s, fx, f); break;
+    case 2: hipLaunchKernelGGL(score_finalize_both_kernel<2>, grid, block, 0, s, fx, f); break;
+    default: hipLaunchKernelGGL(score_finalize_both_kernel<3>, grid, block, 0, s, fx, f); break;
+  }
 }
 
 namespace {
@@ -1197,11 +1248,9 @@
       if (g_prof_on) { g_share_valid = true; g_share_counts = counts; }
       ScoreArgs r = a;
       r.run_if = inexact;
-      if ((rc = launch_score(r, map, rf, s, false))) return rc;
+      if ((rc = launch_score_fallback(r, map, rf, s))) return rc;
     }
-    launch_finalize_exact(f, map, W.npad_part, slots, counts, inexact, W.su_rows, L.ray_split, s);
-    LAUNCH_CHECK("score_finalize_exact");
-    launch_finalize(f, n, s);
+    launch_finalize_exact(f, map, W.npad_part, slots, counts, inexact, W.su_rows, L.ray_split, n, s);
   } else {
     if ((rc = launch_score(a, map, rf, s))) return rc;
     launch_finalize(f, n, s);
@@ -1363,8 +1412,8 @@
   FinalizeArgs f = make_finalize_args(map, fp, a.part, a.nchunks, a.npad, (int64_t)rows * cols, st, cap, n, perm, raw_w);
   f.gate.force_on_map = 0;
   f.gate.scale_unknown = 0;
-  if (int_form) launch_finalize_exact(f, map, io.npad, io.slots, io.counts, io.flags, io.nchunks_dense, io.ray_split, s);
-  launch_finalize(f, n, s);
+  if (int_form) launch_finalize_exact(f, map, io.npad, io.slots, io.counts, io.flags, io.nchunks_dense, io.ray_split, n, s);
+  else launch_finalize(f, n, s);
   LAUNCH_CHECK("score_finalize(cart)");
   return TDR_OK;
 }
diff --git a/top_down_renderer_amd/csrc/tdr_score_su.hip b/top_down_renderer_amd/csrc/tdr_score_su.hip
--- a/top_down_renderer_amd/csrc/tdr_score_su.hip
+++ b/top_down_renderer_amd/csrc/tdr_score_su.hip
@@ -161,51 +161,9 @@
 }
 
 #define SU_SEG 512
-#define SU_COLSCAN_WAVES 16
-__global__ __launch_bounds__(64 * SU_COLSCAN_WAVES) void su_colscan_kernel(int* __restrict__ seg_hist, int segs, int nkeys,
-                                                                           int* __restrict__ cnt) {
-  __shared__ int wsum[SU_COLSCAN_WAVES][64];
-  const int lane = threadIdx.x & 63, w = threadIdx.x >> 6;
-  const int k = blockIdx.x * 64 + lane;
-  const bool live = k < nkeys;
-  const int per = (segs + SU_COLSCAN_WAVES - 1) / SU_COLSCAN_WAVES;
-  const int s0 = min(w * per, segs), s1 = min(s0 + per, segs);
-  int* col = seg_hist + (live ? k : 0);
-  int sum = 0;
-  if (live)
-    for (int sgm = s0; sgm < s1; sgm += 8) {
-      int v[8];
-#pragma unroll
-      for (int u = 0; u < 8; u++) v[u] = sgm + u < s1 ? col[(int64_t)(sgm + u) * nkeys] : 0;
-#pragma unroll
-      for (int u = 0; u < 8; u++) sum += v[u];
-    }
-  wsum[w][lane] = sum;
-  __syncthreads();
-  int run = 0, tot = 0;
-#pragma unroll
-  for (int j = 0; j < SU_COLSCAN_WAVES; j++) {
-    const int v = wsum[j][lane];
-    run += j < w ? v : 0;
-    tot += v;
-  }
-  if (!live) return;
-  if (w == 0) cnt[k] = tot;
-  for (int sgm = s0; sgm < s1; sgm += 8) {
-    int v[8];
-#pragma unroll
-    for (int u = 0; u < 8; u++) v[u] = sgm + u < s1 ? col[(int64_t)(sgm + u) * nkeys] : 0;
-#pragma unroll
-    for (int u = 0; u < 8; u++) {
-      if (sgm + u < s1) col[(int64_t)(sgm + u) * nkeys] = run;
-      run += v[u];
-    }
-  }
-}
 
 __global__ __launch_bounds__(256) void su_offsets_kernel(const int* __restrict__ cnt, int nkeys, int* __restrict__ start,
-                                                         int* __restrict__ slot_start, int* __restrict__ counts,
-                                                         int32_t* __restrict__ pad_slots) {
+                                                         int* __restrict__ slot_start, int* __restrict__ counts) {
   __shared__ int sa[256], sb[256];
   int carry_a = 0, carry_b = 0;
   for (int base = 0; base < nkeys; base += 256) {
@@ -226,8 +184,6 @@
     if (k < nkeys) {
       start[k] = carry_a + sa[threadIdx.x] - c;
       slot_start[k] = carry_b + sb[threadIdx.x] - cp;
-      if (pad_slots)
-        for (int j = c; j < cp; j++) pad_slots[carry_b + sb[threadIdx.x] - cp + j] = -1;
     }
     carry_a += sa[255];
     carry_b += sb[255];
@@ -239,7 +195,107 @@
     counts[1] = sparse;
     counts[2] = carry_b;
   }
-  if (pad_slots && threadIdx.x >= 3 && threadIdx.x < TDR_SU_TAIL_INTS) counts[threadIdx.x] = 0;
+}
+
+#define SU_CO_WAVES 16
+#define SU_CO_FLIGHT 16
+__global__ __launch_bounds__(64 * SU_CO_WAVES) void su_colscan_offsets_kernel(int* __restrict__ seg_hist, int segs, int nkeys,
+                                                                              int* __restrict__ cnt, int* __restrict__ start,
+                                                                              int* __restrict__ slot_start, int* __restrict__ counts,
+                                                                              int32_t* __restrict__ pad_slots) {
+  __shared__ int wsum[64][64];
+  __shared__ int lcnt[4096];
+  __shared__ int wa[SU_CO_WAVES], wb[SU_CO_WAVES];
+  const int lane = threadIdx.x & 63, w = threadIdx.x >> 6;
+  const int kblocks = (nkeys + 63) / 64;
+  const int shares = kblocks >= SU_CO_WAVES ? 1 : SU_CO_WAVES / kblocks;
+  const int tasks = kblocks * shares;
+  const int per = (segs + shares - 1) / shares;
+  auto range = [&](int task, int& k, int& s0, int& s1) {
+    const int kb = task / shares, sh = task - kb * shares;
+    k = kb * 64 + lane;
+    s0 = min(sh * per, segs);
+    s1 = min(s0 + per, segs);
+  };
+  for (int task = w; task < tasks; task += SU_CO_WAVES) {
+    int k, s0, s1;
+    range(task, k, s0, s1);
+    int sum = 0;
+    if (k < nkeys) {
+      const int* col = seg_hist + k;
+      for (int sgm = s0; sgm < s1; sgm += SU_CO_FLIGHT) {
+        int v[SU_CO_FLIGHT];
+#pragma unroll
+        for (int u = 0; u < SU_CO_FLIGHT; u++) v[u] = sgm + u < s1 ? col[(int64_t)(sgm + u) * nkeys] : 0;
+#pragma unroll
+        for (int u = 0; u < SU_CO_FLIGHT; u++) sum += v[u];
+      }
+    }
+    wsum[task][lane] = sum;
+  }
+  __syncthreads();
+  for (int task = w; task < tasks; task += SU_CO_WAVES) {
+    int k, s0, s1;
+    range(task, k, s0, s1);
+    const int kb = task / shares, sh = task - kb * shares;
+    int run = 0, tot = 0;
+    for (int j = 0; j < shares; j++) {
+      const int v = wsum[kb * shares + j][lane];
+      run += j < sh ? v : 0;
+      tot += v;
+    }
+    if (k >= nkeys) continue;
+    if (sh == 0) { cnt[k] = tot; lcnt[k] = tot; }
+    int* col = seg_hist + k;
+    for (int sgm = s0; sgm < s1; sgm += SU_CO_FLIGHT) {
+      int v[SU_CO_FLIGHT];
+#pragma unroll
+      for (int u = 0; u < SU_CO_FLIGHT; u++) v[u] = sgm + u < s1 ? col[(int64_t)(sgm + u) * nkeys] : 0;
+#pragma unroll
+      for (int u = 0; u < SU_CO_FLIGHT; u++) {
+        if (sgm + u < s1) col[(int64_t)(sgm + u) * nkeys] = run;
+        run += v[u];
+      }
+    }
+  }
+  __syncthreads();
+  int carry_a = 0, carry_b = 0;
+  for (int base = 0; base < nkeys; base += 64 * SU_CO_WAVES) {
+    const int k = base + threadIdx.x;
+    const int c = k < nkeys ? lcnt[k] : 0;
+    const int cp = k < nkeys - 1 ? (c + 63) & ~63 : c;
+    int ia = c, ib = cp;
+#pragma unroll
+    for (int d = 1; d < 64; d <<= 1) {
+      const int va = __shfl_up(ia, d, 64), vb = __shfl_up(ib, d, 64);
+      if (lane >= d) { ia += va; ib += vb; }
+    }
+    if (lane == 63) { wa[w] = ia; wb[w] = ib; }
+    __syncthreads();
+    int ba = 0, bb = 0, ta = 0, tb = 0;
+    for (int j = 0; j < SU_CO_WAVES; j++) {
+      ba += j < w ? wa[j] : 0;
+      bb += j < w ? wb[j] : 0;
+      ta += wa[j];
+      tb += wb[j];
+    }
+    if (k < nkeys) {
+      const int sl = carry_b + bb + ib - cp;
+      start[k] = carry_a + ba + ia - c;
+      slot_start[k] = sl;
+      for (int j = c; j < cp; j++) pad_slots[sl + j] = -1;
+    }
+    carry_a += ta;
+    carry_b += tb;
+    __syncthreads();
+  }
+  if (threadIdx.x == 0) {
+    const int sparse = lcnt[nkeys - 1];
+    counts[0] = carry_b - sparse;
+    counts[1] = sparse;
+    counts[2] = carry_b;
+  }
+  if (threadIdx.x >= 3 && threadIdx.x < TDR_SU_TAIL_INTS) counts[threadIdx.x] = 0;
 }
 
 __global__ __launch_bounds__(256) void su_scatter_kernel(const uint32_t* __restrict__ keys, const int32_t* __restrict__ vals,
@@ -1040,11 +1096,9 @@
     hipLaunchKernelGGL(su_key_kernel, dim3((unsigned)segs), dim3(256), sizeof(int) * (size_t)nkeys, s, L.st, L.cap, n, L.perm,
                        L.nb, L.span, SU_SEG, keys_in, vals_in, (int*)nullptr, seg_hist);
     LAUNCH_CHECK("su_key");
-    hipLaunchKernelGGL(su_colscan_kernel, dim3((unsigned)cdiv(nkeys, 64)), dim3(64 * SU_COLSCAN_WAVES), 0, s, seg_hist,
-                       (int)segs, nkeys, cnt);
-    LAUNCH_CHECK("su_colscan");
-    hipLaunchKernelGGL(su_offsets_kernel, dim3(1), dim3(256), 0, s, (const int*)cnt, nkeys, start, slot_start, counts, slots);
-    LAUNCH_CHECK("su_offsets");
+    hipLaunchKernelGGL(su_colscan_offsets_kernel, dim3(1), dim3(64 * SU_CO_WAVES), 0, s, seg_hist, (int)segs, nkeys, cnt, start,
+                       slot_start, counts, slots);
+    LAUNCH_CHECK("su_colscan_offsets");
     unsigned bits = 1;
     while ((1u << bits) < (unsigned)nkeys) bits++;
     hipLaunchKernelGGL(su_rank_scatter_kernel, dim3((unsigned)segs), dim3(64), sizeof(int) * (size_t)nkeys, s,
@@ -1057,8 +1111,7 @@
     hipLaunchKernelGGL(su_key_kernel, dim3((unsigned)cdiv(n, 256)), dim3(256), sizeof(int) * (size_t)nkeys, s, L.st, L.cap, n,
                        L.perm, L.nb, L.span, 256, keys_in, vals_in, cnt, (int*)nullptr);
     LAUNCH_CHECK("su_key");
-    hipLaunchKernelGGL(su_offsets_kernel, dim3(1), dim3(256), 0, s, (const int*)cnt, nkeys, start, slot_start, counts,
-                       (int32_t*)nullptr);
+    hipLaunchKernelGGL(su_offsets_kernel, dim3(1), dim3(256), 0, s, (const int*)cnt, nkeys, start, slot_start, counts);
     LAUNCH_CHECK("su_offsets");
     unsigned bits = 1;
     while ((1u << bits) < (unsigned)nkeys) bits++;
```

Result: no change. 23.71 million, median of 6 (+1.0%).
